# leonavery/KSFD

Hardware: AMD Instinct MI355X
Metric: grid-point-updates/sec (implicit step) (higher is better)
Workload: dtype f64

## Files before the change

### ksfd_amd/csrc/handle.hip.h

```cpp
#pragma once
enum { KC_RHS = 0, KC_JVP, KC_MULTIDOT, KC_GSUPDATE, KC_LINCOMB, KC_BASISAXPY, KC_FINISH, KC_REDUCE,
       KC_GFIELD, KC_VELOCITY, KC_MISC, KC_HALO, KC_MG, KC_SPECTRAL };
static const char *kc_names[KSFD_NKCLASS] = { "rhs", "jvp", "multidot", "gs_update", "lincomb", "basis_axpy",
                                              "rosw_finish", "reduce", "gfield", "velocity", "misc", "halo", "mg", "spectral" };
extern "C" const char *ksfd_kernel_class_name(int32_t c) { return (c >= 0 && c < KSFD_NKCLASS) ? kc_names[c] : "?"; }

static thread_local std::string g_create_error;

struct EvPair { hipEvent_t a, b; int cls; };

struct MGLevel {
    KGeom G;
    KPhys P;
    KVec kv;
    int64_t vlen = 0;
    int nblk = 1;
    double *coef = nullptr;
    float *dinv = nullptr;
    double *x = nullptr, *b = nullptr, *r = nullptr, *d = nullptr, *Ad = nullptr, *dG = nullptr;
    float *x32 = nullptr, *b32 = nullptr, *r32 = nullptr, *d32 = nullptr;
    float *coef32 = nullptr;
    bool f32 = false;
    double *pv = nullptr;
    double pv_norm = 0.0;
    double lam_max = 2.3;
    double ratio = 60.0;
};

struct SpecState {
    bool ok = false, means_valid = false, tile_major = false;
    int cols_split = 0;
    KFFTPlan px, py, pz;
    int dim = 2, lg_cz = 0, pb = 1, nent = 0, lg_rb3 = 0;
    size_t lds_y3 = 0, lds_z3 = 0;
    int *posz = nullptr, *kzofpos = nullptr;
    float *lz = nullptr;
    int rb = 0, npair = 0, nyp = 0;
    int nch = 1;
    size_t lds_rows = 0, lds_cols = 0;
    kcf *W = nullptr, *W2 = nullptr, *twx = nullptr, *twy = nullptr, *twz = nullptr;
    int *posy = nullptr, *kyofpos = nullptr;
    int2 *ytab = nullptr;
    int lgw = -1;
    int4 *pairtab = nullptr;
    int nxl = 0, nblk_cols = 0, lg_pl = 0;
    std::vector<A2APiece> a2a_fwd_s, a2a_fwd_r, a2a_bwd_s, a2a_bwd_r;
    float *lx = nullptr, *ly = nullptr;
    double a_rr = 0.0, a_rU[KSFD_MAXL] = { 0 };
    long long bad_until = 0;
    bool user_off = false;
    int backoff = 8;
    double rho_step = 0.0, rho_prev = 0.0;
};

struct LUState {
    int64_t n = 0, nnz = 0;
    double *A = nullptr;
    int *piv = nullptr, *perm = nullptr, *info = nullptr;
    long long *col = nullptr;
    double *val = nullptr;
    double *y = nullptr, *z = nullptr;
    std::vector<int> piv_h, perm_h;
    bool valid = false;
    double shift = 0.0;
};

struct ksfd_handle {
    ksfd_config cfg;
    int32_t lig_group[KSFD_MAXL];
    double lig_w[KSFD_MAXL], lig_s[KSFD_MAXL], lig_gamma[KSFD_MAXL], lig_D[KSFD_MAXL];
    double grp_alpha[KSFD_MAXL], grp_beta[KSFD_MAXL];
    KGeom G;
    KPhys P;
    KPhys Pst[4];
    bool Pst_valid[4] = { false, false, false, false };
    KVec kv;
    int rank = 0, size = 1, device = 0;
    bool ring = false;
    int64_t slow0 = 0;
    hipStream_t st = nullptr;
    hipStream_t st_comm = nullptr;
    hipEvent_t ev_ready = nullptr, ev_halo = nullptr;
    bool overlap = true;
    Transport *tr = nullptr;
    std::string err;

    int64_t vlen = 0;
    double *u = nullptr, *usave = nullptr, *Z = nullptr, *bvec = nullptr, *Y = nullptr, *V = nullptr;
    double *t1 = nullptr, *t2 = nullptr, *t3 = nullptr, *errv = nullptr;
    double *ckpt = nullptr;
    double *bstore = nullptr;
    bool spec_guess = true;
    int guess_max = getenv("KSFD_GUESS_MAX") ? std::max(1, std::min(atoi(getenv("KSFD_GUESS_MAX")), 3)) : 2;
    bool spec_predict = true;
    long long n_predicted = 0;
    long long n_residual = 0;
    long long n_host_sync = 0;
    struct SolverMemo { double lamJ; int lam_age, lam_period; double mg_shift_floor; int sf_dir, sf_hold; bool sf_tried_down; double sf_prev_its, sf_prev_floor;
                        long long nsteps, spec_bad_until; int spec_backoff; double spec_rho_step, spec_rho_prev; };
    SpecState spec;
    long long nsteps = 0;
    double spec_from = 0.1;
    SolverMemo ckpt_memo;
    bool ckpt_valid = false;
    double *Gb = nullptr, *dGb = nullptr;
    double *coef = nullptr;
    bool use_frozen = true;
    bool coef_fresh = false;
    double *flat = nullptr;
    double *src[4][KSFD_MAXL + 1];
    double *part = nullptr;
    double *dres = nullptr;
    double *hres = nullptr;
    double *hres_dev = nullptr;
    unsigned long long *pub_flag = nullptr, *pub_flag_dev = nullptr, pub_seq = 0;
    unsigned int *pub_count = nullptr;
    bool zero_copy = true;
    int restart_alloc = 0;
    bool restart_grow = true;
    int nblk_vec = 0;
    bool have_err = false;

    int use_fused = 1;
    int yseg = 48;
    int yseg_jvp = 16;
    int zseg = 32;

    bool profiling = false;
    int prof_only = -1;
    std::vector<EvPair> pending;
    std::vector<hipEvent_t> pool;
    ksfd_profile prof;
    double bytes_acc = 0.0;

    double *gm_dev = nullptr;
    double *gm_host = nullptr;
    std::vector<hipEvent_t> gm_ev;
    int async_mode = 0;

    double *Zb = nullptr;
    double *pvec = nullptr;
    double lamJ = -1.0;
    int lam_age = 0, lam_period = 1;
    int poly_deg = 0;
    double poly_alpha[8];
    double poly_shift = -1.0;
    int poly_max_deg = 6;
    double mg_threshold = 75.0;
    double poly_target = 0.02;
    float *coef32 = nullptr;
    bool rhs_carry = true;
    bool fuse_stage = true;
    bool j3l_attr_set = false, j3l_usable = false;
    bool rhs3d_strip = true;
    bool poly_fp32 = true;

    hipStream_t st_io = nullptr;
    double *snap_dev[2] = { nullptr, nullptr }, *snap_host[2] = { nullptr, nullptr };
    hipEvent_t snap_ready[2] = { nullptr, nullptr }, snap_done[2] = { nullptr, nullptr };
    bool snap_busy[2] = { false, false };
    int snap_next = 0;

    struct RecSpace { bool valid = false; int vb = 0, zb = 0, k = 0, pc = 0; std::vector<double> H; };
    RecSpace rec[4];
    int rec_vtop = 0, rec_ztop = 0;
    int rec_mode = 1;
    int rec_keep = 3;
    bool rhs_dots = true;
    bool rec_mg = false;

    int dr_keep = 0;
    bool dr_carry = false;
    double *dr_P = nullptr, *dr_Phost = nullptr;
    struct DrKept { bool valid = false; int kk = 0, pc = -1; double shift = 0.0, shift_pc = 0.0; std::vector<double> H; };
    DrKept dr;
    ksfd_deflation_stats dr_stats = {};

    LUState lu;

    std::vector<MGLevel> mg;
    double mg_shift_floor = 0.0;
    int sf_dir = 0, sf_hold = 0;
    bool sf_tried_down = false, sf_auto = true;
    double sf_prev_its = 0.0, sf_prev_floor = 0.0;
    bool mg_fp32 = true;
    bool mg_use32 = false;
    bool mg_graph_f32 = false;
    bool mg_warm_power = true;
    bool mg_fuse = true;
    bool mg_ok = false;
    double mg_shift = -1.0;
    bool mg_coef_valid = false;
    hipGraphExec_t mg_graph = nullptr;
    double mg_graph_shift = -1.0, mg_graph_bytes = 0.0;
    const void *mg_graph_x = nullptr;
    bool capturing = false, mg_use_graph = true;
    int mg_nu = 2, mg_ncoarse = 400, mg_power_its = 8;
    double mg_ratio = 6.0, mg_coarse_tol = 0.3;

    double At[4][4], Ginv[4][4], bt[4], b2t[4], asum[4];
};

#define GAMMA_RA 4.3586652150845900e-01

static int fail(ksfd_handle *h, int code, const char *fmt, ...)
{
    char buf[512];
    va_list ap;
    va_start(ap, fmt);
    vsnprintf(buf, sizeof buf, fmt, ap);
    va_end(ap);
    if (h) h->err = buf; else g_create_error = buf;
    return code;
}
#define HIPCHK(h, call)                                                                                   \
    do {                                                                                                  \
        hipError_t e_ = (call);                                                                           \
        if (e_ != hipSuccess) return fail(h, KSFD_EHIP, "%s failed: %s (%s:%d)", #call, hipGetErrorString(e_), __FILE__, __LINE__); \
    } while (0)

static hipEvent_t ev_get(ksfd_handle *h)
{
    if (!h->pool.empty()) { hipEvent_t e = h->pool.back(); h->pool.pop_back(); return e; }
    hipEvent_t e;
    hipEventCreate(&e);
    return e;
}
struct Scope {
    ksfd_handle *h; EvPair p; bool on;
    Scope(ksfd_handle *h_, int cls, double bytes, double alg = -1.0) : h(h_), on(h_->profiling && !h_->capturing && (h_->prof_only < 0 || h_->prof_only == cls))
    {
        h->bytes_acc += bytes;
        h->prof.bytes[cls] += bytes;
        h->prof.alg_bytes[cls] += alg < 0.0 ? bytes : alg;
        h->prof.launches[cls] += 1;
        if (on) { p.a = ev_get(h); p.b = ev_get(h); p.cls = cls; hipEventRecord(p.a, h->st); }
    }
    ~Scope() { if (on) { hipEventRecord(p.b, h->st); h->pending.push_back(p); } }
};
static void prof_resolve(ksfd_handle *h)
{
    if (h->pending.empty()) return;
    hipStreamSynchronize(h->st);
    for (auto &p : h->pending) {
        float ms = 0.f;
        if (hipEventElapsedTime(&ms, p.a, p.b) == hipSuccess) h->prof.ms[p.cls] += ms;
        h->pool.push_back(p.a);
        h->pool.push_back(p.b);
    }
    h->pending.clear();
}

static inline dim3 vgrid(const ksfd_handle *h) { return dim3(h->nblk_vec, h->G.F); }
static inline double vbytes(const ksfd_handle *h, double nvec) { return nvec * 8.0 * (double)h->G.F * (double)h->G.nloc; }

static void build_tableau(ksfd_handle *h)
{
    static const double A[4][4] = { { 0, 0, 0, 0 }, { 8.7173304301691801e-01, 0, 0, 0 },
                                    { 8.4457060015369423e-01, -1.1299064236484185e-01, 0, 0 }, { 0, 0, 1., 0 } };
    static const double Gm[4][4] = { { GAMMA_RA, 0, 0, 0 }, { -8.7173304301691801e-01, GAMMA_RA, 0, 0 },
                                     { -9.0338057013044082e-01, 5.4180672388095326e-02, GAMMA_RA, 0 },
                                     { 2.4212380706095346e-01, -1.2232505839045147e+00, 5.4526025533510214e-01, GAMMA_RA } };
    static const double b[4] = { 2.4212380706095346e-01, -1.2232505839045147e+00, 1.5452602553351020e+00, GAMMA_RA };
    static const double b2[4] = { 3.7810903145819369e-01, -9.6042292212423178e-02, 0.5, 2.1793326075422950e-01 };
    memset(h->Ginv, 0, sizeof h->Ginv);
    for (int col = 0; col < 4; col++)
        for (int i = col; i < 4; i++) {
            double s = (i == col) ? 1.0 : 0.0;
            for (int k = col; k < i; k++) s -= Gm[i][k] * h->Ginv[k][col];
            h->Ginv[i][col] = s / Gm[i][i];
        }
    for (int i = 0; i < 4; i++) {
        h->asum[i] = 0.0;
        for (int j = 0; j < 4; j++) {
            double s = 0.0;
            for (int k = 0; k < 4; k++) s += A[i][k] * h->Ginv[k][j];
            h->At[i][j] = s;
            h->asum[i] += A[i][j];
        }
    }
    for (int j = 0; j < 4; j++) {
        double s = 0.0, s2 = 0.0;
        for (int k = 0; k < 4; k++) { s += b[k] * h->Ginv[k][j]; s2 += b2[k] * h->Ginv[k][j]; }
        h->bt[j] = s;
        h->b2t[j] = s2;
    }
}

static int fill_phys(ksfd_handle *h, const ksfd_config *c, KPhys *dst = nullptr)
{
    if (c->nlig < 1 || c->nlig > KSFD_MAXL || c->ngroups < 1 || c->ngroups > KSFD_MAXL)
        return fail(h, KSFD_EINVAL, "nlig=%d ngroups=%d outside 1..%d", c->nlig, c->ngroups, KSFD_MAXL);
    KPhys &P = dst ? *dst : h->P;
    memset(&P, 0, sizeof P);
    P.nlig = c->nlig; P.ngroups = c->ngroups; P.cap_kind = c->cap_kind;
    for (int a = 0; a < 3; a++) {
        double sp = c->L[a] / (double)c->n[a];
        P.inv_h[a] = 1.0 / sp;
        P.inv_h2[a] = 1.0 / (sp * sp);
    }
    P.s2 = c->s2; P.rhomax = c->rhomax; P.inv_cushion = 1.0 / c->cushion; P.ms = c->maxscale * c->s2;
    P.rhomin = c->rhomin; P.Umin = c->Umin; P.inv_rhomax = 1.0 / c->rhomax;
    for (int l = 0; l < c->nlig; l++) {
        if (c->lig_group[l] < 0 || c->lig_group[l] >= c->ngroups) return fail(h, KSFD_EINVAL, "lig_group[%d] out of range", l);
        P.lig_group[l] = h->lig_group[l] = c->lig_group[l];
        P.lig_w[l] = h->lig_w[l] = c->lig_w[l];
        P.lig_s[l] = h->lig_s[l] = c->lig_s[l];
        P.lig_gamma[l] = h->lig_gamma[l] = c->lig_gamma[l];
        P.lig_D[l] = h->lig_D[l] = c->lig_D[l];
    }
    for (int l = c->nlig; l < KSFD_MAXL; l++) P.lig_group[l] = -1;
    for (int q = 0; q < c->ngroups; q++) {
        P.grp_alpha[q] = h->grp_alpha[q] = c->grp_alpha[q];
        P.grp_beta[q] = h->grp_beta[q] = c->grp_beta[q];
    }
    return KSFD_OK;
}

static int alloc_d(ksfd_handle *h, double **p, int64_t n)
{
    if (hipMalloc((void **)p, sizeof(double) * (size_t)n) != hipSuccess) return fail(h, KSFD_ENOMEM, "hipMalloc of %lld doubles failed", (long long)n);
    return KSFD_OK;
}

static bool fused_ok(const ksfd_handle *h)
{
    return h->use_fused && h->G.dim == 2 && (h->G.nx % 2 == 0) && h->G.nx >= 4 && h->G.sloc >= 4 && h->P.nlig <= 4;
}
static bool strip3d_ok(const ksfd_handle *h)
{
    return h->use_fused && h->G.dim == 3 && (h->G.nx % 2 == 0) && h->G.nx >= 4 && h->P.nlig <= 4;
}
```

### ksfd_amd/csrc/krylov.hip.h

```cpp
#pragma once
static int est_lambda_max(ksfd_handle *h, double shift, int nits)
{
    int rc;
    if (!h->pvec) {
        if (alloc_d(h, &h->pvec, h->vlen)) return KSFD_ENOMEM;
        const int nb = blocks_for(h->vlen);
        hipLaunchKernelGGL(k_hash_fill, dim3(nb), dim3(KSFD_BLOCK), 0, h->st, (long long)h->vlen, h->pvec);
        if ((rc = op_multidot(h, h->pvec, h->pvec, 0))) return rc;
        const double n0 = sqrt(h->hres[0]);
        const double *xs[1] = { h->pvec }; double a[1] = { 1.0 / n0 };
        if ((rc = op_lincomb(h, 1, xs, a, h->pvec))) return rc;
    }
    double lamA = 0.0;
    for (int it = 0; it < nits; it++) {
        if ((rc = op_jvp_frozen_halo(h, h->pvec, 1, shift, h->t3))) return rc;
        if ((rc = op_multidot(h, h->t3, h->t3, 0))) return rc;
        lamA = sqrt(h->hres[0]);
        if (!(lamA > 0.0) || lamA != lamA) return fail(h, KSFD_ENAN, "power iteration on the Jacobian broke down");
        const double *xs[1] = { h->t3 }; double a[1] = { 1.0 / lamA };
        if ((rc = op_lincomb(h, 1, xs, a, h->pvec))) return rc;
    }
    const double est = lamA - shift;
    h->lamJ = est > 0.0 ? est : 0.0;
    return KSFD_OK;
}

static void poly_setup(ksfd_handle *h, double shift)
{
    const double a = 0.97, b = 1.0 + 1.15 * h->lamJ / shift;
    h->poly_shift = shift;
    h->poly_deg = 0;
    const double kappa = b / a;
    if (kappa < 1.3) return;
    const double rc_ = (sqrt(kappa) - 1.0) / (sqrt(kappa) + 1.0);
    int d = (int)ceil(log(h->poly_target) / log(rc_)) - 1;
    d = std::min(std::max(d, 1), std::max(h->poly_max_deg, 1));
    const int n = d + 1;
    double m0 = (b + a) / (b - a), m1 = -2.0 / (b - a);
    double Tp[10] = { 1.0 }, Tc[10] = { m0, m1 }, Tn[10];
    int degc = 1;
    for (int k = 1; k < n; k++) {
        for (int i = 0; i < 10; i++) Tn[i] = 0.0;
        for (int i = 0; i <= degc; i++) { Tn[i] += 2.0 * m0 * Tc[i]; Tn[i + 1] += 2.0 * m1 * Tc[i]; }
        for (int i = 0; i <= degc - 1; i++) Tn[i] -= Tp[i];
        for (int i = 0; i < 10; i++) { Tp[i] = Tc[i]; Tc[i] = Tn[i]; }
        degc++;
    }
    const double t0 = Tc[0];
    for (int i = 0; i <= d; i++) h->poly_alpha[i] = -(Tc[i + 1] / t0) / shift;
    h->poly_deg = d;
}

static int poly_apply(ksfd_handle *h, double shift, double *v, double *z)
{
    int rc;
    const int d = h->poly_deg;
    const double *al = h->poly_alpha;
    if (h->poly_fp32 && h->coef32 && fused_ok(h)) {
        const float *C = h->coef32;
        float *tf[2] = { reinterpret_cast<float *>(h->t1), reinterpret_cast<float *>(h->t2) };
        const double *nod = nullptr;
        if (d == 1) return jvp2d_halo_t<float, double, double, double>(h, C, v, 4, shift, z, nod, al[0], al[1] / shift);
        if ((rc = jvp2d_halo_t<float, double, double, float>(h, C, v, 4, shift, tf[0], nod, al[d - 1], al[d] / shift))) return rc;
        int cur32 = 0;
        for (int i = d - 2; i >= 1; i--) {
            if ((rc = jvp2d_halo_t<float, float, double, float>(h, C, tf[cur32], 3, shift, tf[cur32 ^ 1], (const double *)v, al[i], 1.0 / shift))) return rc;
            cur32 ^= 1;
        }
        return jvp2d_halo_t<float, float, double, double>(h, C, tf[cur32], 3, shift, z, (const double *)v, al[0], 1.0 / shift);
    }
    double *tmp[2] = { h->t1, h->t2 };
    double *cur = (d == 1) ? z : tmp[0];
    if ((rc = op_jvp_frozen_halo(h, v, 4, shift, cur, nullptr, al[d - 1], al[d] / shift))) return rc;
    int flip = 1;
    for (int i = d - 2; i >= 0; i--) {
        double *nxt = (i == 0) ? z : tmp[flip];
        if ((rc = op_jvp_frozen_halo(h, cur, 3, shift, nxt, v, al[i], 1.0 / shift))) return rc;
        cur = nxt;
        flip ^= 1;
    }
    return KSFD_OK;
}

struct LinStats { int its; double rel; };

static void rec_reset(ksfd_handle *h)
{
    for (auto &r : h->rec) r.valid = false;
    h->rec_vtop = h->rec_ztop = 0;
}

static void hess_lsq(const double *H, int k, const double *g, double *y, double *Hy)
{
    const int ld = k + 1;
    std::vector<double> R((size_t)ld * k), q((size_t)k + 1);
    for (int i = 0; i < ld * k; i++) R[i] = H[i];
    for (int i = 0; i <= k; i++) q[i] = g[i];
    for (int j = 0; j < k; j++) {
        const double a = R[j * ld + j], b = R[j * ld + j + 1], den = hypot(a, b);
        const double c = den > 0.0 ? a / den : 1.0, sn = den > 0.0 ? b / den : 0.0;
        for (int l = j; l < k; l++) {
            const double t = c * R[l * ld + j] + sn * R[l * ld + j + 1];
            R[l * ld + j + 1] = -sn * R[l * ld + j] + c * R[l * ld + j + 1];
            R[l * ld + j] = t;
        }
        const double t = c * q[j] + sn * q[j + 1];
        q[j + 1] = -sn * q[j] + c * q[j + 1];
        q[j] = t;
    }
    for (int i = k - 1; i >= 0; i--) {
        double t = q[i];
        for (int l = i + 1; l < k; l++) t -= R[l * ld + i] * y[l];
        y[i] = R[i * ld + i] != 0.0 ? t / R[i * ld + i] : 0.0;
    }
    for (int i = 0; i <= k; i++) {
        double t = 0.0;
        for (int l = 0; l < k; l++) t += H[l * ld + i] * y[l];
        Hy[i] = t;
    }
}

static int gmres(ksfd_handle *h, const double *ustate, double shift, const double *b, double *x,
                 const ksfd_step_opts *o, LinStats *ls, int pcmode, int stage = -1, double tol_abs = -1.0)
{
    const bool use_pc = pcmode == 1;
    h->dr.valid = false;
    const double shift_pc = std::max(shift, h->mg_shift_floor);
    const bool use_poly = pcmode == 2 || pcmode == 3;
    auto apply_A = [&](const double *vin, double *wout) -> int {
        return h->use_frozen ? op_jvp_frozen(h, vin, 1, shift, wout) : op_jvp(h, ustate, vin, 1, shift, wout);
    };
    const int m_opt = std::min(o->ksp_restart > 0 ? o->ksp_restart : 30, h->restart_alloc);
    const int maxit = o->ksp_max_it > 0 ? o->ksp_max_it : 2000;
    const int64_t vs = h->vlen;
    const bool rec_full = use_pc && h->rec_mg && stage >= 0 && stage < 4 && h->use_frozen && h->rec_mode > 0;
    bool rec_on = stage >= 0 && stage < 4 && h->rec_mode > 0 && h->use_frozen && (!use_pc || rec_full);
    if (!rec_on || stage == 0 || h->restart_alloc - h->rec_vtop < (rec_full ? 16 : 6)) { if (stage != 0) rec_on = false; rec_reset(h); }
    const int vb = rec_on ? h->rec_vtop : 0, zb = rec_on ? h->rec_ztop : 0;
    const int m = h->restart_alloc - vb;
    int m_cur = (rec_full && rec_on) ? m : std::min(m_opt, m);
    double *V = h->V + (int64_t)vb * vs;
    double *Zq = use_poly ? h->Zb + (int64_t)zb * vs : nullptr;
    int rc;
    std::vector<double> H((size_t)(m + 1) * m, 0.0), Hraw((size_t)(m + 1) * m, 0.0), cs(m), sn(m), g(m + 1), y(m), hcol(m + 2), d(m + 2), Gm((size_t)(m + 1) * (m + 1), 0.0);
    static const int sel[4][3] = { { -1, -1, -1 }, { 0, -1, -1 }, { 0, -1, -1 }, { 0, 2, -1 } };
    int first_space = -1;
    std::vector<double> g_first((size_t)h->restart_alloc + 3, 0.0);
    if (rec_on && stage > 0)
        for (int q = 0; q < stage && first_space < 0; q++) {
            bool use = h->rec_mode == 2 || rec_full;
            for (int e = 0; e < 3; e++) use = use || sel[stage][e] == q;
            if (use && h->rec[q].valid && h->rec[q].pc == pcmode) first_space = q;
        }
    if (first_space >= 0) {
        const ksfd_handle::RecSpace &S = h->rec[first_space];
        if ((rc = op_multidot(h, b, h->V + (int64_t)S.vb * vs, S.k + 1))) return rc;
        for (int i = 0; i <= S.k + 1; i++) g_first[i] = h->hres[i];
    } else if ((rc = op_multidot(h, b, V, 0))) return rc;
    const double bn = sqrt(first_space >= 0 ? g_first[h->rec[first_space].k + 1] : h->hres[0]);
    ls->its = 0; ls->rel = 0.0;
    if (!(bn > 0.0)) {
        if (bn != bn) return fail(h, KSFD_ENAN, "GMRES: right-hand side is not finite");
        HIPCHK(h, hipMemsetAsync(x, 0, sizeof(double) * (size_t)vs, h->st));
        return KSFD_OK;
    }
    const double tol = tol_abs > 0.0 ? tol_abs : std::max(o->ksp_rtol * bn, o->ksp_atol);
    double beta = bn, rn = bn;
    int total = 0;
    bool first = true;
    bool x_set = false;
    bool restarted = false;
    const double *rsrc = b;
    const bool defer_x0 = rec_on && !use_pc;
    std::vector<double> xcoef((size_t)std::max(h->restart_alloc + 2, KSFD_MAXDOT), 0.0);
    bool x0_pending = false;
    double *const Xbase = use_poly ? h->Zb : h->V;
    const int xslot0 = use_poly ? zb : vb;
    bool pc_x0_pending = false;
    double *const rbuf = (x == h->t3) ? V : h->t3;
    if (rec_on && stage > 0) {
        int last_space = -1;
        for (int q = 0; q < stage; q++) {
            bool use = h->rec_mode == 2 || rec_full;
            for (int e = 0; e < 3; e++) use = use || sel[stage][e] == q;
            if (use && h->rec[q].valid && h->rec[q].pc == pcmode) last_space = q;
        }
        bool have_norm = false;
        for (int q = 0; q < stage; q++) {
            bool use = h->rec_mode == 2 || rec_full;
            for (int e = 0; e < 3; e++) use = use || sel[stage][e] == q;
            const ksfd_handle::RecSpace &S = h->rec[q];
            if (!use || !S.valid || S.pc != pcmode) continue;
            const double *Vs = h->V + (int64_t)S.vb * vs;
            const double *Zs = use_poly ? h->Zb + (int64_t)S.zb * vs : Vs;
            std::vector<double> gq_((size_t)S.k + 2), yq_((size_t)S.k + 1), Hy_((size_t)S.k + 2), neg_((size_t)S.k + 2);
            double *gq = gq_.data(), *yq = yq_.data(), *Hy = Hy_.data(), *neg = neg_.data();
            if (q == first_space && rsrc == b) {
                for (int i = 0; i <= S.k; i++) gq[i] = g_first[i];
            } else {
                if ((rc = op_multidot(h, rsrc, Vs, S.k + 1))) return rc;
                for (int i = 0; i <= S.k; i++) gq[i] = h->hres[i];
            }
            hess_lsq(S.H.data(), S.k, gq, yq, Hy);
            if (use_pc) {
                if ((rc = op_basis_axpy(h, h->t2, Vs, S.k, yq, pc_x0_pending ? 1.0 : 0.0))) return rc;
                pc_x0_pending = true;
            } else if (defer_x0) {
                for (int i = 0; i < S.k; i++) xcoef[(use_poly ? S.zb : S.vb) + i] += yq[i];
                x0_pending = true;
            } else {
// ... 355 lines not shown
```

### ksfd_amd/csrc/ksfd_hip.hip

```cpp
#include <hip/hip_runtime.h>
#include <dlfcn.h>
#include <math.h>
#include <stdarg.h>
#include <stdio.h>
#include <stdlib.h>
#include <string.h>
#include <string>
#include <vector>

#include "../../include/ksfd_hip.h"
#include "stencil.hip.h"
#include "mg.hip.h"
#include "spectral.hip.h"
#include "lu.hip.h"
#include "transport.h"


#include "handle.hip.h"
#include "ops.hip.h"
#include "spectral_host.hip.h"
#include "mg_host.hip.h"
#include "krylov.hip.h"
#include "krylov_dr.hip.h"
#include "lu_host.hip.h"
// ... 40 lines not shown
{
    if (!cfg || !out) return fail(nullptr, KSFD_EINVAL, "null argument");
    *out = nullptr;
    if (cfg->dim < 1 || cfg->dim > 3) return fail(nullptr, KSFD_EINVAL, "dim must be 1, 2 or 3");
    for (int a = 0; a < cfg->dim; a++)
        if (cfg->n[a] < 5) return fail(nullptr, KSFD_EINVAL, "n[%d]=%lld < 5: the width-2 periodic star needs >= 5 points", a, (long long)cfg->n[a]);
    ksfd_handle *h = new ksfd_handle();
    memset(h->src, 0, sizeof h->src);
    memset(&h->prof, 0, sizeof h->prof);
    h->cfg = *cfg;
    h->cfg.lig_group = nullptr; h->cfg.lig_w = h->cfg.lig_s = h->cfg.lig_gamma = h->cfg.lig_D = nullptr;
    h->cfg.grp_alpha = h->cfg.grp_beta = nullptr;
    int rc = fill_phys(h, cfg);
    if (rc) { g_create_error = h->err; delete h; return rc; }
    h->rank = dist ? dist->rank : 0;
    h->size = dist ? dist->size : 1;
    h->device = dist ? dist->device : 0;
    if (h->size < 1 || h->rank < 0 || h->rank >= h->size) { delete h; return fail(nullptr, KSFD_EINVAL, "bad rank/size"); }
    h->ring = h->size > 1 || (dist && dist->transport != 0);
    int ndev = 0;
    if (hipGetDeviceCount(&ndev) != hipSuccess || ndev < 1) { delete h; return fail(nullptr, KSFD_EHIP, "no HIP device available (libksfd_hip has no CPU path)"); }
    if (h->device < 0 || h->device >= ndev) { delete h; return fail(nullptr, KSFD_EINVAL, "device %d of %d", h->device, ndev); }
#define CFAIL(code, ...) do { int rc_ = fail(nullptr, code, __VA_ARGS__); ksfd_destroy(h); return rc_; } while (0)
    if (hipSetDevice(h->device) != hipSuccess) CFAIL(KSFD_EHIP, "hipSetDevice(%d) failed", h->device);
    if (hipStreamCreateWithFlags(&h->st, hipStreamNonBlocking) != hipSuccess) CFAIL(KSFD_EHIP, "hipStreamCreate failed");
    if (h->ring && (hipStreamCreateWithFlags(&h->st_comm, hipStreamNonBlocking) != hipSuccess ||
                        hipEventCreateWithFlags(&h->ev_ready, hipEventDisableTiming) != hipSuccess ||
                        hipEventCreateWithFlags(&h->ev_halo, hipEventDisableTiming) != hipSuccess)) CFAIL(KSFD_EHIP, "comm stream/event creation failed");

    KGeom &G = h->G;
    G.dim = cfg->dim; G.F = cfg->nlig + 1;
    const int slow = cfg->dim - 1;
    int64_t nglob = cfg->n[slow];
    if (h->size > 1 && (nglob % h->size != 0 || nglob / h->size < 4))
        CFAIL(KSFD_EINVAL, "slab axis extent %lld must be divisible by %d ranks with >= 4 units each", (long long)nglob, h->size);
    int64_t sloc = nglob / h->size;
    h->slow0 = sloc * h->rank;
    G.ng = h->ring ? 2 : 0;
    G.wrap_slow = !h->ring;
    G.nx = cfg->n[0]; G.ny = cfg->dim >= 2 ? cfg->n[1] : 1; G.nz = cfg->dim >= 3 ? cfg->n[2] : 1;
    if (slow == 0) G.nx = sloc; else if (slow == 1) G.ny = sloc; else G.nz = sloc;
    G.inner = slow == 0 ? 1 : (slow == 1 ? G.nx : G.nx * G.ny);
    G.sloc = sloc;
    G.plane = (sloc + 2 * G.ng) * G.inner;
    G.nloc = sloc * G.inner;
    h->kv.plane = G.plane; h->kv.off = (long long)G.ng * G.inner; h->kv.nloc = G.nloc; h->kv.nf = G.F;
    h->vlen = (int64_t)G.F * G.plane;
    h->nblk_vec = (int)std::min<long long>((G.nloc + KSFD_BLOCK - 1) / KSFD_BLOCK, 2048);
    build_tableau(h);

    h->restart_alloc = 30;
    int fit_local = 30;
    {
        size_t mfree = 0, mtotal = 0;
        if (hipMemGetInfo(&mfree, &mtotal) == hipSuccess && mfree > 0) {
            const double vecbytes = 8.0 * (double)h->vlen;
            const double room = 0.92 * (double)mfree / vecbytes - 30.0;
            const int fit_room = (int)floor(std::min((room - 1.0) / 2.0, 1.0e6));
            const int fit_40 = (int)floor(std::min(0.4 * (double)mfree / vecbytes / 2.0, 1.0e6));
            static const int cap = getenv("KSFD_RESTART_MAX") ? std::max(8, std::min(atoi(getenv("KSFD_RESTART_MAX")), 120)) : 120;
            fit_local = std::max(std::min(std::min(cap, fit_room), fit_40), std::min(30, fit_room));
        }
    }
    if (alloc_d(h, &h->dres, 128)) CFAIL(KSFD_ENOMEM, "%s", h->err.c_str());
    if (h->ring) {
        std::string terr;
        h->tr = make_transport(dist, G.F, G.inner, terr);
        if (!h->tr) CFAIL(KSFD_ECOMM, "transport %d: %s", dist->transport, terr.c_str());
        double v = -(double)fit_local;
        if (hipMemcpyAsync(h->dres, &v, sizeof v, hipMemcpyHostToDevice, h->st) != hipSuccess || h->tr->allreduce(h->dres, 1, 1, h->st))
            CFAIL(KSFD_ECOMM, "agreeing on the restart length failed: %s", h->tr->error().c_str());
        if (h->tr->result_on_host()) v = h->tr->host_result()[0];
        else if (hipMemcpyAsync(&v, h->dres, sizeof v, hipMemcpyDeviceToHost, h->st) != hipSuccess || hipStreamSynchronize(h->st) != hipSuccess)
            CFAIL(KSFD_EHIP, "reading the agreed restart length failed");
        fit_local = (int)(-v + 0.5);
    }
    if (fit_local != 30) {
        if (fit_local < 8) CFAIL(KSFD_ENOMEM, "grid too large for this device: a vector is %.2f GB, the solver needs ~47 of them (restart length that fits: %d)", 8.0 * (double)h->vlen / 1e9, fit_local);
        h->restart_alloc = fit_local;
    }
    double **vecs[] = { &h->u, &h->usave, &h->Z, &h->bvec, &h->t1, &h->t2, &h->t3, &h->errv };
    for (double **v : vecs) {
        if (alloc_d(h, v, h->vlen)) CFAIL(KSFD_ENOMEM, "%s", h->err.c_str());
        hipMemsetAsync(*v, 0, sizeof(double) * (size_t)h->vlen, h->st);
    }
    if (alloc_d(h, &h->Y, 4 * h->vlen) || alloc_d(h, &h->V, (int64_t)(h->restart_alloc + 1) * h->vlen) ||
        alloc_d(h, &h->Gb, G.plane) || alloc_d(h, &h->dGb, G.plane) || alloc_d(h, &h->coef, (int64_t)(3 + cfg->nlig) * G.plane) ||
        alloc_d(h, &h->flat, (int64_t)std::max(G.F, 3) * G.nloc) ||
        alloc_d(h, &h->part, (int64_t)(2 * KSFD_MAXDOT + 4) * 4096))
        CFAIL(KSFD_ENOMEM, "%s", h->err.c_str());
    if (hipMalloc((void **)&h->Zb, sizeof(double) * (size_t)h->restart_alloc * (size_t)h->vlen) != hipSuccess) { h->Zb = nullptr; hipGetLastError(); }
    hipMemsetAsync(h->Y, 0, sizeof(double) * (size_t)(4 * h->vlen), h->st);
    hipMemsetAsync(h->V, 0, sizeof(double) * (size_t)((h->restart_alloc + 1) * h->vlen), h->st);
    if (hipHostMalloc((void **)&h->hres, sizeof(double) * 128 + 64, hipHostMallocMapped | hipHostMallocCoherent) != hipSuccess) CFAIL(KSFD_ENOMEM, "hipHostMalloc failed");
    h->pub_flag = reinterpret_cast<unsigned long long *>(h->hres + 128);
    *h->pub_flag = 0;
    if (hipHostGetDevicePointer((void **)&h->hres_dev, h->hres, 0) != hipSuccess || hipMalloc((void **)&h->pub_count, sizeof(unsigned int)) != hipSuccess ||
        hipMemset(h->pub_count, 0, sizeof(unsigned int)) != hipSuccess) { h->zero_copy = false; h->hres_dev = nullptr; }
    else h->pub_flag_dev = reinterpret_cast<unsigned long long *>(h->hres_dev + 128);
    {
        const int m = h->restart_alloc;
        const size_t ndev = (size_t)(m + 1) * (m + 1) + (size_t)(m + 1) * m + 2 * m + (m + 1) + KSFD_MAXDOT + 1 + 2 * (m + 1);
        const size_t nhost = 2 * (m + 1) + (size_t)(m + 1) * m + (m + 1);
        if (alloc_d(h, &h->gm_dev, (int64_t)ndev)) CFAIL(KSFD_ENOMEM, "%s", h->err.c_str());
        if (hipHostMalloc((void **)&h->gm_host, sizeof(double) * nhost, hipHostMallocDefault) != hipSuccess) CFAIL(KSFD_ENOMEM, "hipHostMalloc failed");
        h->gm_ev.resize(m + 1);
        for (auto &e : h->gm_ev) if (hipEventCreateWithFlags(&e, hipEventDisableTiming) != hipSuccess) CFAIL(KSFD_EHIP, "hipEventCreate failed");
    }

    spec_build(h);
    if (mg_build(h)) { mg_free(h); h->mg_ok = false; }
    if ((h->spec.ok || h->mg_ok) && alloc_d(h, &h->bstore, 3 * h->vlen)) { h->bstore = nullptr; h->spec_guess = false; h->err.clear(); }
    if (h->ring) {
        double flags[3] = { h->spec.ok ? 1.0 : 0.0, h->mg_ok ? 1.0 : 0.0, (h->spec_guess && h->bstore) ? 1.0 : 0.0 };
        for (double &f : flags) f = -f;
        if (hipMemcpyAsync(h->dres, flags, sizeof flags, hipMemcpyHostToDevice, h->st) != hipSuccess || h->tr->allreduce(h->dres, 3, 1, h->st))
            CFAIL(KSFD_ECOMM, "agreeing on the available solvers failed: %s", h->tr->error().c_str());
        if (h->tr->result_on_host()) memcpy(flags, h->tr->host_result(), sizeof flags);
        else if (hipMemcpyAsync(flags, h->dres, sizeof flags, hipMemcpyDeviceToHost, h->st) != hipSuccess || hipStreamSynchronize(h->st) != hipSuccess)
            CFAIL(KSFD_EHIP, "reading the agreed solver flags failed");
        if (flags[0] > -0.5 && h->spec.ok) spec_free(h);
        if (flags[1] > -0.5 && h->mg_ok) { mg_free(h); h->mg_ok = false; }
        if (flags[2] > -0.5) h->spec_guess = false;
    }
    if (hipStreamSynchronize(h->st) != hipSuccess) CFAIL(KSFD_EHIP, "stream sync failed in create");
#undef CFAIL
    *out = h;
    return KSFD_OK;
}

extern "C" int ksfd_rccl_unique_id(void *out128)
{
    if (!out128) return KSFD_EINVAL;
    std::string err;
    RcclApi api;
    if (!api.load(err)) return fail(nullptr, KSFD_ECOMM, "%s", err.c_str());
    auto getid = (decltype(&ncclGetUniqueId))dlsym(api.lib, "ncclGetUniqueId");
    if (!getid) return fail(nullptr, KSFD_ECOMM, "librccl lacks ncclGetUniqueId");
    ncclUniqueId id;
    ncclResult_t r = getid(&id);
    if (r != ncclSuccess) return fail(nullptr, KSFD_ECOMM, "ncclGetUniqueId: %s", api.GetErrorString(r));
    memcpy(out128, &id, sizeof id);
    return KSFD_OK;
}

extern "C" int ksfd_update_params(ksfd_handle *h, const ksfd_config *cfg)
{
    if (!h || !cfg) return KSFD_EINVAL;
    if (cfg->dim != h->cfg.dim || cfg->nlig != h->cfg.nlig) return fail(h, KSFD_EINVAL, "update_params cannot change dim/nlig");
    for (int a = 0; a < 3; a++) if (cfg->n[a] != h->cfg.n[a]) return fail(h, KSFD_EINVAL, "update_params cannot change the grid");
    h->cfg = *cfg;
    h->cfg.lig_group = nullptr; h->cfg.lig_w = h->cfg.lig_s = h->cfg.lig_gamma = h->cfg.lig_D = nullptr;
    h->cfg.grp_alpha = h->cfg.grp_beta = nullptr;
    h->coef_fresh = false;
    return fill_phys(h, cfg);
}

extern "C" int ksfd_set_stage_params(ksfd_handle *h, int32_t stage, const ksfd_config *cfg)
{
    if (!h || stage < -1 || stage > 3) return KSFD_EINVAL;
    if (!cfg) {
        for (int s = 0; s < 4; s++) if (stage == -1 || s == stage) h->Pst_valid[s] = false;
        return KSFD_OK;
    }
    if (cfg->dim != h->cfg.dim || cfg->nlig != h->cfg.nlig) return fail(h, KSFD_EINVAL, "set_stage_params cannot change dim/nlig");
    for (int a = 0; a < 3; a++) if (cfg->n[a] != h->cfg.n[a] || cfg->L[a] != h->cfg.L[a]) return fail(h, KSFD_EINVAL, "set_stage_params cannot change the grid");
    for (int s = 0; s < 4; s++) {
        if (stage != -1 && s != stage) continue;
        int rc = fill_phys(h, cfg, &h->Pst[s]);
        if (rc) return rc;
        h->Pst_valid[s] = true;
    }
    return KSFD_OK;
}

extern "C" int ksfd_local_range(const ksfd_handle *h, int64_t *b, int64_t *e)
{
    if (!h) return KSFD_EINVAL;
    if (b) *b = h->slow0;
    if (e) *e = h->slow0 + h->G.sloc;
    return KSFD_OK;
}
extern "C" int64_t ksfd_local_size(const ksfd_handle *h) { return h ? (int64_t)h->G.F * h->G.nloc : 0; }
extern "C" double *ksfd_device_state(ksfd_handle *h) { return h ? h->u : nullptr; }
extern "C" int64_t ksfd_device_plane_stride(const ksfd_handle *h) { return h ? h->G.plane : 0; }
extern "C" int64_t ksfd_device_interior_offset(const ksfd_handle *h) { return h ? (int64_t)h->G.ng * h->G.inner : 0; }

extern "C" int ksfd_set_state(ksfd_handle *h, const double *u, int32_t layout)
{
    if (!h || !u) return KSFD_EINVAL;
    hipSetDevice(h->device);
    int rc = upload(h, u, layout, h->u);
    h->coef_fresh = false;
    if (rc) return rc;
    HIPCHK(h, hipStreamSynchronize(h->st));
    return KSFD_OK;
}
extern "C" int ksfd_snapshot_begin(ksfd_handle *h, int32_t layout, int32_t *slot)
{
    if (!h || !slot) return KSFD_EINVAL;
    if (layout < 0 || layout > 2) return fail(h, KSFD_EINVAL, "bad layout %d", layout);
    hipSetDevice(h->device);
    const KGeom &G = h->G;
    const size_t bytes = sizeof(double) * (size_t)G.F * G.nloc;
    if (!h->st_io) {
        if (hipStreamCreateWithFlags(&h->st_io, hipStreamNonBlocking) != hipSuccess) return fail(h, KSFD_EHIP, "hipStreamCreate (io) failed");
        for (int q = 0; q < 2; q++) {
            if (hipMalloc((void **)&h->snap_dev[q], bytes) != hipSuccess || hipHostMalloc((void **)&h->snap_host[q], bytes, hipHostMallocDefault) != hipSuccess)
                return fail(h, KSFD_ENOMEM, "snapshot staging buffers (%zu bytes each) could not be allocated", bytes);
            if (hipEventCreateWithFlags(&h->snap_ready[q], hipEventDisableTiming) != hipSuccess ||
                hipEventCreateWithFlags(&h->snap_done[q], hipEventDisableTiming) != hipSuccess) return fail(h, KSFD_EHIP, "hipEventCreate failed");
        }
    }
    const int q = h->snap_next;
    h->snap_next ^= 1;
    if (h->snap_busy[q]) HIPCHK(h, hipEventSynchronize(h->snap_done[q]));
    {
        Scope sc(h, KC_MISC, vbytes(h, 2));
        hipLaunchKernelGGL(k_to_host_layout, vgrid(h), dim3(KSFD_BLOCK), 0, h->st, G, layout, (const double *)h->u, G.plane,
                           (long long)G.ng * G.inner, h->snap_dev[q]);
    }
    HIPCHK(h, hipGetLastError());
    HIPCHK(h, hipEventRecord(h->snap_ready[q], h->st));
    HIPCHK(h, hipStreamWaitEvent(h->st_io, h->snap_ready[q], 0));
    HIPCHK(h, hipMemcpyAsync(h->snap_host[q], h->snap_dev[q], bytes, hipMemcpyDeviceToHost, h->st_io));
    HIPCHK(h, hipEventRecord(h->snap_done[q], h->st_io));
    h->snap_busy[q] = true;
    *slot = q;
    return KSFD_OK;
}

extern "C" int ksfd_snapshot_wait(ksfd_handle *h, int32_t slot, const double **host)
{
    if (!h || !host || slot < 0 || slot > 1) return KSFD_EINVAL;
    if (!h->snap_busy[slot]) return fail(h, KSFD_EINVAL, "snapshot slot %d holds nothing", slot);
    hipSetDevice(h->device);
    HIPCHK(h, hipEventSynchronize(h->snap_done[slot]));
    *host = h->snap_host[slot];
    return KSFD_OK;
}

extern "C" int ksfd_checkpoint(ksfd_handle *h, int32_t op)
{
    if (!h || op < 0 || op > 1) return KSFD_EINVAL;
    hipSetDevice(h->device);
    h->dr.valid = false;
    if (op == 0) {
        if (!h->ckpt && alloc_d(h, &h->ckpt, h->vlen)) return KSFD_ENOMEM;
        HIPCHK(h, hipMemcpyAsync(h->ckpt, h->u, sizeof(double) * (size_t)h->vlen, hipMemcpyDeviceToDevice, h->st));
        h->ckpt_memo = { h->lamJ, h->lam_age, h->lam_period, h->mg_shift_floor, h->sf_dir, h->sf_hold, h->sf_tried_down, h->sf_prev_its, h->sf_prev_floor,
                         h->nsteps, h->spec.bad_until, h->spec.backoff, h->spec.rho_step, h->spec.rho_prev };
        for (MGLevel &L : h->mg) L.pv_norm = 0.0;
        h->ckpt_valid = true;
        return KSFD_OK;
    }
    if (!h->ckpt_valid) return fail(h, KSFD_EINVAL, "no checkpoint has been saved");
    HIPCHK(h, hipMemcpyAsync(h->u, h->ckpt, sizeof(double) * (size_t)h->vlen, hipMemcpyDeviceToDevice, h->st));
    h->coef_fresh = false;
    const ksfd_handle::SolverMemo &m = h->ckpt_memo;
    h->lamJ = m.lamJ; h->lam_age = m.lam_age; h->lam_period = m.lam_period; h->mg_shift_floor = m.mg_shift_floor;
    h->sf_dir = m.sf_dir; h->sf_hold = m.sf_hold; h->sf_tried_down = m.sf_tried_down; h->sf_prev_its = m.sf_prev_its; h->sf_prev_floor = m.sf_prev_floor;
    h->nsteps = m.nsteps; h->spec.bad_until = m.spec_bad_until; h->spec.backoff = m.spec_backoff; h->spec.means_valid = false;
    h->spec.rho_step = m.spec_rho_step; h->spec.rho_prev = m.spec_rho_prev;
    h->mg_coef_valid = false; h->mg_shift = -1.0; h->poly_shift = -1.0; h->have_err = false;
    for (MGLevel &L : h->mg) L.pv_norm = 0.0;
    rec_reset(h);
    return KSFD_OK;
}

extern "C" int ksfd_set_state_random(ksfd_handle *h, const int64_t *nc, const double *z, double rho0)
{
    if (!h || !nc || !z) return KSFD_EINVAL;
    hipSetDevice(h->device);
    int64_t n = 1;
    for (int a = 0; a < 3; a++) {
        if (a < h->G.dim ? nc[a] < 1 : nc[a] != 1) return fail(h, KSFD_EINVAL, "coarse grid must be >= 1 per used axis and 1 elsewhere");
        n *= nc[a];
    }
    double *dz = nullptr;
    h->coef_fresh = false;
    if (hipMalloc((void **)&dz, sizeof(double) * (size_t)n) != hipSuccess) return fail(h, KSFD_ENOMEM, "hipMalloc of the coarse samples failed");
    hipError_t e = hipMemcpyAsync(dz, z, sizeof(double) * (size_t)n, hipMemcpyHostToDevice, h->st);
    const KGeom &G = h->G;
    int nb = (int)std::min<long long>((G.nloc + KSFD_BLOCK - 1) / KSFD_BLOCK, 65535);
    if (e == hipSuccess) {
        Scope sc(h, KC_MISC, vbytes(h, 1));
        NL_DISPATCH(h->P.nlig, hipLaunchKernelGGL((k_random_start<NL>), dim3(nb), dim3(KSFD_BLOCK), 0, h->st, G, h->P, (long long)h->cfg.n[G.dim - 1],
                                                  (long long)h->slow0, (long long)nc[0], (long long)nc[1], (long long)nc[2], (const double *)dz, rho0, h->u));
        e = hipGetLastError();
    }
    if (e == hipSuccess) e = hipStreamSynchronize(h->st);
    hipFree(dz);
    if (e != hipSuccess) return fail(h, KSFD_EHIP, "random start: %s", hipGetErrorString(e));
    return KSFD_OK;
}
extern "C" int ksfd_get_state(ksfd_handle *h, double *u, int32_t layout)
{
    if (!h || !u) return KSFD_EINVAL;
    hipSetDevice(h->device);
    return download(h, h->u, layout, u);
}

extern "C" int ksfd_set_source(ksfd_handle *h, int32_t stage, int32_t field, const double *srch, int32_t layout)
{
    if (!h || field < 0 || field >= h->G.F || stage < -1 || stage > 3) return h ? fail(h, KSFD_EINVAL, "bad stage/field") : KSFD_EINVAL;
    if (layout != KSFD_LAYOUT_SOA) return fail(h, KSFD_EINVAL, "sources are single dense planes: pass layout SOA");
    hipSetDevice(h->device);
    for (int s = 0; s < 4; s++) {
        if (stage != -1 && s != stage) continue;
        if (!srch) {
            if (h->src[s][field]) { HIPCHK(h, hipStreamSynchronize(h->st)); hipFree(h->src[s][field]); h->src[s][field] = nullptr; }
            continue;
        }
        if (!h->src[s][field] && alloc_d(h, &h->src[s][field], h->G.nloc)) return KSFD_ENOMEM;
        HIPCHK(h, hipMemcpyAsync(h->src[s][field], srch, sizeof(double) * (size_t)h->G.nloc, hipMemcpyHostToDevice, h->st));
    }
    HIPCHK(h, hipStreamSynchronize(h->st));
    return KSFD_OK;
}

extern "C" int ksfd_rhs(ksfd_handle *h, double t, const double *uh, double *outh, int32_t layout)
{
    (void)t;
    if (!h || !outh) return KSFD_EINVAL;
    hipSetDevice(h->device);
    int rc;
    double *uin = h->u;
    if (uh) { if ((rc = upload(h, uh, layout, h->t1))) return rc; uin = h->t1; }
    if ((rc = halo(h, uin))) return rc;
    if ((rc = op_rhs(h, uin, 0, h->t3))) return rc;
    return download(h, h->t3, layout, outh);
}

extern "C" int ksfd_jvp(ksfd_handle *h, const double *uh, const double *vh, double *outh, int32_t layout)
{
    if (!h || !vh || !outh) return KSFD_EINVAL;
    hipSetDevice(h->device);
    int rc;
    double *uin = h->u;
    if (uh) { if ((rc = upload(h, uh, layout, h->t1))) return rc; uin = h->t1; }
    if ((rc = upload(h, vh, layout, h->t2))) return rc;
    if ((rc = halo(h, uin)) || (rc = halo(h, h->t2))) return rc;
    if (!uh && h->use_frozen) {
        if ((rc = ensure_coef(h, true))) return rc;
        if ((rc = op_jvp_frozen(h, h->t2, 0, 0.0, h->t3))) return rc;
    } else if ((rc = op_jvp(h, uin, h->t2, 0, 0.0, h->t3))) return rc;
    return download(h, h->t3, layout, outh);
}

static int velocity_common(ksfd_handle *h, const double *uin, double *vel_dev, double vmax[3])
{
    const KGeom &G = h->G;
    int rc;
    const double *Gplane = h->Gb;
    if (uin == h->u && h->use_frozen) {
        if ((rc = ensure_coef(h))) return rc;
        Gplane = h->coef + G.plane;
    } else {
        if ((rc = halo(h, (double *)uin))) return rc;
        Scope sc(h, KC_GFIELD, 8.0 * (G.F + 1) * (double)G.plane);
        NL_DISPATCH(h->P.nlig, hipLaunchKernelGGL((k_gfield<NL, false>), dim3(plane_blocks(G)), dim3(KSFD_BLOCK), 0, h->st, G, h->P, uin, (const double *)nullptr, h->Gb, (double *)nullptr));
    }
    int nb = (int)std::min<long long>((G.nloc + KSFD_BLOCK - 1) / KSFD_BLOCK, 1024);
    if (vmax && !vel_dev && G.dim == 2 && (G.nx % 2 == 0) && G.nx >= 4) {
        const int bx = (int)((G.nx / 2 + KSFD_BLOCK - 1) / KSFD_BLOCK), by = (int)std::min<long long>(G.sloc, std::max(1, 2048 / bx));
        nb = bx * by;
        Scope sc(h, KC_VELOCITY, 8.0 * (double)G.nloc);
        hipLaunchKernelGGL(k_velmax2d, dim3(bx, by), dim3(KSFD_BLOCK), 0, h->st, G, h->P, Gplane, h->part);
    } else if (vmax && !vel_dev && G.dim == 3 && (G.nx % 2 == 0) && G.nx >= 4 && G.ny >= 4 && G.nx * G.ny < (1LL << 30)) {
        const int bx = (int)((G.nx / 2 * G.ny + KSFD_BLOCK - 1) / KSFD_BLOCK);
        int zseg = (int)G.sloc;
        while (zseg >= 32 && (long long)bx * ((G.sloc + zseg - 1) / zseg) < 8192) zseg = (zseg + 1) / 2;
        const int by = (int)((G.sloc + zseg - 1) / zseg);
        nb = bx * by;
        if (3LL * nb > part_capacity()) return fail(h, KSFD_EINVAL, "velocity_max: grid too large for the partial-result buffer");
        Scope sc(h, KC_VELOCITY, 8.0 * (double)G.nloc);
        hipLaunchKernelGGL(k_velmax3d, dim3(bx, by), dim3(KSFD_BLOCK), 0, h->st, G, h->P, zseg, Gplane, h->part);
    } else {
        Scope sc(h, KC_VELOCITY, 8.0 * (double)G.nloc * (1 + (vel_dev ? G.dim : 0)));
        hipLaunchKernelGGL(k_velocity, dim3(nb), dim3(KSFD_BLOCK), 0, h->st, G, h->P, Gplane, vel_dev, vmax ? h->part : (double *)nullptr);
    }
    HIPCHK(h, hipGetLastError());
    if (vmax) {
        if ((rc = reduce_rows(h, 3, nb, 1))) return rc;
        for (int a = 0; a < 3; a++) vmax[a] = a < G.dim ? h->hres[a] : 0.0;
    }
    return KSFD_OK;
}

extern "C" int ksfd_velocity(ksfd_handle *h, const double *uh, double *velh, int32_t layout)
{
    if (!h || !velh) return KSFD_EINVAL;
    if (layout != KSFD_LAYOUT_SOA) return fail(h, KSFD_EINVAL, "velocity output is dim dense SoA planes: pass layout SOA for it");
    hipSetDevice(h->device);
    int rc;
    double *uin = h->u;
    if (uh) { if ((rc = upload(h, uh, layout, h->t1))) return rc; uin = h->t1; }
    if ((rc = velocity_common(h, uin, h->flat, nullptr))) return rc;
    HIPCHK(h, hipMemcpyAsync(velh, h->flat, sizeof(double) * (size_t)h->G.dim * h->G.nloc, hipMemcpyDeviceToHost, h->st));
    HIPCHK(h, hipStreamSynchronize(h->st));
    return KSFD_OK;
}

extern "C" int ksfd_velocity_max(ksfd_handle *h, double vmax[3])
{
    if (!h || !vmax) return KSFD_EINVAL;
    hipSetDevice(h->device);
    return velocity_common(h, h->u, nullptr, vmax);
}

extern "C" int ksfd_groom(ksfd_handle *h)
{
    if (!h) return KSFD_EINVAL;
    hipSetDevice(h->device);
    Scope sc(h, KC_MISC, vbytes(h, 2));
    hipLaunchKernelGGL(k_groom, vgrid(h), dim3(KSFD_BLOCK), 0, h->st, h->kv, h->u, h->P.rhomin, h->P.Umin);
    HIPCHK(h, hipGetLastError());
    return KSFD_OK;
}

extern "C" int ksfd_count_worms(ksfd_handle *h, double *total)
{
    if (!h || !total) return KSFD_EINVAL;
    hipSetDevice(h->device);
    {
        Scope sc(h, KC_MISC, 8.0 * (double)h->G.nloc);
        hipLaunchKernelGGL(k_sum_rho, dim3(h->nblk_vec), dim3(KSFD_BLOCK), 0, h->st, h->kv, h->u, h->part);
    }
    HIPCHK(h, hipGetLastError());
    int rc = reduce_rows(h, 1, h->nblk_vec, 0);
    if (rc) return rc;
    *total = h->hres[0];
    return KSFD_OK;
}

extern "C" int ksfd_scale_rho(ksfd_handle *h, double factor)
{
    if (!h) return KSFD_EINVAL;
    hipSetDevice(h->device);
    h->coef_fresh = false;
    Scope sc(h, KC_MISC, 16.0 * (double)h->G.nloc);
    hipLaunchKernelGGL(k_mul_rho, dim3(h->nblk_vec), dim3(KSFD_BLOCK), 0, h->st, h->kv, h->u, (const double *)nullptr, factor);
    HIPCHK(h, hipGetLastError());
    return KSFD_OK;
}

extern "C" int ksfd_mul_rho(ksfd_handle *h, const double *fh)
{
    if (!h || !fh) return KSFD_EINVAL;
    hipSetDevice(h->device);
    HIPCHK(h, hipMemcpyAsync(h->flat, fh, sizeof(double) * (size_t)h->G.nloc, hipMemcpyHostToDevice, h->st));
    h->coef_fresh = false;
    Scope sc(h, KC_MISC, 24.0 * (double)h->G.nloc);
    hipLaunchKernelGGL(k_mul_rho, dim3(h->nblk_vec), dim3(KSFD_BLOCK), 0, h->st, h->kv, h->u, (const double *)h->flat, 1.0);
    HIPCHK(h, hipGetLastError());
    HIPCHK(h, hipStreamSynchronize(h->st));
    return KSFD_OK;
}

extern "C" int ksfd_jacobian_nnz(ksfd_handle *h, int64_t *nrows, int64_t *nnz)
{
    if (!h) return KSFD_EINVAL;
    const int64_t npts = 4 * h->G.dim + 1;
    if (nrows) *nrows = (int64_t)h->G.F * h->G.nloc;
    if (nnz) *nnz = h->G.nloc * ((int64_t)h->G.F * npts + (int64_t)h->P.nlig * (npts + 1));
    return KSFD_OK;
}

extern "C" int ksfd_jacobian_csr(ksfd_handle *h, int64_t *rowptr, int64_t *col, double *val)
{
    if (!h || !rowptr || !col || !val) return KSFD_EINVAL;
    hipSetDevice(h->device);
    int64_t nrows, nnz;
    ksfd_jacobian_nnz(h, &nrows, &nnz);
    int rc;
    if ((rc = ensure_coef(h))) return rc;
    long long *dcol = nullptr;
    double *dval = nullptr;
    if (hipMalloc((void **)&dcol, sizeof(long long) * (size_t)nnz) != hipSuccess ||
        hipMalloc((void **)&dval, sizeof(double) * (size_t)nnz) != hipSuccess) {
        if (dcol) hipFree(dcol);
        return fail(h, KSFD_ENOMEM, "hipMalloc of the CSR staging buffers failed");
    }
    const KGeom &G = h->G;
    int nb = (int)std::min<long long>((G.nloc + KSFD_BLOCK - 1) / KSFD_BLOCK, 65535);
    {
        Scope sc(h, KC_MISC, 16.0 * (double)nnz + 8.0 * (3 + h->P.nlig) * (double)G.nloc);
        NL_DISPATCH(h->P.nlig, hipLaunchKernelGGL((k_jac_csr<NL>), dim3(nb), dim3(KSFD_BLOCK), 0, h->st, G, h->P, (const double *)h->coef,
                                                  (long long)h->cfg.n[G.dim - 1], (long long)h->slow0, dcol, dval));
    }
    hipError_t e = hipGetLastError();
    if (e == hipSuccess) e = hipMemcpyAsync(col, dcol, sizeof(long long) * (size_t)nnz, hipMemcpyDeviceToHost, h->st);
    if (e == hipSuccess) e = hipMemcpyAsync(val, dval, sizeof(double) * (size_t)nnz, hipMemcpyDeviceToHost, h->st);
    if (e == hipSuccess) e = hipStreamSynchronize(h->st);
    hipFree(dcol);
    hipFree(dval);
    if (e != hipSuccess) return fail(h, KSFD_EHIP, "jacobian export: %s", hipGetErrorString(e));
    const int64_t npts = 4 * G.dim + 1, F = G.F, per = F * npts + (F - 1) * (npts + 1);
    for (int64_t p = 0; p < G.nloc; p++) {
        rowptr[p * F] = p * per;
        for (int64_t l = 1; l < F; l++) rowptr[p * F + l] = p * per + F * npts + (l - 1) * (npts + 1);
    }
    rowptr[nrows] = nnz;
    return KSFD_OK;
}


extern "C" void ksfd_default_step_opts(ksfd_step_opts *o)
{
    memset(o, 0, sizeof *o);
    o->rtol = 1e-5; o->atol = 1e-5;
    o->adapt = 1; o->max_reject = 10;
    o->clip_lo = 0.1; o->clip_hi = 5.0;
    o->dt_min = 1e-20; o->dt_max = 1e4;
    o->safety = 0.9; o->reject_safety = 0.5;
    o->ksp_rtol = 1e-6; o->ksp_atol = 1e-50;
    o->ksp_restart = 30; o->ksp_max_it = 2000;
    o->pc_type = 2;
}

extern "C" int ksfd_step(ksfd_handle *h, double *t, double *hstep, const ksfd_step_opts *opts, ksfd_step_stats *stats)
{
    if (!h || !t || !hstep || !opts) return KSFD_EINVAL;
    hipSetDevice(h->device);
    const bool direct = opts->pc_type == 5;
    if (direct) {
        const int g = direct_guard(h);
        if (g) return g;
    }
    const bool dr_on = h->dr_keep > 0 && !direct;
    if (dr_on) {
        const int m_dr = std::min(opts->ksp_restart > 0 ? opts->ksp_restart : 30, h->restart_alloc);
        if (h->dr_keep > m_dr - 3) return fail(h, KSFD_EINVAL, "deflation: keep = %d needs a restart length of at least %d (ksp_restart %d, basis vectors allocated %d)", h->dr_keep, h->dr_keep + 3, (int)opts->ksp_restart, h->restart_alloc);
    }
    memset(&h->dr_stats, 0, sizeof h->dr_stats);
    if (getenv("KSFD_PC_SIGMA")) { h->mg_shift_floor = atof(getenv("KSFD_PC_SIGMA")); h->sf_auto = false; }
    ksfd_step_stats st;
    memset(&st, 0, sizeof st);
    const double bytes0 = h->bytes_acc;
    const int64_t rhs0 = h->prof.launches[KC_RHS], jvp0 = h->prof.launches[KC_JVP];
    int64_t launches0 = 0;
    for (int c = 0; c < KSFD_NKCLASS; c++) launches0 += h->prof.launches[c];
    const long long sync0 = h->n_host_sync, pred0 = h->n_predicted, resid0 = h->n_residual;
    int rc = KSFD_OK;
    const int64_t vs = h->vlen;
    double hh = *hstep;
    bool prev_accept = !(opts->reserved & 4);
    bool lam_done = false;
    int rejects = 0;
    const int max_rej = opts->max_reject < 0 ? 0x7fffffff : opts->max_reject;
    const bool single = (opts->reserved & 2) != 0;
    {
        Scope sc(h, KC_MISC, vbytes(h, 3));
        hipLaunchKernelGGL(k_groom, vgrid(h), dim3(KSFD_BLOCK), 0, h->st, h->kv, h->u, h->P.rhomin, h->P.Umin, h->usave);
        if (hipGetLastError() != hipSuccess) { rc = fail(h, KSFD_EHIP, "k_groom launch failed"); goto out; }
    }
    if ((rc = halo(h, h->u))) goto out;
    if (h->use_frozen && (rc = ensure_coef(h, true))) goto out;
    h->poly_shift = -1.0;
    h->nsteps++;
    if (h->spec.rho_step > 0.0) h->spec.rho_prev = h->spec.rho_step;
    h->spec.rho_step = 0.0;
    while (true) {
        const double shift = 1.0 / (GAMMA_RA * hh);
        h->dr.valid = false;
        double dmax = h->P.s2, lap = 0.0;
        for (int l = 0; l < h->P.nlig; l++) dmax = std::max(dmax, h->P.lig_D[l]);
        for (int a = 0; a < h->G.dim; a++) lap += (16.0 / 3.0) * h->P.inv_h2[a];
        const double stiff = dmax * lap / shift;
        const double mg_from = h->mg_threshold * ((double)h->G.F * (double)h->G.nloc < 8.0e6 ? 3.0 : 1.0);
        bool use_spec = !direct && h->spec.ok && h->use_frozen && (opts->pc_type == 4 || (opts->pc_type == 2 && stiff >= (fused_ok(h) ? h->spec_from : std::max(h->spec_from, 0.3)) && h->nsteps > h->spec.bad_until && !h->spec.user_off));
        if (use_spec) {
            if (!h->Zb && alloc_d(h, &h->Zb, (int64_t)h->restart_alloc * h->vlen)) { rc = KSFD_ENOMEM; goto out; }
            if (!h->spec.means_valid && (rc = spec_means(h))) goto out;
        }
        const bool use_pc = !direct && !use_spec && h->mg_ok && h->use_frozen && (opts->pc_type == 1 || (opts->pc_type == 2 && stiff > mg_from));
        bool use_poly = false;
        if (!use_spec && !use_pc && h->use_frozen && (opts->pc_type == 2 || opts->pc_type == 3) && stiff >= 0.3) {
            if (!h->Zb && alloc_d(h, &h->Zb, (int64_t)h->restart_alloc * h->vlen)) { rc = KSFD_ENOMEM; goto out; }
            if (!lam_done) {
                if (h->lamJ < 0.0 || ++h->lam_age >= h->lam_period) {
                    const double before = h->lamJ;
                    if ((rc = est_lambda_max(h, shift, before < 0.0 ? 8 : 2))) goto out;
                    const bool stable = before > 0.0 && fabs(h->lamJ - before) <= 0.02 * before;
                    h->lam_period = stable ? std::min(2 * h->lam_period, 8) : 1;
                    h->lam_age = 0;
                }
                lam_done = true;
            }
            if (h->poly_shift != shift) poly_setup(h, shift);
            use_poly = h->poly_deg >= 1 && h->poly_max_deg >= 1;
        }
        const bool small = (double)h->G.F * (double)h->G.nloc <= 6.0e6;
        const bool use_async = !dr_on && !direct && !use_spec && !use_pc && !use_poly && h->use_frozen && !(opts->reserved & 1) && stiff >= 1e-3 &&
                               (!h->ring || h->tr->device_allreduce()) &&
                               (h->async_mode == 1 || (h->async_mode == 2 && small));
        h->mg_use32 = opts->ksp_rtol >= 1e-7;
        const bool fuse_stage = (fused_ok(h) || (strip3d_ok(h) && h->rhs3d_strip)) && h->P.nlig <= 4 && h->fuse_stage;
        const int its_before = st.linear_its;
        bool spec_failed = false;
        const bool guess_on = (use_spec || use_pc) && fuse_stage && h->spec_guess && h->bstore;
        double gb[4][4];
        if (direct && !(rc = ensure_coef(h, true))) rc = direct_factor(h, shift);
        for (int i = 0; i < 4 && !rc; i++) {
            const double *zin = h->u;
            double bnorm2 = -1.0;
            bool rhs_dots_done = false;
            double rhs_dot[2] = { 0.0, 0.0 };
            double *bcur = (guess_on && i < 3) ? h->bstore + (int64_t)i * vs : h->bvec;
            if (fuse_stage) {
                KComb cmb = KComb{};
                for (int j = 0; j < i; j++) {
                    if (h->At[i][j] != 0.0) { cmb.yin[cmb.nin] = h->Y + (int64_t)j * vs; cmb.ain[cmb.nin++] = h->At[i][j]; }
                    if (h->Ginv[i][j] != 0.0) { cmb.yout[cmb.nout] = h->Y + (int64_t)j * vs; cmb.aout[cmb.nout++] = -h->Ginv[i][j] / hh; }
                }
                const int gdot_j0 = std::max(0, i - h->guess_max), gdot_n = (guess_on && i > 0 && h->rhs_dots) ? i - gdot_j0 : 0;
                const bool rhs_norm = use_spec && fused_ok(h) && (!(guess_on && i > 0) || (gdot_n > 0 && gdot_n <= 2 && strip_waves(h) * (1 + gdot_n) <= part_capacity()));
                rhs_dots_done = rhs_norm && gdot_n > 0;
                if ((rc = op_rhs(h, h->u, i, bcur, &cmb, rhs_norm, i > 0 ? h->Y + (int64_t)(i - 1) * vs : nullptr, rhs_dots_done ? gdot_n : 0,
                                 rhs_dots_done ? h->bstore + (int64_t)gdot_j0 * vs : nullptr))) break;
                if (rhs_norm) bnorm2 = h->hres[0];
                if (rhs_dots_done) for (int j = 0; j < gdot_n; j++) rhs_dot[j] = h->hres[1 + j];
            } else {
            if (i > 0) {
                const double *xs[5]; double a[5]; int nt = 0;
                xs[nt] = h->u; a[nt++] = 1.0;
                for (int j = 0; j < i; j++) if (h->At[i][j] != 0.0) { xs[nt] = h->Y + (int64_t)j * vs; a[nt++] = h->At[i][j]; }
                if (nt > 1) {
                    if ((rc = op_lincomb(h, nt, xs, a, h->Z))) break;
                    if ((rc = halo(h, h->Z))) break;
                    zin = h->Z;
                }
            }
            if ((rc = op_rhs(h, zin, i, h->bvec))) break;
            if (i > 0) {
                const double *xs[5]; double a[5]; int nt = 0;
                xs[nt] = h->bvec; a[nt++] = 1.0;
                for (int j = 0; j < i; j++) if (h->Ginv[i][j] != 0.0) { xs[nt] = h->Y + (int64_t)j * vs; a[nt++] = -h->Ginv[i][j] / hh; }
                if (nt > 1 && (rc = op_lincomb(h, nt, xs, a, h->bvec))) break;
            }
            }
            LinStats ls;
            SpecGuess sg;
            sg.n = 0;
            {
                if (guess_on) {
                    if (i == 0) {
                        if (bnorm2 < 0.0) { if ((rc = op_multidot(h, bcur, bcur, 0))) break; bnorm2 = h->hres[0]; }
                        gb[0][0] = bnorm2;
                    }
                    else {
                        const int j0 = std::max(0, i - h->guess_max), ng = i - j0;
                        if (rhs_dots_done) {
                            for (int j = 0; j < ng; j++) gb[i][j0 + j] = gb[j0 + j][i] = rhs_dot[j];
                            gb[i][i] = bnorm2;
                        } else {
                            if ((rc = op_multidot(h, bcur, h->bstore + (int64_t)j0 * vs, ng))) break;
                            for (int j = 0; j < ng; j++) gb[i][j0 + j] = gb[j0 + j][i] = h->hres[j];
                            gb[i][i] = bnorm2 = h->hres[ng];
                        }
                        double M[3][4];
                        for (int a = 0; a < ng; a++) { for (int c = 0; c < ng; c++) M[a][c] = gb[j0 + a][j0 + c]; M[a][ng] = gb[i][j0 + a]; M[a][a] *= 1.0 + 1e-13; }
                        bool okls = ng > 0;
                        for (int c = 0; c < ng && okls; c++) {
                            int pv = c;
                            for (int a = c + 1; a < ng; a++) if (fabs(M[a][c]) > fabs(M[pv][c])) pv = a;
                            if (!(fabs(M[pv][c]) > 0.0)) { okls = false; break; }
                            for (int q = 0; q <= ng; q++) std::swap(M[c][q], M[pv][q]);
                            for (int a = c + 1; a < ng; a++) { const double f = M[a][c] / M[c][c]; for (int q = c; q <= ng; q++) M[a][q] -= f * M[c][q]; }
                        }
                        double cf[3] = { 0, 0, 0 };
                        for (int a = ng - 1; a >= 0 && okls; a--) { double t = M[a][ng]; for (int q = a + 1; q < ng; q++) t -= M[a][q] * cf[q]; cf[a] = t / M[a][a]; }
                        double pred = gb[i][i];
                        for (int a = 0; a < ng; a++) { pred -= 2.0 * cf[a] * gb[i][j0 + a]; for (int c = 0; c < ng; c++) pred += cf[a] * cf[c] * gb[j0 + a][j0 + c]; }
                        if (okls && pred == pred && pred < 0.09 * gb[i][i]) {
                            for (int j = 0; j < ng; j++) if (cf[j] != 0.0) { sg.Y[sg.n] = h->Y + (int64_t)(j0 + j) * vs; sg.b[sg.n] = h->bstore + (int64_t)(j0 + j) * vs; sg.c[sg.n++] = cf[j]; }
                        }
                    }
                }
            }
            if (direct) {
                rc = direct_stage(h, shift, bcur, h->Y + (int64_t)i * vs, opts, &ls);
                st.pc_used |= 16;
            } else if (use_spec) {
                const bool skip = spec_failed && opts->pc_type == 2;
                if (!skip) {
                    rc = spec_solve(h, shift, bcur, h->Y + (int64_t)i * vs, opts, &ls, bnorm2, opts->pc_type == 2 ? (h->spec.backoff > 8 ? 8 : 40) : 0, sg.n ? &sg : nullptr);
                    st.pc_used |= 8;
                }
                if (skip || (rc == KSFD_ELINEAR && opts->pc_type == 2)) {
                    if (!skip) st.linear_its += ls.its;
                    spec_failed = true;
                    const bool mg_here = h->mg_ok && stiff > 0.3;
                    rc = gmres(h, h->u, shift, bcur, h->Y + (int64_t)i * vs, opts, &ls, mg_here ? 1 : 0);
                    st.pc_used |= mg_here ? 2 : 1;
                }
            } else if (use_pc && sg.n) {
                double *xi = h->Y + (int64_t)i * vs;
                const double *xs[3]; double a[3];
                for (int j = 0; j < sg.n; j++) { xs[j] = sg.Y[j]; a[j] = sg.c[j]; }
                if ((rc = op_lincomb(h, sg.n, xs, a, xi)) || (rc = halo(h, xi)) || (rc = op_jvp_frozen(h, xi, 2, shift, h->Z, bcur))) break;
                const double tol = std::max(opts->ksp_rtol * sqrt(bnorm2), opts->ksp_atol);
                rc = dr_on ? gmres_dr(h, h->u, shift, h->Z, h->t3, opts, &ls, 1, i, tol)
                           : gmres(h, h->u, shift, h->Z, h->t3, opts, &ls, 1, i, tol);
                if (!rc) { const double *x2[2] = { xi, h->t3 }; double a2[2] = { 1.0, 1.0 }; rc = op_lincomb(h, 2, x2, a2, xi); }
                st.pc_used |= 2;
            } else {
            rc = use_async ? gmres_async(h, shift, bcur, h->Y + (int64_t)i * vs, opts, &ls)
                 : dr_on ? gmres_dr(h, h->u, shift, bcur, h->Y + (int64_t)i * vs, opts, &ls, use_pc ? 1 : (use_poly ? 2 : 0), i)
                           : gmres(h, h->u, shift, bcur, h->Y + (int64_t)i * vs, opts, &ls, use_pc ? 1 : (use_poly ? 2 : 0), i);
            st.pc_used |= use_pc ? 2 : (use_poly ? 4 : 1);
            }
            st.linear_its += ls.its;
            st.ksp_resid = ls.rel;
            {
                static const bool stage_trace = getenv("KSFD_STAGE_TRACE") != nullptr;
                if (stage_trace) fprintf(stderr, "[stage %d] its %d rel %.2e guess %d\n", i, ls.its, ls.rel, sg.n);
            }
            if (rc == KSFD_ELINEAR && !direct && !use_pc && h->mg_ok && h->use_frozen && opts->pc_type) {
                rc = gmres(h, h->u, shift, bcur, h->Y + (int64_t)i * vs, opts, &ls, 1);
                st.pc_used |= 2;
                st.linear_its += ls.its;
                st.ksp_resid = ls.rel;
            }
        }
        if (use_spec && opts->pc_type == 2) {
            if (spec_failed || st.linear_its - its_before > 48) {
                h->spec.bad_until = h->nsteps + h->spec.backoff;
                h->spec.backoff = std::min(2 * h->spec.backoff, 512);
            } else h->spec.backoff = 8;
        }
        if (!rc && use_pc && h->sf_auto) {
            const double its = (double)(st.linear_its - its_before);
            if (h->sf_dir == 0) {
                if (h->sf_hold > 0) h->sf_hold--;
                else if (its > 64.0) {
                    h->sf_prev_its = its; h->sf_prev_floor = h->mg_shift_floor;
                    h->mg_shift_floor = 2.0 * std::max(h->mg_shift_floor, shift);
                    h->sf_dir = 1; h->sf_tried_down = false;
                }
            } else if (its < 0.95 * h->sf_prev_its) {
                h->sf_prev_its = its; h->sf_prev_floor = h->mg_shift_floor;
                h->mg_shift_floor = h->sf_dir > 0 ? 2.0 * h->mg_shift_floor : 0.5 * h->mg_shift_floor;
                if (h->mg_shift_floor <= shift) { h->sf_dir = 0; h->sf_hold = 25; }
            } else {
                h->mg_shift_floor = h->sf_prev_floor;
                if (h->sf_dir > 0 && !h->sf_tried_down && 0.5 * h->sf_prev_floor > shift) {
                    h->sf_dir = -1; h->sf_tried_down = true;
                    h->mg_shift_floor = 0.5 * h->sf_prev_floor;
                } else { h->sf_dir = 0; h->sf_hold = 25; }
            }
        }
        if (rc == KSFD_ELINEAR && opts->adapt && !single && rejects < max_rej && hh * 0.25 >= opts->dt_min) {
            rejects++;
            st.rejections = rejects;
            prev_accept = false;
            if ((rc = op_copy(h, h->u, h->usave))) goto out;
            hh *= 0.25;
            *hstep = hh;
            if ((rc = halo(h, h->u))) goto out;
            continue;
        }
        if (rc) { op_copy(h, h->u, h->usave); hipStreamSynchronize(h->st); goto out; }
        {
            Scope sc(h, KC_FINISH, vbytes(h, 7));
            hipLaunchKernelGGL(k_rosw_finish, dim3(h->nblk_vec), dim3(KSFD_BLOCK), 0, h->st, h->kv, h->u, h->Y, vs,
                               h->bt[0], h->bt[1], h->bt[2], h->bt[3], h->b2t[0] - h->bt[0], h->b2t[1] - h->bt[1],
                               h->b2t[2] - h->bt[2], h->b2t[3] - h->bt[3], opts->atol, opts->rtol, h->errv, h->part);
        }
        h->have_err = true;
        h->coef_fresh = false;
        if ((rc = reduce_rows(h, 1, h->nblk_vec, 0))) goto out;
        {
            double ntot = (double)h->G.F * (double)h->cfg.n[0] * (double)h->cfg.n[1] * (double)h->cfg.n[2];
            st.wrms = sqrt(h->hres[0] / ntot);
        }
        if (!(st.wrms == st.wrms) || isinf(st.wrms)) {
            op_copy(h, h->u, h->usave); hipStreamSynchronize(h->st);
            h->coef_fresh = h->use_frozen;
            rc = fail(h, KSFD_ENAN, "non-finite error norm at t=%g h=%g", *t, hh);
            goto out;
        }
        bool accept = true;
        double hnext = hh;
        if (opts->adapt) {
            double safety = opts->safety;
            if (st.wrms > 1.0) {
                if (!prev_accept) safety *= opts->reject_safety;
                accept = hh < (1.0 + 1.4901161193847656e-08) * opts->dt_min;
            }
            double hfac = st.wrms > 0.0 ? safety * pow(st.wrms, -1.0 / 3.0) : INFINITY;
            hfac = std::min(std::max(hfac, opts->clip_lo), opts->clip_hi);
            hnext = std::min(std::max(hh * hfac, opts->dt_min), opts->dt_max);
        }
        prev_accept = accept;
        if (accept) {
            st.accepted = 1; st.h_used = hh;
            *t += hh;
            *hstep = hnext;
            break;
        }
        rejects++;
        st.rejections = rejects;
        if ((rc = op_copy(h, h->u, h->usave))) goto out;
        h->coef_fresh = h->use_frozen;
        hh = hnext;
        *hstep = hnext;
        if (single) break;
        if (rejects > max_rej) { rc = fail(h, KSFD_EREJECT, "step rejected %d times at t=%g", rejects, *t); break; }
        if ((rc = halo(h, h->u))) goto out;
    }
out:
    prof_resolve(h);
    st.bytes = h->bytes_acc - bytes0;
    st.rhs_evals = (int32_t)(h->prof.launches[KC_RHS] - rhs0);
    st.jvp_evals = (int32_t)(h->prof.launches[KC_JVP] - jvp0);
    {
        int64_t l1 = 0;
        for (int c = 0; c < KSFD_NKCLASS; c++) l1 += h->prof.launches[c];
        st.launches = (int32_t)(l1 - launches0);
    }
    st.host_syncs = (int32_t)(h->n_host_sync - sync0);
    st.predicted_final = (int32_t)(h->n_predicted - pred0);
    st.residual_evals = (int32_t)(h->n_residual - resid0);
    if (stats) *stats = st;
    return rc;
}

extern "C" int ksfd_get_last_error_vector(ksfd_handle *h, double *eh, int32_t layout)
{
    if (!h || !eh) return KSFD_EINVAL;
    if (!h->have_err) return fail(h, KSFD_EINVAL, "no step has been attempted yet");
    hipSetDevice(h->device);
    return download(h, h->errv, layout, eh);
}

extern "C" int ksfd_set_profiling(ksfd_handle *h, int32_t on)
{
    if (!h) return KSFD_EINVAL;
    prof_resolve(h);
    if (on < 0 || on >= 2 + KSFD_NKCLASS) return KSFD_EINVAL;
    h->profiling = on != 0;
    h->prof_only = on >= 2 ? on - 2 : -1;
    return KSFD_OK;
}
extern "C" int ksfd_get_profile(ksfd_handle *h, ksfd_profile *p, int32_t reset)
{
    if (!h || !p) return KSFD_EINVAL;
    prof_resolve(h);
    *p = h->prof;
    if (reset) memset(&h->prof, 0, sizeof h->prof);
    return KSFD_OK;
}
extern "C" int ksfd_set_mg_params(ksfd_handle *h, int32_t nu, int32_t ncoarse_max, int32_t power_its, double ratio, double coarse_tol)
{
    if (!h) return KSFD_EINVAL;
    if (nu > 0) h->mg_nu = nu;
    if (ncoarse_max > 0) h->mg_ncoarse = ncoarse_max;
    if (power_its > 0) h->mg_power_its = power_its;
    if (ratio > 1.0) h->mg_ratio = ratio;
    if (coarse_tol > 0.0) h->mg_coarse_tol = coarse_tol;
    h->mg_use_graph = power_its != -7 && !h->ring;
    h->mg_shift = -1.0;
    return KSFD_OK;
}
extern "C" int ksfd_set_poly_params(ksfd_handle *h, int32_t max_degree, double target, double mg_threshold)
{
    if (!h || max_degree < 0 || max_degree > 7) return KSFD_EINVAL;
    if (mg_threshold > 0.0) h->mg_threshold = mg_threshold;
    h->poly_max_deg = max_degree;
    if (target > 0.0 && target < 1.0) h->poly_target = target;
    h->poly_shift = -1.0;
    return KSFD_OK;
}
extern "C" int ksfd_spectral_apply(ksfd_handle *h, double shift, const double *vh, double *outh, int32_t layout)
{
    if (!h || !vh || !outh || !(shift > 0.0)) return KSFD_EINVAL;
    hipSetDevice(h->device);
    if (!h->spec.ok) return fail(h, KSFD_EINVAL, "spectral preconditioner not available for this handle (needs power-of-two extents of 32 ... 16384 points; 1, 2, 4 or 8 slab ranks with an all-to-all transport)");
    int rc;
    if ((rc = upload(h, vh, layout, h->t2))) return rc;
    if ((rc = ensure_coef(h))) return rc;
    if ((rc = spec_means(h)) || (rc = spec_apply(h, shift, h->t2, h->t3))) return rc;
    return download(h, h->t3, layout, outh);
}
extern "C" int ksfd_direct_apply(ksfd_handle *h, double shift, const double *vh, double *outh, int32_t layout)
{
    if (!h || !vh || !outh) return KSFD_EINVAL;
    if (!isfinite(shift)) return fail(h, KSFD_EINVAL, "direct_apply: non-finite shift");
    if (layout < 0 || layout > 2) return fail(h, KSFD_EINVAL, "bad layout %d", layout);
    hipSetDevice(h->device);
    int rc;
    if ((rc = direct_guard(h))) return rc;
    if ((rc = ensure_coef(h)) || (rc = direct_factor(h, shift))) return rc;
    if ((rc = upload(h, vh, layout, h->t2)) || (rc = direct_solve(h, h->t2, h->t3))) return rc;
    return download(h, h->t3, layout, outh);
}
extern "C" int ksfd_set_deflation(ksfd_handle *h, int32_t keep, int32_t carry_stages)
{
    if (!h) return KSFD_EINVAL;
    if (keep < 0 || keep > 16) return fail(h, KSFD_EINVAL, "deflation: keep = %d outside 0 (off) .. 16", (int)keep);
    h->dr_keep = keep;
    h->dr_carry = carry_stages != 0;
    h->dr.valid = false;
    return KSFD_OK;
}
extern "C" int ksfd_get_deflation_stats(ksfd_handle *h, ksfd_deflation_stats *s)
{
    if (!h || !s) return KSFD_EINVAL;
    *s = h->dr_stats;
    return KSFD_OK;
}
extern "C" int32_t ksfd_basis_capacity(const ksfd_handle *h) { return h ? h->restart_alloc + 1 : 0; }
extern "C" int ksfd_basis_rotate(ksfd_handle *h, int32_t nin, int32_t nout, const double *P, const double *vin, double *vout, int32_t layout)
{
    if (!h || !P || !vin || !vout) return KSFD_EINVAL;
    if (layout < 0 || layout > 2) return fail(h, KSFD_EINVAL, "bad layout %d", layout);
    if (nin < 1 || nout < 1 || nout > nin || nout > KSFD_ROT_MAXOUT || nin > KSFD_ROT_MAXIN || nin > h->restart_alloc + 1)
        return fail(h, KSFD_EINVAL, "basis_rotate: %d -> %d vectors outside 1 <= nout <= %d, nout <= nin <= min(%d, %d)", (int)nin, (int)nout, KSFD_ROT_MAXOUT, KSFD_ROT_MAXIN, h->restart_alloc + 1);
    hipSetDevice(h->device);
    h->dr.valid = false;
    rec_reset(h);
    int rc;
    const int64_t nl = (int64_t)h->G.F * h->G.nloc;
    for (int i = 0; i < nin; i++) {
        if ((rc = upload(h, vin + (int64_t)i * nl, layout, h->V + (int64_t)i * h->vlen))) return rc;
        HIPCHK(h, hipStreamSynchronize(h->st));
    }
    std::vector<double> Pp((size_t)nin * KSFD_ROT_MAXOUT, 0.0);
    for (int i = 0; i < nin; i++) for (int j = 0; j < nout; j++) Pp[(size_t)i * KSFD_ROT_MAXOUT + j] = P[(size_t)i * nout + j];
    if ((rc = op_basis_rotate(h, h->V, nin, nout, Pp.data(), KSFD_ROT_MAXOUT))) return rc;
    for (int i = 0; i < nin; i++)
        if ((rc = download(h, h->V + (int64_t)i * h->vlen, layout, vout + (int64_t)i * nl))) return rc;
    return KSFD_OK;
}
extern "C" int ksfd_set_spectral_params(ksfd_handle *h, double from_stiffness, int32_t enable)
{
    if (!h) return KSFD_EINVAL;
    if (from_stiffness > 0.0) h->spec_from = from_stiffness;
    if (enable == 0) h->spec.user_off = true;
    else if (enable > 0) { h->spec.user_off = false; h->spec.bad_until = 0; h->spec.backoff = 8; }
    return KSFD_OK;
}
extern "C" int ksfd_synchronize(ksfd_handle *h)
{
    if (!h) return KSFD_EINVAL;
    hipSetDevice(h->device);
    HIPCHK(h, hipStreamSynchronize(h->st));
    return KSFD_OK;
}
extern "C" int ksfd_set_tuning(ksfd_handle *h, int32_t use_fused, int32_t yseg, int32_t yseg_jvp)
{
    if (!h) return KSFD_EINVAL;
    if (use_fused >= 0) {
        h->use_fused = use_fused & 1; h->use_frozen = !(use_fused & 2); h->overlap = !(use_fused & 4);
        h->async_mode = (use_fused & 8) ? 1 : 0;
        h->rec_mode = (use_fused & 16) ? 0 : ((use_fused & 32) ? 2 : 1);
        if ((use_fused >> 6) & 7) h->rec_keep = std::min((use_fused >> 6) & 7, 4);
        h->poly_fp32 = !(use_fused & 512);
        h->fuse_stage = !(use_fused & 1024);
        h->zero_copy = !(use_fused & 2048) && h->hres_dev;
        h->rhs3d_strip = !(use_fused & 8192);
        h->spec_guess = !(use_fused & 16384);
        h->rhs_carry = !(use_fused & 32768);
        h->spec_predict = !(use_fused & 65536);
        h->restart_grow = !(use_fused & 131072);
        h->mg_warm_power = !(use_fused & 262144);
        h->mg_fp32 = !(use_fused & 524288);
        h->rec_mg = (use_fused & 1048576) != 0;
        h->rhs_dots = !(use_fused & 2097152);
        if (h->mg_fuse != !(use_fused & 4096)) { h->mg_fuse = !(use_fused & 4096); h->mg_shift = -1.0; if (h->mg_graph) { hipGraphExecDestroy(h->mg_graph); h->mg_graph = nullptr; } }
    }
    if (yseg > 0) h->yseg = yseg;
    if (yseg_jvp > 0) h->yseg_jvp = yseg_jvp;
    return KSFD_OK;
}

extern "C" int ksfd_bench_kernel(ksfd_handle *h, int32_t cls, int32_t reps, double *avg_ms, double *bytes_per_launch)
{
    if (!h || reps < 1 || !avg_ms) return KSFD_EINVAL;
    hipSetDevice(h->device);
    hipEvent_t a, b;
    HIPCHK(h, hipEventCreate(&a));
    HIPCHK(h, hipEventCreate(&b));
    const bool was = h->profiling;
    h->profiling = false;
    int rc = KSFD_OK;
    double by = 0.0;
    auto one = [&]() -> int {
        const double b0 = h->bytes_acc;
        int r = KSFD_OK;
        double coef[KSFD_MAXDOT] = { 0 };
        switch (cls) {
        case KC_RHS: r = op_rhs(h, h->u, -1, h->t3); break;
        case KC_JVP: r = h->use_frozen ? op_jvp_frozen(h, h->Y, 1, 1.0, h->t3) : op_jvp(h, h->u, h->Y, 1, 1.0, h->t3); break;
        case KC_MULTIDOT: {
            Scope sc(h, KC_MULTIDOT, vbytes(h, 9));
            VW_DISPATCH(h, hipLaunchKernelGGL((k_multidot<8, VW>), dim3(vec2(h) ? (h->nblk_vec + 1) / 2 : h->nblk_vec), dim3(KSFD_BLOCK), 0, h->st, h->kv, (const double *)h->t3, (const double *)h->V, h->vlen, 8, h->part));
        } break;
        case KC_GSUPDATE: r = op_gs_update(h, h->t3, h->V, 8, coef, 1.0); break;
        case KC_SPECTRAL: r = spec_apply(h, 10.0, h->Y, h->t3); break;
        case KC_LINCOMB: { const double *xs[3] = { h->u, h->Y, h->Y + h->vlen }; double aa[3] = { 1.0, 0.5, 0.25 }; r = op_lincomb(h, 3, xs, aa, h->t3); } break;
        case KSFD_BENCH_ROTATE: {
            std::vector<double> Pb((size_t)31 * KSFD_ROT_MAXOUT, 0.0);
            for (int j = 0; j < 11; j++) Pb[(size_t)j * KSFD_ROT_MAXOUT + j] = 1.0;
            r = op_basis_rotate(h, h->V, 31, 11, Pb.data(), KSFD_ROT_MAXOUT);
        } break;
        case KSFD_BENCH_ROTATE_COMPOSED: {
            for (int i = 0; i < 31; i++) coef[i] = 1.0 / 31.0;
            for (int j = 0; j < 11 && !r; j++) r = op_basis_axpy(h, h->Zb + (int64_t)j * h->vlen, h->V, 31, coef, 0.0);
        } break;
        default: r = fail(h, KSFD_EINVAL, "bench_kernel: class %d not benchable", cls);
        }
        by = h->bytes_acc - b0;
        return r;
    };
    if ((cls == KSFD_BENCH_ROTATE || cls == KSFD_BENCH_ROTATE_COMPOSED) && (h->restart_alloc < 30 || !h->Zb)) { rc = fail(h, KSFD_EINVAL, "bench_kernel: the rotation benchmark needs 31 basis vectors and the flexible basis"); goto done; }
    if (cls == KSFD_BENCH_ROTATE || cls == KSFD_BENCH_ROTATE_COMPOSED) { h->dr.valid = false; rec_reset(h); }
    if ((rc = halo(h, h->u))) goto done;
    if (h->use_frozen && (cls == KC_JVP || cls == KC_SPECTRAL) && (rc = ensure_coef(h, true))) goto done;
    if (cls == KC_SPECTRAL && (rc = spec_means(h))) goto done;
    for (int i = 0; i < 3 && !rc; i++) rc = one();
    if (rc) goto done;
    hipEventRecord(a, h->st);
    for (int i = 0; i < reps && !rc; i++) rc = one();
    hipEventRecord(b, h->st);
    if (hipEventSynchronize(b) != hipSuccess) rc = fail(h, KSFD_EHIP, "event sync failed");
    if (!rc) {
        float ms = 0.f;
        hipEventElapsedTime(&ms, a, b);
        *avg_ms = ms / reps;
        if (bytes_per_launch) *bytes_per_launch = by;
    }
done:
    h->profiling = was;
    hipEventDestroy(a);
    hipEventDestroy(b);
    return rc;
}
```

### ksfd_amd/csrc/mg_host.hip.h

```cpp
#pragma once
static void mg_free(ksfd_handle *h)
{
    if (h->mg_graph) { hipGraphExecDestroy(h->mg_graph); h->mg_graph = nullptr; }
    for (size_t l = 0; l < h->mg.size(); l++) {
        MGLevel &L = h->mg[l];
        if (L.dinv) hipFree(L.dinv);
        double *bufs[] = { l ? L.coef : nullptr, l ? L.x : nullptr, l ? L.b : nullptr, L.r, L.d, L.Ad, L.dG, L.pv };
        for (double *b : bufs) if (b) hipFree(b);
        float *fb[] = { L.x32, L.b32, L.r32, L.d32, L.coef32 };
        for (float *b : fb) if (b) hipFree(b);
    }
    h->mg.clear();
    h->mg_ok = false;
}

static int mg_build(ksfd_handle *h)
{
    const int dim = h->G.dim;
    int nl = h->P.nlig, F = h->G.F;
    long long nx = h->G.nx, ny = dim == 3 ? h->G.ny : 1, rows = h->G.sloc;
    KPhys P = h->P;
    for (int l = 0;; l++) {
        MGLevel L;
        L.G = h->G; L.G.nx = nx;
// ... 281 lines not shown
static int mg_vcycle(ksfd_handle *h, size_t l, double shift, const double *b, double *x);

static int mg_coarse_correction(ksfd_handle *h, size_t l, double shift, double *x)
{
    int rc;
    MGLevel &L = h->mg[l], &Lc = h->mg[l + 1];
    if ((rc = mg_halo(h, L, L.r, L.G.F))) return rc;
    {
        Scope sc(h, KC_MG, 8.0 * L.G.F * (L.G.nloc + Lc.G.nloc));
        mg_launch_restrict(h, L, Lc, L.G.F, L.r, Lc.b);
    }
    if ((rc = mg_vcycle(h, l + 1, shift, Lc.b, Lc.x))) return rc;
    if ((rc = mg_halo(h, Lc, Lc.x, L.G.F))) return rc;
    {
        Scope sc(h, KC_MG, 8.0 * L.G.F * (2 * L.G.nloc + Lc.G.nloc));
        mg_launch_prolong(h, L, Lc, L.G.F, Lc.x, x);
    }
    HIPCHK(h, hipGetLastError());
    return KSFD_OK;
}

template <typename Body>
static int mg_coarse_graph(ksfd_handle *h, double shift, const void *xkey, bool f32, Body body)
{
    int rc;
    if (!h->mg_graph || h->mg_graph_shift != shift || h->mg_graph_x != xkey || h->mg_graph_f32 != f32) {
        if (h->mg_graph) { hipGraphExecDestroy(h->mg_graph); h->mg_graph = nullptr; }
        hipGraph_t g = nullptr;
        const double b0 = h->bytes_acc;
        HIPCHK(h, hipStreamBeginCapture(h->st, hipStreamCaptureModeThreadLocal));
        h->capturing = true;
        rc = body();
        h->capturing = false;
        hipError_t e = hipStreamEndCapture(h->st, &g);
        if (rc) { if (g) hipGraphDestroy(g); return rc; }
        if (e != hipSuccess || !g) return fail(h, KSFD_EHIP, "hipStreamEndCapture: %s", hipGetErrorString(e));
        e = hipGraphInstantiate(&h->mg_graph, g, nullptr, nullptr, 0);
        hipGraphDestroy(g);
        if (e != hipSuccess) { h->mg_graph = nullptr; return fail(h, KSFD_EHIP, "hipGraphInstantiate: %s", hipGetErrorString(e)); }
        h->mg_graph_bytes = h->bytes_acc - b0;
        h->bytes_acc = b0;
        h->mg_graph_shift = shift;
        h->mg_graph_x = xkey;
        h->mg_graph_f32 = f32;
    }
    Scope sc(h, KC_MG, h->mg_graph_bytes);
    HIPCHK(h, hipGraphLaunch(h->mg_graph, h->st));
    return KSFD_OK;
}

static int mg_vcycle(ksfd_handle *h, size_t l, double shift, const double *b, double *x)
{
    int rc;
    MGLevel &L = h->mg[l];
    if (l + 1 == h->mg.size()) {
        int sweeps = (int)ceil(0.5 * sqrt(L.ratio) * log(2.0 / h->mg_coarse_tol));
        sweeps = std::min(std::max(sweeps, 4), h->mg_ncoarse);
        return mg_smooth(h, L, shift, b, x, sweeps, true, L.ratio);
    }
    if ((rc = mg_smooth(h, L, shift, b, x, h->mg_nu, true, h->mg_ratio))) return rc;
    if ((rc = mg_op(h, L, x, 2, shift, L.r, b))) return rc;
    if (l == 0 && h->mg_use_graph && !h->capturing) {
        if ((rc = mg_coarse_graph(h, shift, x, false, [&]() { return mg_coarse_correction(h, 0, shift, x); }))) return rc;
    } else if ((rc = mg_coarse_correction(h, l, shift, x))) return rc;
    return mg_smooth(h, L, shift, b, x, h->mg_nu, false, h->mg_ratio);
}

static int mg_op32(ksfd_handle *h, MGLevel &L, const float *v, int mode, double shift, float *out, const float *yadd, const KSmoothT<float> *sm)
{
    const KGeom &G = L.G;
    if (h->ring) { int rch = mg_halo32(h, L, const_cast<float *>(v), G.F); if (rch) return rch; }
    const int cls = (&L == &h->mg[0]) ? KC_JVP : KC_MG;
    const float *c32 = (&L == &h->mg[0]) ? (h->poly_fp32 ? h->coef32 : nullptr) : L.coef32;
    const double by = ((c32 ? 4.0 : 8.0) * (3 + h->P.nlig) + 4.0 * G.F + (mode == 2 ? 8.0 * G.F : 12.0 * G.F + 4.0 * G.F * G.F + ((sm && sm->x64) ? 4.0 * G.F : 0.0))) * (double)G.nloc;
    const KStrips K = strips_for(G, h->yseg_jvp, 4096);
    const KSmoothT<float> S = sm ? *sm : KSmoothT<float>{};
    Scope sc(h, cls, by);
    if (sm && c32) {
        NL_DISPATCH(h->P.nlig, if constexpr (NL <= 4) hipLaunchKernelGGL((k_jvp2d_frozen<NL, float, float, float, float, 1, true, float>), dim3(K.nblocks), dim3(KSFD_BLOCK), 0, h->st, G, L.P, K, c32, v, mode, shift, out, yadd, 0.0, 0.0, S));
    } else if (sm) {
        NL_DISPATCH(h->P.nlig, if constexpr (NL <= 4) hipLaunchKernelGGL((k_jvp2d_frozen<NL, double, float, float, float, 1, true, float>), dim3(K.nblocks), dim3(KSFD_BLOCK), 0, h->st, G, L.P, K, (const double *)L.coef, v, mode, shift, out, yadd, 0.0, 0.0, S));
    } else if (c32) {
        NL_DISPATCH(h->P.nlig, if constexpr (NL <= 4) hipLaunchKernelGGL((k_jvp2d_frozen<NL, float, float, float, float>), dim3(K.nblocks), dim3(KSFD_BLOCK), 0, h->st, G, L.P, K, c32, v, mode, shift, out, yadd));
    } else {
        NL_DISPATCH(h->P.nlig, if constexpr (NL <= 4) hipLaunchKernelGGL((k_jvp2d_frozen<NL, double, float, float, float>), dim3(K.nblocks), dim3(KSFD_BLOCK), 0, h->st, G, L.P, K, (const double *)L.coef, v, mode, shift, out, yadd));
    }
    HIPCHK(h, hipGetLastError());
    return KSFD_OK;
}

static int mg_vcycle32(ksfd_handle *h, size_t l, double shift, const double *b64, double *x64);

static int mg_coarse_correction32(ksfd_handle *h, size_t l, double shift)
{
    int rc;
    MGLevel &L = h->mg[l], &Lc = h->mg[l + 1];
    const int F = L.G.F;
    const int nbr = point_blocks(Lc.G);
    const int nbp = point_blocks(L.G);
    if ((rc = mg_halo32(h, L, L.r32, F))) return rc;
    {
        Scope sc(h, KC_MG, F * (4.0 * L.G.nloc + (Lc.f32 ? 4.0 : 8.0) * Lc.G.nloc));
        if (Lc.f32) hipLaunchKernelGGL((k_restrict2d<float, float>), dim3(nbr), dim3(KSFD_BLOCK), 0, h->st, F, L.G.nx, L.G.sloc, L.G.wrap_slow, (const float *)L.r32, L.G.plane, L.kv.off, Lc.b32, Lc.G.plane, Lc.kv.off);
        else hipLaunchKernelGGL((k_restrict2d<float, double>), dim3(nbr), dim3(KSFD_BLOCK), 0, h->st, F, L.G.nx, L.G.sloc, L.G.wrap_slow, (const float *)L.r32, L.G.plane, L.kv.off, Lc.b, Lc.G.plane, Lc.kv.off);
    }
    if (Lc.f32) rc = mg_vcycle32(h, l + 1, shift, nullptr, nullptr);
    else rc = mg_vcycle(h, l + 1, shift, Lc.b, Lc.x);
    if (rc) return rc;
    if ((rc = Lc.f32 ? mg_halo32(h, Lc, Lc.x32, F) : mg_halo(h, Lc, Lc.x, F))) return rc;
    {
        Scope sc(h, KC_MG, F * (8.0 * L.G.nloc + (Lc.f32 ? 4.0 : 8.0) * Lc.G.nloc));
        if (Lc.f32) hipLaunchKernelGGL((k_prolong_add2d<float, float>), dim3(nbp), dim3(KSFD_BLOCK), 0, h->st, F, L.G.nx, L.G.sloc, L.G.wrap_slow, (const float *)Lc.x32, Lc.G.plane, Lc.kv.off, L.x32, L.G.plane, L.kv.off);
        else hipLaunchKernelGGL((k_prolong_add2d<double, float>), dim3(nbp), dim3(KSFD_BLOCK), 0, h->st, F, L.G.nx, L.G.sloc, L.G.wrap_slow, (const double *)Lc.x, Lc.G.plane, Lc.kv.off, L.x32, L.G.plane, L.kv.off);
    }
    HIPCHK(h, hipGetLastError());
    return KSFD_OK;
}

static int mg_vcycle32(ksfd_handle *h, size_t l, double shift, const double *b64, double *x64)
{
    int rc;
    MGLevel &L = h->mg[l];
    const int F = L.G.F;
    const int nb = point_blocks(L.G);
    const double lmax = L.lam_max, lmin = lmax / h->mg_ratio;
    const double theta = 0.5 * (lmax + lmin), delta = 0.5 * (lmax - lmin), sig1 = theta / delta;
    const double rho0 = 1.0 / sig1, rhon = 1.0 / (2.0 * sig1 - rho0);
    const long long off = L.kv.off;
    KSmoothT<float> S = KSmoothT<float>{};
    S.dinv = L.dinv; S.x = L.x32; S.c1 = rhon * rho0; S.c2 = 2.0 * rhon / delta;
    {
        Scope sc(h, KC_MG, ((b64 ? 8.0 + 4.0 : 4.0) * F + 4.0 * F + 4.0 * F * F) * (double)L.G.nloc);
        if (b64) {
            NL_DISPATCH(h->P.nlig, hipLaunchKernelGGL((k_dinv_apply<NL, double, float>), dim3(nb), dim3(KSFD_BLOCK), 0, h->st, L.G.nloc, L.G.plane, (const float *)(L.dinv + off), b64 + off, 1.0 / theta, L.d32 + off, (float *)nullptr, L.b32 + off));
        } else {
            NL_DISPATCH(h->P.nlig, hipLaunchKernelGGL((k_dinv_apply<NL, float, float>), dim3(nb), dim3(KSFD_BLOCK), 0, h->st, L.G.nloc, L.G.plane, (const float *)(L.dinv + off), (const float *)(L.b32 + off), 1.0 / theta, L.d32 + off));
        }
    }
    S.rr = L.b32; S.x_has_d = 1;
    if ((rc = mg_op32(h, L, L.d32, 6, shift, nullptr, nullptr, &S))) return rc;
    if ((rc = mg_op32(h, L, L.x32, 2, shift, L.r32, L.b32, nullptr))) return rc;
    if (l == 0 && h->mg_use_graph && !h->capturing) {
        if ((rc = mg_coarse_graph(h, shift, L.x32, true, [&]() { return mg_coarse_correction32(h, 0, shift); }))) return rc;
    } else if ((rc = mg_coarse_correction32(h, l, shift))) return rc;
    S.out2 = L.d32; S.scale = 1.0 / theta;
    if ((rc = mg_op32(h, L, L.x32, 5, shift, L.r32, L.b32, &S))) return rc;
    S.rr = L.r32; S.x_has_d = 0; S.x64 = x64;
    return mg_op32(h, L, L.d32, 6, shift, nullptr, nullptr, &S);
}

static int mg_precond(ksfd_handle *h, double shift, const double *in, double *out)
{
    int rc;
    if (!h->mg_coef_valid && (rc = mg_restrict_coefs(h))) return rc;
    if (h->mg_shift != shift && (rc = mg_setup_shift(h, shift))) return rc;
    if (h->mg_use32 && h->mg_fp32 && h->mg[0].f32 && h->mg_nu == 2 && mg_can_fuse(h, h->mg[0])) return mg_vcycle32(h, 0, shift, in, out);
    return mg_vcycle(h, 0, shift, in, out);
}
```

### ksfd_amd/csrc/ops.hip.h

```cpp
#pragma once
static int halo(ksfd_handle *h, double *vec)
{
    if (!h->ring) return KSFD_OK;
    Scope sc(h, KC_HALO, 4.0 * 2.0 * 8.0 * h->G.F * (double)h->G.inner * 2.0);
    int rc = h->tr->exchange(vec, h->G.F, h->G.plane, h->G.inner, h->G.sloc, h->G.ng, h->st);
    if (rc) return fail(h, KSFD_ECOMM, "halo exchange failed: %s", h->tr->error().c_str());
    return KSFD_OK;
}

static int spin_for(ksfd_handle *h, unsigned long long seq)
{
    for (unsigned long long spins = 1;; spins++) {
        if (__atomic_load_n(h->pub_flag, __ATOMIC_ACQUIRE) == seq) return KSFD_OK;
        if ((spins & 0xffff) == 0) {
            hipError_t e = hipStreamQuery(h->st);
            if (e == hipSuccess) {
                if (__atomic_load_n(h->pub_flag, __ATOMIC_ACQUIRE) == seq) return KSFD_OK;
                return fail(h, KSFD_EHIP, "reduction finished without publishing its result");
            }
            if (e != hipErrorNotReady) return fail(h, KSFD_EHIP, "stream error while waiting for a reduction: %s", hipGetErrorString(e));
        }
    }
}

// ... 95 lines not shown
{
    static const int env = getenv("KSFD_J3L") ? atoi(getenv("KSFD_J3L")) : 1;
    if (!env || !strip3d_ok(h) || h->P.nlig > 2 || h->G.ny % KSFD_J3L_ROWS) return false;
    if (!h->j3l_attr_set) {
        hipError_t e = hipSuccess;
        if (h->P.nlig == 1) {
            e = hipFuncSetAttribute((const void *)k_jvp3d_lds<1, double>, hipFuncAttributeMaxDynamicSharedMemorySize, (int)ksfd_j3l_lds_bytes<1>());
            if (e == hipSuccess) e = hipFuncSetAttribute((const void *)k_jvp3d_lds<1, float>, hipFuncAttributeMaxDynamicSharedMemorySize, (int)ksfd_j3l_lds_bytes<1>());
        } else {
            e = hipFuncSetAttribute((const void *)k_jvp3d_lds<2, double>, hipFuncAttributeMaxDynamicSharedMemorySize, (int)ksfd_j3l_lds_bytes<2>());
            if (e == hipSuccess) e = hipFuncSetAttribute((const void *)k_jvp3d_lds<2, float>, hipFuncAttributeMaxDynamicSharedMemorySize, (int)ksfd_j3l_lds_bytes<2>());
        }
        h->j3l_attr_set = true;
        h->j3l_usable = e == hipSuccess;
        if (e != hipSuccess) hipGetLastError();
    }
    return h->j3l_usable;
}
static K3D make_k3d_lds(const ksfd_handle *h) { return k3d_for(h->G, KSFD_J3L_ROWS, 0, h->zseg, 1024); }

static inline long long part_capacity() { return (long long)(2 * KSFD_MAXDOT + 4) * 4096; }
static long long strip_waves(const ksfd_handle *h, bool jvp = false) { const KStrips K = make_strips(h, jvp); return (long long)K.nstrips * K.nseg; }
static long long k3d_waves(ksfd_handle *h) { const K3D K = j3l_ok(h) ? make_k3d_lds(h) : make_k3d(h); return (long long)K.nblocks * K.rows; }

template <typename TO>
static void j3l_launch(ksfd_handle *h, const K3D &K, const double *v, int mode, double shift, TO *out, const double *yadd, double alpha, double beta, double *normpart)
{
    const KGeom &G = h->G;
    if (h->P.nlig == 1) hipLaunchKernelGGL((k_jvp3d_lds<1, TO>), dim3(K.nblocks), dim3(KSFD_J3L_ROWS * KSFD_WAVE), ksfd_j3l_lds_bytes<1>(), h->st, G, h->P, K, (const double *)h->coef, v, mode, shift, out, yadd, alpha, beta, normpart);
    else hipLaunchKernelGGL((k_jvp3d_lds<2, TO>), dim3(K.nblocks), dim3(KSFD_J3L_ROWS * KSFD_WAVE), ksfd_j3l_lds_bytes<2>(), h->st, G, h->P, K, (const double *)h->coef, v, mode, shift, out, yadd, alpha, beta, normpart);
}

static KSrc src_of(const ksfd_handle *h, int stage)
{
    KSrc s;
    for (int c = 0; c <= KSFD_MAXL; c++) s.p[c] = (stage >= 0 && c < h->G.F) ? h->src[stage][c] : nullptr;
    return s;
}

static void dg_pass(ksfd_handle *h, const KGeom &G, const double *coef, const double *v, double *dG, int cls = KC_GFIELD)
{
    auto launch = [&] { NL_DISPATCH(h->P.nlig, hipLaunchKernelGGL((k_dg_frozen<NL>), dim3(plane_blocks(G)), dim3(KSFD_BLOCK), 0, h->st, G, coef, v, dG)); };
    if (cls < 0) return launch();
    Scope sc(h, cls, 8.0 * (2 + h->P.nlig + G.F) * (double)G.plane);
    launch();
}

struct JvpBytes { double impl, alg; };
template <typename TC = double, typename TV = double, typename TY = double, typename TO = double>
static JvpBytes jvp_bytes(const KGeom &G, int mode, double ncoef, double extra = 0.0)
{
    const double y = (mode == 2 || mode == 3) ? G.F : 0;
    return { ncoef * sizeof(TC) + G.F * (double)(sizeof(TV) + sizeof(TO)) + y * (double)sizeof(TY) + extra, 8.0 * (3.0 * G.F + y) };
}

template <typename Exchange, typename Launch>
static int with_halo_overlap(ksfd_handle *h, const KStrips &K, double *normpart, Exchange exchange, Launch launch)
{
    int rc;
    const bool ovl = h->overlap && K.nseg >= 3;
    if (ovl) {
        HIPCHK(h, hipEventRecord(h->ev_ready, h->st));
        if ((rc = launch(strips_sub(K, 1, 1, K.nseg - 2), (double)(K.nseg - 2) / K.nseg, normpart))) return rc;
        HIPCHK(h, hipStreamWaitEvent(h->st_comm, h->ev_ready, 0));
    }
    if (exchange(ovl ? h->st_comm : h->st)) return fail(h, KSFD_ECOMM, "halo exchange failed: %s", h->tr->error().c_str());
    if (!ovl) return launch(K, 1.0, normpart);
    HIPCHK(h, hipEventRecord(h->ev_halo, h->st_comm));
    HIPCHK(h, hipStreamWaitEvent(h->st, h->ev_halo, 0));
    return launch(strips_sub(K, 0, K.nseg - 1, 2), 2.0 / K.nseg, normpart ? normpart + (long long)K.nstrips * (K.nseg - 2) : nullptr);
}

static int op_rhs(ksfd_handle *h, const double *u, int stage, double *out, const KComb *cmb = nullptr, bool want_norm = false, double *halo_vec = nullptr,
                  int ndots = 0, const double *dotv = nullptr)
{
    const KGeom &G = h->G;
    KSrc S = src_of(h, stage);
    const KPhys &PP = (stage >= 0 && stage < 4 && h->Pst_valid[stage]) ? h->Pst[stage] : h->P;
    if (!h->ring) halo_vec = nullptr;
    if (fused_ok(h)) {
        KStrips K = make_strips(h);
        KComb C = cmb ? *cmb : KComb{};
        const long long nwaves = strip_waves(h);
        const bool fused_norm = want_norm && nwaves * (1 + ndots) <= part_capacity();
        KDots D = KDots{};
        if (fused_norm && ndots > 0) { D.n = std::min(ndots, 2); D.stride = nwaves; for (int q = 0; q < D.n; q++) D.v[q] = dotv + (int64_t)q * h->vlen; }
        bool carry = h->rhs_carry && C.nout > 0 && C.nout == C.nin;
        for (int j = 0; j < C.nout && carry; j++) carry = C.yin[j] == C.yout[j];
        auto launch = [&](const KStrips &Kx, double frac, double *np) -> int {
            Scope sc(h, KC_RHS, vbytes(h, 2 + C.nin + (carry ? 0 : C.nout) + D.n) * frac, vbytes(h, 2 + C.nin + C.nout + D.n) * frac);
            if (carry) { NL_DISPATCH(h->P.nlig, if constexpr (NL <= 4) hipLaunchKernelGGL((k_rhs2d_fused<NL, true>), dim3(Kx.nblocks), dim3(KSFD_BLOCK), 0, h->st, G, PP, Kx, u, S, out, C, np, D)); }
            else { NL_DISPATCH(h->P.nlig, if constexpr (NL <= 4) hipLaunchKernelGGL((k_rhs2d_fused<NL>), dim3(Kx.nblocks), dim3(KSFD_BLOCK), 0, h->st, G, PP, Kx, u, S, out, C, np, D)); }
            return KSFD_OK;
        };
        double *np = fused_norm ? h->part : (double *)nullptr;
        int rc = !halo_vec ? launch(K, 1.0, np) : with_halo_overlap(h, K, np, [&](hipStream_t st) {
            Scope sc(h, KC_HALO, 4.0 * 2.0 * 8.0 * G.F * (double)G.inner * 2.0);
            return h->tr->exchange(halo_vec, G.F, G.plane, G.inner, G.sloc, G.ng, st);
        }, launch);
        if (rc) return rc;
        HIPCHK(h, hipGetLastError());
        if (fused_norm) return reduce_rows(h, 1 + D.n, (int)nwaves, 0);
        if (want_norm) return fail(h, KSFD_EINVAL, "op_rhs: fused norm needs the strip kernels");
        return KSFD_OK;
    }
    if (halo_vec) { int rc = halo(h, halo_vec); if (rc) return rc; }
    if (strip3d_ok(h) && h->rhs3d_strip) {
        if (want_norm) return fail(h, KSFD_EINVAL, "op_rhs: fused norm is a 2-D feature");
        KComb C = cmb ? *cmb : KComb{};
        const double *uin = u;
        const double *Gplane = h->Gb;
        const bool reuse_G = C.nin == 0 && u == h->u && h->coef_fresh && h->use_frozen && h->coef && &PP == &h->P;
        if (reuse_G) Gplane = h->coef + G.plane;
        else {
            Scope sc(h, KC_GFIELD, 8.0 * ((1 + C.nin) * G.F + (C.nin ? G.F : 0) + 1) * (double)G.plane, C.nin ? vbytes(h, 2 + C.nin) : 0.0);
            NL_DISPATCH(h->P.nlig, if constexpr (NL <= 4) hipLaunchKernelGGL((k_gfield_comb<NL>), dim3(plane_blocks(G)), dim3(KSFD_BLOCK), 0, h->st, G, PP, u, C, C.nin ? h->Z : (double *)nullptr, h->Gb));
        }
        if (C.nin) uin = h->Z;
        K3D K = make_k3d(h);
        Scope sc(h, KC_RHS, 8.0 * (2.0 * G.F + 1 + C.nout * G.F) * (double)G.nloc, vbytes(h, 2 + C.nout));
        if (K.rows == 8) hipLaunchKernelGGL((k_rhs3d_strip<1, 8>), dim3(K.nblocks), dim3(8 * KSFD_WAVE), 0, h->st, G, PP, K, uin, Gplane, S, out, C);
        else NL_DISPATCH(h->P.nlig, if constexpr (NL <= 4) hipLaunchKernelGGL((k_rhs3d_strip<NL>), dim3(K.nblocks), dim3(KSFD_BLOCK), 0, h->st, G, PP, K, uin, Gplane, S, out, C));
    } else {
        {
            Scope sc(h, KC_GFIELD, 8.0 * (G.F + 1) * (double)G.plane);
            NL_DISPATCH(h->P.nlig, hipLaunchKernelGGL((k_gfield<NL, false>), dim3(plane_blocks(G)), dim3(KSFD_BLOCK), 0, h->st, G, PP, u, (const double *)nullptr, h->Gb, (double *)nullptr));
        }
        Scope sc(h, KC_RHS, vbytes(h, 2) + 8.0 * (double)G.nloc, vbytes(h, 2));
        NL_DISPATCH(h->P.nlig, hipLaunchKernelGGL((k_rhs_generic<NL>), dim3(point_blocks(G)), dim3(KSFD_BLOCK), 0, h->st, G, PP, u, h->Gb, S, out));
    }
    HIPCHK(h, hipGetLastError());
    return KSFD_OK;
}

static int op_jvp(ksfd_handle *h, const double *u, const double *v, int mode, double shift, double *out)
{
    const KGeom &G = h->G;
    if (fused_ok(h)) {
        KStrips K = make_strips(h, true);
        Scope sc(h, KC_JVP, vbytes(h, 3));
        NL_DISPATCH(h->P.nlig, if constexpr (NL <= 4) hipLaunchKernelGGL((k_jvp2d_fused<NL>), dim3(K.nblocks), dim3(KSFD_BLOCK), 0, h->st, G, h->P, K, u, v, mode, shift, out));
    } else {
        {
            Scope sc(h, KC_GFIELD, 8.0 * (2 * G.F + 2) * (double)G.plane);
            NL_DISPATCH(h->P.nlig, hipLaunchKernelGGL((k_gfield<NL, true>), dim3(plane_blocks(G)), dim3(KSFD_BLOCK), 0, h->st, G, h->P, u, v, h->Gb, h->dGb));
        }
        Scope sc(h, KC_JVP, vbytes(h, 3) + 16.0 * (double)G.nloc, vbytes(h, 3));
        NL_DISPATCH(h->P.nlig, hipLaunchKernelGGL((k_jvp_generic<NL>), dim3(point_blocks(G)), dim3(KSFD_BLOCK), 0, h->st, G, h->P, u, v, h->Gb, h->dGb, mode, shift, out));
    }
    HIPCHK(h, hipGetLastError());
    return KSFD_OK;
}

static int op_jcoef(ksfd_handle *h, const double *u, bool want_means = false)
{
    const KGeom &G = h->G;
    const int nbp = plane_blocks(G);
    if (!h->coef32 && h->poly_fp32 && fused_ok(h) && h->P.nlig <= 4 && G.plane % 2 == 0 && G.inner % 2 == 0 &&
        hipMalloc((void **)&h->coef32, sizeof(float) * (size_t)(3 + h->P.nlig) * G.plane) != hipSuccess) { h->coef32 = nullptr; h->poly_fp32 = false; }
    float *c32 = h->poly_fp32 ? h->coef32 : nullptr;
    want_means = want_means && (long long)(1 + h->P.nlig) * nbp <= part_capacity();
    {
    Scope sc(h, KC_GFIELD, (8.0 * (G.F + 3 + h->P.nlig) + (c32 ? 4.0 * (3 + h->P.nlig) : 0.0)) * (double)G.plane);
    NL_DISPATCH(h->P.nlig, hipLaunchKernelGGL((k_jcoef<NL>), dim3(nbp), dim3(KSFD_BLOCK), 0, h->st, G, h->P, u, h->coef, c32, want_means ? h->part : (double *)nullptr));
    }
    HIPCHK(h, hipGetLastError());
    if (want_means) {
        int rc = reduce_rows(h, 1 + h->P.nlig, nbp, 0);
        if (rc) return rc;
        const double ntot = (double)h->cfg.n[0] * (double)h->cfg.n[1] * (double)h->cfg.n[2];
        h->spec.a_rr = h->hres[0] / ntot;
        for (int l = 0; l < h->P.nlig; l++) h->spec.a_rU[l] = h->hres[1 + l] / ntot;
    }
    return KSFD_OK;
}

static int ensure_coef(ksfd_handle *h, bool ghosts_done = false)
{
    if (h->coef_fresh) return KSFD_OK;
    int rc;
    if (!ghosts_done && (rc = halo(h, h->u))) return rc;
    if ((rc = op_jcoef(h, h->u, h->spec.ok))) return rc;
    h->coef_fresh = true;
    h->mg_coef_valid = false; h->mg_shift = -1.0;
    h->spec.means_valid = h->spec.ok && (long long)(1 + h->P.nlig) * plane_blocks(h->G) <= part_capacity();
    return KSFD_OK;
}

static int op_jvp_frozen(ksfd_handle *h, const double *v, int mode, double shift, double *out,
                         const double *yadd = nullptr, double alpha = 0.0, double beta = 0.0, bool want_norm = false)
{
    const KGeom &G = h->G;
    const JvpBytes B = jvp_bytes(G, mode, 3 + h->P.nlig), Bdg = jvp_bytes(G, mode, 3);
    if (fused_ok(h)) {
        KStrips K = make_strips(h, true);
        const long long nwaves = strip_waves(h, true);
        if (want_norm && nwaves > part_capacity()) return fail(h, KSFD_EINVAL, "op_jvp_frozen: too many waves for the fused norm");
        {
            Scope sc(h, KC_JVP, B.impl * (double)G.nloc, B.alg * (double)G.nloc);
            NL_DISPATCH(h->P.nlig, if constexpr (NL <= 4) hipLaunchKernelGGL((k_jvp2d_frozen<NL>), dim3(K.nblocks), dim3(KSFD_BLOCK), 0, h->st, G, h->P, K, (const double *)h->coef, v, mode, shift, out, yadd, alpha, beta, KSmooth{}, want_norm ? h->part : (double *)nullptr));
        }
        HIPCHK(h, hipGetLastError());
        return want_norm ? reduce_rows(h, 1, (int)nwaves, 0) : KSFD_OK;
    } else if (!want_norm && j3l_ok(h)) {
        K3D K = make_k3d_lds(h);
        Scope sc(h, KC_JVP, B.impl * (double)G.nloc, B.alg * (double)G.nloc);
        j3l_launch<double>(h, K, v, mode, shift, out, yadd, alpha, beta, nullptr);
    } else if (h->use_fused && G.dim == 3 && (G.nx % 2 == 0) && G.nx >= 4 && h->P.nlig <= 4) {
        dg_pass(h, G, h->coef, v, h->dGb);
        K3D K = make_k3d(h);
        Scope sc(h, KC_JVP, Bdg.impl * (double)G.nloc, Bdg.alg * (double)G.nloc);
        if (K.rows == 8) hipLaunchKernelGGL((k_jvp3d_frozen<1, double, 8>), dim3(K.nblocks), dim3(8 * KSFD_WAVE), 0, h->st, G, h->P, K, (const double *)h->coef, v, (const double *)h->dGb, mode, shift, out, yadd, alpha, beta);
        else NL_DISPATCH(h->P.nlig, if constexpr (NL <= 4) hipLaunchKernelGGL((k_jvp3d_frozen<NL>), dim3(K.nblocks), dim3(KSFD_BLOCK), 0, h->st, G, h->P, K, (const double *)h->coef, v, (const double *)h->dGb, mode, shift, out, yadd, alpha, beta));
    } else {
        dg_pass(h, G, h->coef, v, h->dGb);
        Scope sc(h, KC_JVP, Bdg.impl * (double)G.nloc, Bdg.alg * (double)G.nloc);
        NL_DISPATCH(h->P.nlig, hipLaunchKernelGGL((k_jvp_generic<NL>), dim3(point_blocks(G)), dim3(KSFD_BLOCK), 0, h->st, G, h->P, (const double *)h->coef, v, (const double *)(h->coef + G.plane), (const double *)h->dGb, mode, shift, out, yadd, alpha, beta));
    }
    HIPCHK(h, hipGetLastError());
    return KSFD_OK;
}

template <typename TC, typename TV, typename TY, typename TO>
static int jvp2d_launch_t(ksfd_handle *h, const KStrips &K, double frac, const TC *C, const TV *v, int mode, double shift,
                          TO *out, const TY *yadd, double alpha, double beta, double *normpart = nullptr)
{
    const KGeom &G = h->G;
    const JvpBytes B = jvp_bytes<TC, TV, TY, TO>(G, mode, 3 + h->P.nlig);
    Scope sc(h, KC_JVP, B.impl * (double)G.nloc * frac, B.alg * (double)G.nloc * frac);
    NL_DISPATCH(h->P.nlig, if constexpr (NL <= 4) hipLaunchKernelGGL((k_jvp2d_frozen<NL, TC, TV, TY, TO>), dim3(K.nblocks), dim3(KSFD_BLOCK), 0, h->st,
                                                                     G, h->P, K, C, (const TV *)v, mode, shift, out, yadd, alpha, beta, KSmooth{}, normpart));
    HIPCHK(h, hipGetLastError());
    return KSFD_OK;
}

template <typename TC, typename TV, typename TY, typename TO>
static int jvp2d_halo_t(ksfd_handle *h, const TC *C, TV *v, int mode, double shift, TO *out, const TY *yadd, double alpha, double beta, double *normpart = nullptr)
{
    const KGeom &G = h->G;
    auto launch = [&](const KStrips &Kx, double frac, double *np) { return jvp2d_launch_t(h, Kx, frac, C, v, mode, shift, out, yadd, alpha, beta, np); };
    if (!h->ring) return launch(make_strips(h, true), 1.0, normpart);
    const long long scale = sizeof(double) / sizeof(TV);
    return with_halo_overlap(h, make_strips(h, true), normpart, [&](hipStream_t st) {
        Scope sc(h, KC_HALO, 4.0 * 2.0 * sizeof(TV) * G.F * (double)G.inner * 2.0);
        return h->tr->exchange(reinterpret_cast<double *>(v), G.F, G.plane / scale, G.inner / scale, G.sloc, G.ng, st);
    }, launch);
}

static int op_jvp_frozen_halo(ksfd_handle *h, double *v, int mode, double shift, double *out,
                              const double *yadd = nullptr, double alpha = 0.0, double beta = 0.0)
{
    if (!h->ring) return op_jvp_frozen(h, v, mode, shift, out, yadd, alpha, beta);
    if (!h->overlap || !fused_ok(h) || make_strips(h, true).nseg < 3 || h->P.nlig > 4) {
        const int rc = halo(h, v);
        return rc ? rc : op_jvp_frozen(h, v, mode, shift, out, yadd, alpha, beta);
    }
    return jvp2d_halo_t<double, double, double, double>(h, (const double *)h->coef, v, mode, shift, out, yadd, alpha, beta);
}

static int op_residual32(ksfd_handle *h, const double *x, double shift, const double *b, float *r32)
{
    const KGeom &G = h->G;
    const long long nwaves = G.dim == 3 ? k3d_waves(h) : strip_waves(h, true);
    if (G.dim == 3) {
        const bool j3l = j3l_ok(h);
        if (!j3l) dg_pass(h, G, h->coef, x, h->dGb);
        if (nwaves > part_capacity()) return fail(h, KSFD_EINVAL, "op_residual32: too many waves for the fused norm");
        const JvpBytes B = j3l ? jvp_bytes<double, double, double, float>(G, 2, 3 + h->P.nlig, 8.0 * G.F) : jvp_bytes<double, double, double, float>(G, 2, 3);
        const K3D K = j3l ? make_k3d_lds(h) : make_k3d(h);
        {
            Scope sc(h, KC_JVP, B.impl * (double)G.nloc, B.alg * (double)G.nloc);
            if (j3l) j3l_launch<float>(h, K, x, 2, shift, r32, b, 0.0, 0.0, h->part);
            else if (K.rows == 8) hipLaunchKernelGGL((k_jvp3d_frozen<1, float, 8>), dim3(K.nblocks), dim3(8 * KSFD_WAVE), 0, h->st, G, h->P, K, (const double *)h->coef, x, (const double *)h->dGb, 2, shift, r32, b, 0.0, 0.0, h->part);
            else NL_DISPATCH(h->P.nlig, if constexpr (NL <= 4) hipLaunchKernelGGL((k_jvp3d_frozen<NL, float>), dim3(K.nblocks), dim3(KSFD_BLOCK), 0, h->st, G, h->P, K, (const double *)h->coef, x, (const double *)h->dGb, 2, shift, r32, b, 0.0, 0.0, h->part));
        }
        HIPCHK(h, hipGetLastError());
        return reduce_rows(h, 1, (int)nwaves, 0);
    }
    if (nwaves > part_capacity()) return fail(h, KSFD_EINVAL, "op_residual32: too many waves for the fused norm");
    int rc = jvp2d_halo_t<double, double, double, float>(h, (const double *)h->coef, const_cast<double *>(x), 2, shift, r32, b, 0.0, 0.0, h->part);
    if (rc) return rc;
    return reduce_rows(h, 1, (int)nwaves, 0);
}

static inline bool vec2(const ksfd_handle *h) { return (h->G.nloc % 2 == 0) && (h->kv.off % 2 == 0) && (h->G.plane % 2 == 0); }
static inline dim3 vgridw(const ksfd_handle *h, int vw) { return dim3((h->nblk_vec + vw - 1) / vw, h->G.F); }
#define VW_DISPATCH(h, CALL) do { if (vec2(h)) { constexpr int VW = 2; CALL; } else { constexpr int VW = 1; CALL; } } while (0)
#define KB_DISPATCH(k, CALL)                                                                       \
    do {                                                                                           \
        if ((k) <= 4) { constexpr int KB = 4; CALL; }                                              \
        else if ((k) <= 8) { constexpr int KB = 8; CALL; }                                         \
        else if ((k) <= 16) { constexpr int KB = 16; CALL; }                                       \
        else { constexpr int KB = 32; CALL; }                                                      \
    } while (0)
#define NT_DISPATCH(nt, CALL)                                                                      \
    switch (nt) {                                                                                  \
    case 1: { constexpr int NT = 1; CALL; } break;                                                 \
    case 2: { constexpr int NT = 2; CALL; } break;                                                 \
    case 3: { constexpr int NT = 3; CALL; } break;                                                 \
    case 4: { constexpr int NT = 4; CALL; } break;                                                 \
    case 5: { constexpr int NT = 5; CALL; } break;                                                 \
    default: { constexpr int NT = 6; CALL; } break;                                                \
    }

static int op_lincomb(ksfd_handle *h, int nt, const double *const *x, const double *a, double *out, bool want_norm = false)
{
    double *part = want_norm ? h->part : nullptr;
    KLin L;
    for (int t = 0; t < 6; t++) { L.x[t] = t < nt ? x[t] : nullptr; L.a[t] = t < nt ? a[t] : 0.0; }
    Scope sc(h, KC_LINCOMB, vbytes(h, nt + 1));
    NT_DISPATCH(nt, VW_DISPATCH(h, hipLaunchKernelGGL((k_lincomb<NT, VW>), vgridw(h, VW), dim3(KSFD_BLOCK), 0, h->st, h->kv, L, out, part)));
    HIPCHK(h, hipGetLastError());
    if (want_norm) { const dim3 gr = vgridw(h, vec2(h) ? 2 : 1); return reduce_rows(h, 1, (int)(gr.x * gr.y), 0); }
    return KSFD_OK;
}

static int op_multidot(ksfd_handle *h, const double *w, const double *V, int k)
{
    if (k > 32) {
        std::vector<double> acc((size_t)k + 1);
        for (int c0 = 0; c0 < k; c0 += 32) {
            const int kc = std::min(32, k - c0);
            int rc = op_multidot(h, w, V + (int64_t)c0 * h->vlen, kc);
            if (rc) return rc;
            for (int i = 0; i < kc; i++) acc[c0 + i] = h->hres[i];
            acc[k] = h->hres[kc];
        }
        if (k + 1 > 128) return fail(h, KSFD_EINVAL, "op_multidot: %d vectors exceed the result buffer", k);
        for (int i = 0; i <= k; i++) h->hres[i] = acc[i];
        return KSFD_OK;
    }
    const int nb = vec2(h) ? (h->nblk_vec + 1) / 2 : h->nblk_vec;
    {
        Scope sc(h, KC_MULTIDOT, vbytes(h, k + 1));
        KB_DISPATCH(k, VW_DISPATCH(h, hipLaunchKernelGGL((k_multidot<KB, VW>), dim3(nb), dim3(KSFD_BLOCK), 0, h->st, h->kv, w, V, h->vlen, k, h->part)));
    }
    HIPCHK(h, hipGetLastError());
    return reduce_rows(h, k + 1, nb, 0);
// ... 107 lines not shown
```

### ksfd_amd/csrc/pointwise.hip.h

```cpp
#pragma once
#include <hip/hip_runtime.h>
#include "params.h"

#define KSFD_WAVE 64
#define KSFD_BLOCK 256
#define KSFD_MAXDOT 34

__device__ __forceinline__ double ksfd_clamp(double x, double lo) { return !(x >= lo) ? lo : x; }

__device__ __forceinline__ double ksfd_rcp(double x)
{
    double r = __builtin_amdgcn_rcp(x);
    r = fma(fma(-x, r, 1.0), r, r);
    r = fma(fma(-x, r, 1.0), r, r);
    return r;
}
__device__ __forceinline__ double ksfd_div(double a, double x)
{
    const double r = ksfd_rcp(x);
    const double q = a * r;
    return fma(fma(-x, q, a), r, q);
}
__device__ __forceinline__ double ksfd_log(double x)
{
// ... 94 lines not shown
__device__ __forceinline__ void kset(double2 &v, int e, double x) { if (e) v.y = x; else v.x = x; }
template <int VW> __device__ __forceinline__ typename KPack<VW>::T kload(const double *p)
{
    return *reinterpret_cast<const typename KPack<VW>::T *>(p);
}
template <int VW> __device__ __forceinline__ void kstore(double *p, const typename KPack<VW>::T &v)
{
    *reinterpret_cast<typename KPack<VW>::T *>(p) = v;
}

__device__ __forceinline__ void ksfd_block_sum_to(double v, double *dst)
{
    __shared__ double red_[KSFD_BLOCK / KSFD_WAVE];
    v = ksfd_wave_sum(v);
    if ((threadIdx.x & (KSFD_WAVE - 1)) == 0) red_[threadIdx.x / KSFD_WAVE] = v;
    __syncthreads();
    if (threadIdx.x == 0) {
        double t = 0.0;
        for (int q = 0; q < KSFD_BLOCK / KSFD_WAVE; q++) t += red_[q];
        *dst = t;
    }
}

struct KLin {
    const double *x[6];
    double a[6];
};
template <int NT, int VW>
__global__ void __launch_bounds__(KSFD_BLOCK) k_lincomb(KVec g, KLin L, double *out, double *part = nullptr)
{
    const long long base = (long long)blockIdx.y * g.plane + g.off;
    const long long stride = (long long)gridDim.x * blockDim.x * VW;
    double nrm = 0.0;
    for (long long p = ((long long)blockIdx.x * blockDim.x + threadIdx.x) * VW; p < g.nloc; p += stride) {
        typename KPack<VW>::T s, xv;
#pragma unroll
        for (int e = 0; e < VW; e++) kset(s, e, 0.0);
#pragma unroll
        for (int t = 0; t < NT; t++) {
            xv = kload<VW>(L.x[t] + base + p);
#pragma unroll
            for (int e = 0; e < VW; e++) kset(s, e, kget(s, e) + L.a[t] * kget(xv, e));
        }
        kstore<VW>(out + base + p, s);
#pragma unroll
        for (int e = 0; e < VW; e++) nrm += kget(s, e) * kget(s, e);
    }
    if (part) ksfd_block_sum_to(nrm, part + (long long)blockIdx.y * gridDim.x + blockIdx.x);
}

template <int KMAX, int VW>
__global__ void __launch_bounds__(KSFD_BLOCK) k_multidot(KVec g, const double *__restrict__ w,
                                                         const double *__restrict__ V, long long vstride,
                                                         int k, double *__restrict__ part)
{
    __shared__ double red[KSFD_BLOCK / KSFD_WAVE][KMAX + 1];
    double acc[KMAX + 1];
#pragma unroll
    for (int i = 0; i <= KMAX; i++) acc[i] = 0.0;
    const long long stride = (long long)gridDim.x * blockDim.x * VW;
    for (int c = 0; c < g.nf; c++) {
        const long long base = (long long)c * g.plane + g.off;
        for (long long p = ((long long)blockIdx.x * blockDim.x + threadIdx.x) * VW; p < g.nloc; p += stride) {
            const typename KPack<VW>::T wv = kload<VW>(w + base + p);
#pragma unroll
            for (int i = 0; i < KMAX; i++)
                if (i < k) {
                    const typename KPack<VW>::T vv = kload<VW>(V + (long long)i * vstride + base + p);
#pragma unroll
                    for (int e = 0; e < VW; e++) acc[i] += kget(wv, e) * kget(vv, e);
                }
#pragma unroll
            for (int e = 0; e < VW; e++) acc[KMAX] += kget(wv, e) * kget(wv, e);
        }
    }
    const int lane = threadIdx.x & (KSFD_WAVE - 1), wv_ = threadIdx.x / KSFD_WAVE;
#pragma unroll
    for (int i = 0; i <= KMAX; i++) {
        if (i < k || i == KMAX) {
            double s = ksfd_wave_sum(acc[i]);
            if (lane == 0) red[wv_][i] = s;
        }
    }
    __syncthreads();
    if (threadIdx.x <= KMAX) {
        int i = threadIdx.x;
        if (i < k || i == KMAX) {
            double s = 0.0;
            for (int q = 0; q < KSFD_BLOCK / KSFD_WAVE; q++) s += red[q][i];
            int row = (i == KMAX) ? k : i;
            part[(long long)row * gridDim.x + blockIdx.x] = s;
        }
    }
}

template <int KMAX, int VW>
__global__ void __launch_bounds__(KSFD_BLOCK) k_multidot_gram(KVec g, const double *__restrict__ w,
                                                              const double *__restrict__ V, long long vstride,
                                                              int k, double *__restrict__ part)
{
    __shared__ double red[KSFD_BLOCK / KSFD_WAVE][2 * KMAX + 1];
    double acc[2 * KMAX + 1];
#pragma unroll
    for (int i = 0; i <= 2 * KMAX; i++) acc[i] = 0.0;
    const long long stride = (long long)gridDim.x * blockDim.x * VW;
    for (int c = 0; c < g.nf; c++) {
        const long long base = (long long)c * g.plane + g.off;
        for (long long p = ((long long)blockIdx.x * blockDim.x + threadIdx.x) * VW; p < g.nloc; p += stride) {
            const typename KPack<VW>::T wv = kload<VW>(w + base + p);
            const typename KPack<VW>::T lv = kload<VW>(V + (long long)(k - 1) * vstride + base + p);
#pragma unroll
            for (int i = 0; i < KMAX; i++)
                if (i < k) {
                    const typename KPack<VW>::T vv = (i == k - 1) ? lv : kload<VW>(V + (long long)i * vstride + base + p);
#pragma unroll
                    for (int e = 0; e < VW; e++) {
                        acc[i] += kget(wv, e) * kget(vv, e);
                        acc[KMAX + i] += kget(lv, e) * kget(vv, e);
                    }
                }
#pragma unroll
            for (int e = 0; e < VW; e++) acc[2 * KMAX] += kget(wv, e) * kget(wv, e);
        }
    }
    const int lane = threadIdx.x & (KSFD_WAVE - 1), wv_ = threadIdx.x / KSFD_WAVE;
#pragma unroll
    for (int i = 0; i <= 2 * KMAX; i++) {
        const bool live = (i < k) || (i >= KMAX && i < KMAX + k) || (i == 2 * KMAX);
        if (live) {
            double s = ksfd_wave_sum(acc[i]);
            if (lane == 0) red[wv_][i] = s;
        }
    }
    __syncthreads();
    if (threadIdx.x <= 2 * KMAX) {
        const int i = threadIdx.x;
        const bool live = (i < k) || (i >= KMAX && i < KMAX + k) || (i == 2 * KMAX);
        if (live) {
            double s = 0.0;
            for (int q = 0; q < KSFD_BLOCK / KSFD_WAVE; q++) s += red[q][i];
            const int row = (i == 2 * KMAX) ? 2 * k : (i >= KMAX ? k + (i - KMAX) : i);
            part[(long long)row * gridDim.x + blockIdx.x] = s;
        }
    }
}

__global__ void __launch_bounds__(KSFD_BLOCK) k_reduce_rows(const double *__restrict__ part, int nblk, int op,
                                                            double *__restrict__ out, double *pub = nullptr,
                                                            unsigned int *count = nullptr, unsigned long long *flag = nullptr,
                                                            unsigned long long seq = 0)
{
    __shared__ double red[KSFD_BLOCK / KSFD_WAVE];
    const double *row = part + (long long)blockIdx.x * nblk;
    double s = op ? -1.0e300 : 0.0;
    for (int b0 = threadIdx.x; b0 < nblk; b0 += 8 * blockDim.x) {
        double t[8];
#pragma unroll
        for (int q = 0; q < 8; q++) { const int b = b0 + q * blockDim.x; t[q] = b < nblk ? row[b] : (op ? -1.0e300 : 0.0); }
#pragma unroll
        for (int q = 0; q < 8; q++) s = op ? fmax(s, t[q]) : s + t[q];
    }
    s = op ? ksfd_wave_max(s) : ksfd_wave_sum(s);
    if ((threadIdx.x & (KSFD_WAVE - 1)) == 0) red[threadIdx.x / KSFD_WAVE] = s;
    __syncthreads();
    if (threadIdx.x == 0) {
        double t = red[0];
        for (int q = 1; q < KSFD_BLOCK / KSFD_WAVE; q++) t = op ? fmax(t, red[q]) : t + red[q];
        out[blockIdx.x] = t;
        if (pub) {
            __hip_atomic_store(pub + blockIdx.x, t, __ATOMIC_RELAXED, __HIP_MEMORY_SCOPE_SYSTEM);
            __threadfence_system();
            if (atomicAdd(count, 1u) == gridDim.x - 1) {
                *count = 0;
                __threadfence_system();
                __hip_atomic_store(flag, seq, __ATOMIC_RELEASE, __HIP_MEMORY_SCOPE_SYSTEM);
            }
        }
    }
}

__global__ void k_publish(const double *__restrict__ res, int n, double *pub, unsigned long long *flag, unsigned long long seq)
{
    if (threadIdx.x < n) __hip_atomic_store(pub + threadIdx.x, res[threadIdx.x], __ATOMIC_RELAXED, __HIP_MEMORY_SCOPE_SYSTEM);
    __threadfence_system();
    __syncthreads();
    if (threadIdx.x == 0) __hip_atomic_store(flag, seq, __ATOMIC_RELEASE, __HIP_MEMORY_SCOPE_SYSTEM);
}

struct KCoef {
    double h[KSFD_MAXDOT];
};
template <int KMAX, int VW>
__global__ void __launch_bounds__(KSFD_BLOCK) k_gs_update(KVec g, double *__restrict__ w,
                                                          const double *__restrict__ V, long long vstride, int k,
                                                          KCoef C, double scale)
{
    const long long base = (long long)blockIdx.y * g.plane + g.off;
    const long long stride = (long long)gridDim.x * blockDim.x * VW;
    for (long long p = ((long long)blockIdx.x * blockDim.x + threadIdx.x) * VW; p < g.nloc; p += stride) {
        typename KPack<VW>::T s = kload<VW>(w + base + p);
#pragma unroll
        for (int i = 0; i < KMAX; i++)
            if (i < k) {
                const typename KPack<VW>::T vv = kload<VW>(V + (long long)i * vstride + base + p);
#pragma unroll
                for (int e = 0; e < VW; e++) kset(s, e, kget(s, e) - C.h[i] * kget(vv, e));
            }
#pragma unroll
        for (int e = 0; e < VW; e++) kset(s, e, kget(s, e) * scale);
        kstore<VW>(w + base + p, s);
    }
}

template <int KMAX, int VW>
__global__ void __launch_bounds__(KSFD_BLOCK) k_basis_axpy(KVec g, double *__restrict__ x,
                                                           const double *__restrict__ V, long long vstride, int k,
                                                           KCoef C, double beta, double *part = nullptr)
{
    const long long base = (long long)blockIdx.y * g.plane + g.off;
    const long long stride = (long long)gridDim.x * blockDim.x * VW;
    double nrm = 0.0;
    for (long long p = ((long long)blockIdx.x * blockDim.x + threadIdx.x) * VW; p < g.nloc; p += stride) {
        typename KPack<VW>::T s;
        if (beta == 0.0) {
#pragma unroll
            for (int e = 0; e < VW; e++) kset(s, e, 0.0);
        } else {
            s = kload<VW>(x + base + p);
#pragma unroll
            for (int e = 0; e < VW; e++) kset(s, e, beta * kget(s, e));
        }
#pragma unroll
        for (int i = 0; i < KMAX; i++)
            if (i < k && C.h[i] != 0.0) {
                const typename KPack<VW>::T vv = kload<VW>(V + (long long)i * vstride + base + p);
#pragma unroll
                for (int e = 0; e < VW; e++) kset(s, e, kget(s, e) + C.h[i] * kget(vv, e));
            }
        kstore<VW>(x + base + p, s);
#pragma unroll
        for (int e = 0; e < VW; e++) nrm += kget(s, e) * kget(s, e);
    }
    if (part) ksfd_block_sum_to(nrm, part + (long long)blockIdx.y * gridDim.x + blockIdx.x);
}

#define KSFD_ROT_MAXIN 121
#define KSFD_ROT_MAXOUT 18
template <int NOUT, int VW>
__global__ void __launch_bounds__(KSFD_BLOCK) k_basis_rotate(KVec g, double *V, long long vstride, int nin, int nout,
                                                             const double *__restrict__ P, int ldp)
{
    __shared__ double sP[KSFD_ROT_MAXIN * NOUT];
    for (int q = threadIdx.x; q < nin * NOUT; q += blockDim.x) {
        const int i = q / NOUT, j = q - i * NOUT;
        sP[q] = j < nout ? P[i * ldp + j] : 0.0;
    }
    __syncthreads();
    const long long base = (long long)blockIdx.y * g.plane + g.off;
    const long long stride = (long long)gridDim.x * blockDim.x * VW;
    for (long long p = ((long long)blockIdx.x * blockDim.x + threadIdx.x) * VW; p < g.nloc; p += stride) {
        double acc[NOUT][VW];
#pragma unroll
        for (int j = 0; j < NOUT; j++)
#pragma unroll
            for (int e = 0; e < VW; e++) acc[j][e] = 0.0;
        const double *src = V + base + p;
#pragma unroll 4
        for (int i = 0; i < nin; i++) {
            const typename KPack<VW>::T vv = kload<VW>(src + (long long)i * vstride);
            const double *row = sP + i * NOUT;
#pragma unroll
            for (int j = 0; j < NOUT; j++) {
                const double c = row[j];
#pragma unroll
                for (int e = 0; e < VW; e++) acc[j][e] = fma(c, kget(vv, e), acc[j][e]);
            }
        }
#pragma unroll
        for (int j = 0; j < NOUT; j++)
            if (j < nout) {
                typename KPack<VW>::T s;
#pragma unroll
                for (int e = 0; e < VW; e++) kset(s, e, acc[j][e]);
                kstore<VW>(V + (long long)j * vstride + base + p, s);
            }
    }
}

__global__ void __launch_bounds__(KSFD_BLOCK) k_rosw_finish(KVec g, double *__restrict__ u,
                                                            const double *__restrict__ Y, long long ystride,
                                                            double bt0, double bt1, double bt2, double bt3,
                                                            double e0, double e1, double e2, double e3,
                                                            double atol, double rtol, double *__restrict__ errout,
                                                            double *__restrict__ part)
{
    __shared__ double red[KSFD_BLOCK / KSFD_WAVE];
    double acc = 0.0;
    const long long stride = (long long)gridDim.x * blockDim.x;
    for (int c = 0; c < g.nf; c++) {
        const long long base = (long long)c * g.plane + g.off;
        for (long long p = (long long)blockIdx.x * blockDim.x + threadIdx.x; p < g.nloc; p += stride) {
            const double y0 = Y[base + p], y1 = Y[ystride + base + p], y2 = Y[2 * ystride + base + p],
                         y3 = Y[3 * ystride + base + p];
            const double un = u[base + p] + (bt0 * y0 + bt1 * y1 + bt2 * y2 + bt3 * y3);
            const double er = e0 * y0 + e1 * y1 + e2 * y2 + e3 * y3;
            const double tol = atol + rtol * fmax(fabs(un), fabs(un + er));
            const double q = er / tol;
            acc += q * q;
            u[base + p] = un;
            if (errout) errout[base + p] = er;
        }
    }
    acc = ksfd_wave_sum(acc);
    if ((threadIdx.x & (KSFD_WAVE - 1)) == 0) red[threadIdx.x / KSFD_WAVE] = acc;
    __syncthreads();
    if (threadIdx.x == 0) {
        double t = 0.0;
        for (int q = 0; q < KSFD_BLOCK / KSFD_WAVE; q++) t += red[q];
        part[blockIdx.x] = t;
    }
// ... 143 lines not shown
```

### ksfd_amd/csrc/stencil.hip.h

```cpp
#pragma once
#include <type_traits>
#include "pointwise.hip.h"

struct KSrc {
    const double *p[KSFD_MAXL + 1];
};

struct KComb {
    int nin, nout;
    const double *yin[3], *yout[3];
    double ain[3], aout[3];
};

struct KDots {
    int n;
    long long stride;
    const double *v[2];
};

template <typename TS = double>
struct KSmoothT {
    const float *dinv;
    const TS *rr;
    TS *x, *out2;
// ... 443 lines not shown
};
__device__ __forceinline__ KWaveJob ksfd_wave_job(const KGeom &G, const KStrips &S)
{
    KWaveJob J;
    const int lane = threadIdx.x & (KSFD_WAVE - 1);
    const long long wid = (long long)ksfd_xcd_remap(blockIdx.x, S.nblocks) * (KSFD_BLOCK / KSFD_WAVE) + (threadIdx.x >> 6);
    J.wid = wid;
    J.valid = wid < (long long)S.nstrips * S.nseg;
    const int strip = (int)(wid % S.nstrips);
    const long long seg = S.seg0 + (wid / S.nstrips) * S.seg_stride;
    const long long half = G.nx >> 1;
    const long long xs = 2 * ((long long)strip * half / S.nstrips);
    const long long xe = 2 * ((long long)(strip + 1) * half / S.nstrips);
    long long c = xs - 2 + 2 * lane;
    c %= G.nx;
    if (c < 0) c += G.nx;
    J.c0 = c;
    J.store = lane >= 1 && lane <= (int)((xe - xs) >> 1);
    J.r0 = seg * S.yseg;
    J.r1 = J.r0 + S.yseg < G.sloc ? J.r0 + S.yseg : G.sloc;
    J.up = (seg & 1) == 0;
    return J;
}

template <int NL, bool CARRY = false>
__global__ void __launch_bounds__(KSFD_BLOCK) k_rhs2d_fused(KGeom G, KPhys P, KStrips S, const double *__restrict__ u,
                                                            KSrc src, double *__restrict__ out, KComb cmb = KComb{},
                                                            double *__restrict__ normpart = nullptr, KDots dots = KDots{})
{
    const KWaveJob J = ksfd_wave_job(G, S);
    if (!J.valid) return;
    double nacc = 0.0, dacc[2] = { 0.0, 0.0 };
    double rw[5][2], gw[5][2], uw[NL][5][2];
    double nr[2], nu[NL][2];
    __shared__ double2 cring[CARRY ? KSFD_BLOCK / KSFD_WAVE : 1][CARRY ? 4 : 1][CARRY ? NL + 1 : 1][CARRY ? KSFD_WAVE : 1];
    const int cw = CARRY ? (threadIdx.x >> 6) : 0, cl = CARRY ? (threadIdx.x & (KSFD_WAVE - 1)) : 0;
    int nload = 0;

    auto load_row = [&](long long r) {
        const long long o = ksfd_rowoff(G, r) + J.c0;
        double2 t = ksfd_ld2(u + o);
        nr[0] = t.x; nr[1] = t.y;
#pragma unroll
        for (int l = 0; l < NL; l++) {
            double2 q = ksfd_ld2(u + (long long)(l + 1) * G.plane + o);
            nu[l][0] = q.x; nu[l][1] = q.y;
        }
        double2 co[NL + 1];
#pragma unroll
        for (int c = 0; c <= NL; c++) co[c] = make_double2(0.0, 0.0);
        for (int j = 0; j < cmb.nin; j++) {
            const double a = cmb.ain[j], ao = CARRY ? cmb.aout[j] : 0.0;
            double2 y = ksfd_ld2(cmb.yin[j] + o);
            nr[0] += a * y.x; nr[1] += a * y.y;
            if (CARRY) { co[0].x += ao * y.x; co[0].y += ao * y.y; }
#pragma unroll
            for (int l = 0; l < NL; l++) {
                double2 q = ksfd_ld2(cmb.yin[j] + (long long)(l + 1) * G.plane + o);
                nu[l][0] += a * q.x; nu[l][1] += a * q.y;
                if (CARRY) { co[l + 1].x += ao * q.x; co[l + 1].y += ao * q.y; }
            }
        }
        if (CARRY) {
#pragma unroll
            for (int c = 0; c <= NL; c++) cring[cw][nload & 3][c][cl] = co[c];
        }
        nload++;
    };
    auto push_row = [&]() {
#pragma unroll
        for (int s = 0; s < 4; s++) {
#pragma unroll
            for (int e = 0; e < 2; e++) {
                rw[s][e] = rw[s + 1][e];
                gw[s][e] = gw[s + 1][e];
#pragma unroll
                for (int l = 0; l < NL; l++) uw[l][s][e] = uw[l][s + 1][e];
            }
        }
#pragma unroll
        for (int e = 0; e < 2; e++) {
            double U[NL], GU[NL], gr;
            double rho = ksfd_clamp(nr[e], P.rhomin);
#pragma unroll
            for (int l = 0; l < NL; l++) { U[l] = ksfd_clamp(nu[l][e], P.Umin); uw[l][4][e] = U[l]; }
            ksfd_G<NL, false>(P, rho, U, gw[4][e], gr, GU);
            rw[4][e] = rho;
        }
    };

    for (int q = -2; q <= 1; q++) { load_row(J.row(J.r0 + q)); push_row(); }
    load_row(J.row(J.r0 + 2));
    for (long long r = J.r0; r < J.r1; r++) {
        push_row();
        if (r + 1 < J.r1) load_row(J.row(r + 3));
        const KX xr = ksfd_xnb(rw[2][0], rw[2][1]);
        const KX xg = ksfd_xnb(gw[2][0], gw[2][1]);
        double d1rx[2], d1gx[2], d2gx[2];
        ksfd_dx(rw[2][0], rw[2][1], xr, d1rx[0], d1rx[1]);
        ksfd_dx(gw[2][0], gw[2][1], xg, d1gx[0], d1gx[1]);
        ksfd_dxx(gw[2][0], gw[2][1], xg, d2gx[0], d2gx[1]);
        double res[NL + 1][2];
#pragma unroll
        for (int e = 0; e < 2; e++) {
            const double d1ry = KSFD_D1(rw[0][e], rw[1][e], rw[3][e], rw[4][e]) * P.inv_h[1];
            const double d1gy = KSFD_D1(gw[0][e], gw[1][e], gw[3][e], gw[4][e]) * P.inv_h[1];
            const double d2gy = KSFD_D2(gw[0][e], gw[1][e], gw[2][e], gw[3][e], gw[4][e]) * P.inv_h2[1];
            res[0][e] = (d1rx[e] * P.inv_h[0]) * (d1gx[e] * P.inv_h[0]) + d1ry * d1gy +
                        rw[2][e] * (d2gx[e] * P.inv_h2[0] + d2gy);
        }
#pragma unroll
        for (int l = 0; l < NL; l++) {
            const KX xu = ksfd_xnb(uw[l][2][0], uw[l][2][1]);
            double d2ux[2];
            ksfd_dxx(uw[l][2][0], uw[l][2][1], xu, d2ux[0], d2ux[1]);
#pragma unroll
            for (int e = 0; e < 2; e++) {
                const double d2uy = KSFD_D2(uw[l][0][e], uw[l][1][e], uw[l][2][e], uw[l][3][e], uw[l][4][e]) * P.inv_h2[1];
                res[l + 1][e] = -P.lig_gamma[l] * uw[l][2][e] + P.lig_s[l] * rw[2][e] +
                                P.lig_D[l] * (d2ux[e] * P.inv_h2[0] + d2uy);
            }
        }
        if (J.store) {
            const long long pi = J.row(r) * G.nx + J.c0;
            const long long o = (long long)G.ng * G.inner + pi;
#pragma unroll
            for (int c = 0; c <= NL; c++) {
                double a = res[c][0], b = res[c][1];
                if (src.p[c]) { double2 s = ksfd_ld2(src.p[c] + pi); a += s.x; b += s.y; }
                if (CARRY) { const double2 cc = cring[cw][(int)(r - J.r0 + 2) & 3][c][cl]; a += cc.x; b += cc.y; }
                else for (int j = 0; j < cmb.nout; j++) {
                    const double2 y = ksfd_ld2(cmb.yout[j] + (long long)c * G.plane + o);
                    a += cmb.aout[j] * y.x; b += cmb.aout[j] * y.y;
                }
                ksfd_st2(out + (long long)c * G.plane + o, a, b);
                nacc += a * a + b * b;
#pragma unroll
                for (int q = 0; q < 2; q++)
                    if (q < dots.n) { const double2 y = ksfd_ld2(dots.v[q] + (long long)c * G.plane + o); dacc[q] += a * y.x + b * y.y; }
            }
        }
    }
    if (normpart) {
        nacc = ksfd_wave_sum(nacc);
        if ((threadIdx.x & (KSFD_WAVE - 1)) == 0) normpart[J.wid] = nacc;
        for (int q = 0; q < dots.n; q++) {
            const double t = ksfd_wave_sum(dacc[q]);
            if ((threadIdx.x & (KSFD_WAVE - 1)) == 0) normpart[(long long)(1 + q) * dots.stride + J.wid] = t;
        }
    }
}

template <int NL>
__global__ void __launch_bounds__(KSFD_BLOCK) k_jvp2d_fused(KGeom G, KPhys P, KStrips S, const double *__restrict__ u,
                                                            const double *__restrict__ v, int mode, double shift,
                                                            double *__restrict__ out)
{
    const KWaveJob J = ksfd_wave_job(G, S);
    if (!J.valid) return;
    double rw[5][2], gw[5][2], vw[5][2], ew[5][2], zw[NL][5][2];
    double nr[2], nv[2], nu[NL][2], nz[NL][2];

    auto load_row = [&](long long r) {
        const long long o = ksfd_rowoff(G, r) + J.c0;
        double2 t = ksfd_ld2(u + o), w = ksfd_ld2(v + o);
        nr[0] = t.x; nr[1] = t.y; nv[0] = w.x; nv[1] = w.y;
#pragma unroll
        for (int l = 0; l < NL; l++) {
            double2 q = ksfd_ld2(u + (long long)(l + 1) * G.plane + o);
            double2 z = ksfd_ld2(v + (long long)(l + 1) * G.plane + o);
            nu[l][0] = q.x; nu[l][1] = q.y; nz[l][0] = z.x; nz[l][1] = z.y;
        }
    };
    auto push_row = [&]() {
#pragma unroll
        for (int s = 0; s < 4; s++) {
#pragma unroll
            for (int e = 0; e < 2; e++) {
                rw[s][e] = rw[s + 1][e]; gw[s][e] = gw[s + 1][e];
                vw[s][e] = vw[s + 1][e]; ew[s][e] = ew[s + 1][e];
#pragma unroll
                for (int l = 0; l < NL; l++) zw[l][s][e] = zw[l][s + 1][e];
            }
        }
#pragma unroll
        for (int e = 0; e < 2; e++) {
            double U[NL], GU[NL], gr;
            double rho = ksfd_clamp(nr[e], P.rhomin);
#pragma unroll
            for (int l = 0; l < NL; l++) U[l] = ksfd_clamp(nu[l][e], P.Umin);
            ksfd_G<NL, true>(P, rho, U, gw[4][e], gr, GU);
            double d = gr * nv[e];
#pragma unroll
            for (int l = 0; l < NL; l++) { d += GU[l] * nz[l][e]; zw[l][4][e] = nz[l][e]; }
            rw[4][e] = rho; vw[4][e] = nv[e]; ew[4][e] = d;
        }
    };

    for (int q = -2; q <= 1; q++) { load_row(J.row(J.r0 + q)); push_row(); }
    load_row(J.row(J.r0 + 2));
    for (long long r = J.r0; r < J.r1; r++) {
        push_row();
        if (r + 1 < J.r1) load_row(J.row(r + 3));
        const KX xr = ksfd_xnb(rw[2][0], rw[2][1]);
        const KX xg = ksfd_xnb(gw[2][0], gw[2][1]);
        const KX xv = ksfd_xnb(vw[2][0], vw[2][1]);
        const KX xe = ksfd_xnb(ew[2][0], ew[2][1]);
        double d1r[2], d1g[2], d1v[2], d1e[2], d2g[2], d2e[2];
        ksfd_dx(rw[2][0], rw[2][1], xr, d1r[0], d1r[1]);
        ksfd_dx(gw[2][0], gw[2][1], xg, d1g[0], d1g[1]);
        ksfd_dx(vw[2][0], vw[2][1], xv, d1v[0], d1v[1]);
        ksfd_dx(ew[2][0], ew[2][1], xe, d1e[0], d1e[1]);
        ksfd_dxx(gw[2][0], gw[2][1], xg, d2g[0], d2g[1]);
        ksfd_dxx(ew[2][0], ew[2][1], xe, d2e[0], d2e[1]);
        double res[NL + 1][2];
#pragma unroll
        for (int e = 0; e < 2; e++) {
            const double ih0 = P.inv_h[0], ih1 = P.inv_h[1];
            const double yr = KSFD_D1(rw[0][e], rw[1][e], rw[3][e], rw[4][e]) * ih1;
            const double yg = KSFD_D1(gw[0][e], gw[1][e], gw[3][e], gw[4][e]) * ih1;
            const double yv = KSFD_D1(vw[0][e], vw[1][e], vw[3][e], vw[4][e]) * ih1;
            const double ye = KSFD_D1(ew[0][e], ew[1][e], ew[3][e], ew[4][e]) * ih1;
            const double lapG = d2g[e] * P.inv_h2[0] + KSFD_D2(gw[0][e], gw[1][e], gw[2][e], gw[3][e], gw[4][e]) * P.inv_h2[1];
            const double lapE = d2e[e] * P.inv_h2[0] + KSFD_D2(ew[0][e], ew[1][e], ew[2][e], ew[3][e], ew[4][e]) * P.inv_h2[1];
            const double jr = (d1v[e] * ih0) * (d1g[e] * ih0) + (d1r[e] * ih0) * (d1e[e] * ih0) + yv * yg + yr * ye +
                              vw[2][e] * lapG + rw[2][e] * lapE;
            res[0][e] = mode ? shift * vw[2][e] - jr : jr;
        }
#pragma unroll
        for (int l = 0; l < NL; l++) {
            const KX xz = ksfd_xnb(zw[l][2][0], zw[l][2][1]);
            double d2z[2];
            ksfd_dxx(zw[l][2][0], zw[l][2][1], xz, d2z[0], d2z[1]);
#pragma unroll
            for (int e = 0; e < 2; e++) {
                const double lap = d2z[e] * P.inv_h2[0] +
                                   KSFD_D2(zw[l][0][e], zw[l][1][e], zw[l][2][e], zw[l][3][e], zw[l][4][e]) * P.inv_h2[1];
                const double ju = -P.lig_gamma[l] * zw[l][2][e] + P.lig_s[l] * vw[2][e] + P.lig_D[l] * lap;
                res[l + 1][e] = mode ? shift * zw[l][2][e] - ju : ju;
            }
        }
        if (J.store) {
            const long long o = (long long)G.ng * G.inner + J.row(r) * G.nx + J.c0;
#pragma unroll
            for (int c = 0; c <= NL; c++) ksfd_st2(out + (long long)c * G.plane + o, res[c][0], res[c][1]);
        }
    }
}

__global__ void __launch_bounds__(KSFD_BLOCK) k_velmax2d(KGeom G, KPhys P, const double *__restrict__ Gb, double *__restrict__ part)
{
    __shared__ double red[KSFD_BLOCK / KSFD_WAVE][2];
    double mx = 0.0, my = 0.0;
    const long long half = G.nx >> 1;
    const long long pc = (long long)blockIdx.x * blockDim.x + threadIdx.x;
    if (pc < half) {
        const long long x = 2 * pc;
        const long long xl = x >= 2 ? x - 2 : G.nx - 2, xr = x + 2 < G.nx ? x + 2 : 0;
        for (long long r = blockIdx.y; r < G.sloc; r += gridDim.y) {
            const double *row = Gb + ksfd_rowoff(G, r);
            const double2 c = ksfd_ld2(row + x), l = ksfd_ld2(row + xl), rr = ksfd_ld2(row + xr);
            const double2 m2 = ksfd_ld2(Gb + ksfd_rowoff(G, r - 2) + x), m1 = ksfd_ld2(Gb + ksfd_rowoff(G, r - 1) + x),
                          p1 = ksfd_ld2(Gb + ksfd_rowoff(G, r + 1) + x), p2 = ksfd_ld2(Gb + ksfd_rowoff(G, r + 2) + x);
            mx = fmax(mx, fmax(fabs(KSFD_D1(l.x, l.y, c.y, rr.x)), fabs(KSFD_D1(l.y, c.x, rr.x, rr.y))));
            my = fmax(my, fmax(fabs(KSFD_D1(m2.x, m1.x, p1.x, p2.x)), fabs(KSFD_D1(m2.y, m1.y, p1.y, p2.y))));
        }
    }
    mx = ksfd_wave_max(mx * P.inv_h[0]);
    my = ksfd_wave_max(my * P.inv_h[1]);
    if ((threadIdx.x & (KSFD_WAVE - 1)) == 0) { red[threadIdx.x / KSFD_WAVE][0] = mx; red[threadIdx.x / KSFD_WAVE][1] = my; }
    __syncthreads();
    if (threadIdx.x < 3) {
        double m = 0.0;
        if (threadIdx.x < 2) for (int q = 0; q < KSFD_BLOCK / KSFD_WAVE; q++) m = fmax(m, red[q][threadIdx.x]);
        const long long nb = (long long)gridDim.x * gridDim.y;
        part[(long long)threadIdx.x * nb + (long long)blockIdx.y * gridDim.x + blockIdx.x] = m;
    }
}

__global__ void __launch_bounds__(KSFD_BLOCK) k_velmax3d(KGeom G, KPhys P, int zseg, const double *__restrict__ Gb, double *__restrict__ part)
{
    __shared__ double red[KSFD_BLOCK / KSFD_WAVE][3];
    double mx = 0.0, my = 0.0, mz = 0.0;
    const int half = (int)(G.nx >> 1), ny = (int)G.ny, nx = (int)G.nx;
    const int t = blockIdx.x * blockDim.x + threadIdx.x;
    if (t < half * ny) {
        const int y = t / half, x = 2 * (t - y * half);
        const int xl = x >= 2 ? x - 2 : nx - 2, xr = x + 2 < nx ? x + 2 : 0;
        const int ym2 = y >= 2 ? y - 2 : y - 2 + ny, ym1 = y >= 1 ? y - 1 : ny - 1, yp1 = y + 1 < ny ? y + 1 : 0, yp2 = y + 2 < ny ? y + 2 : y + 2 - ny;
        auto zoff = [&](int k) -> long long {
            if (G.wrap_slow) { if (k < 0) k += (int)G.sloc; else if (k >= (int)G.sloc) k -= (int)G.sloc; return (long long)k * G.inner; }
            return (long long)(k + G.ng) * G.inner;
        };
        const int z0 = blockIdx.y * zseg, z1 = min(z0 + zseg, (int)G.sloc);
        const long long yo = (long long)y * nx + x;
        double2 m2 = ksfd_ld2(Gb + zoff(z0 - 2) + yo), m1 = ksfd_ld2(Gb + zoff(z0 - 1) + yo), c = ksfd_ld2(Gb + zoff(z0) + yo), p1 = ksfd_ld2(Gb + zoff(z0 + 1) + yo);
#pragma unroll 4
        for (int z = z0; z < z1; z++) {
            const double *pl = Gb + zoff(z);
            const double2 p2 = ksfd_ld2(Gb + zoff(z + 2) + yo);
            const double2 l = ksfd_ld2(pl + (long long)y * nx + xl), rr = ksfd_ld2(pl + (long long)y * nx + xr);
            const double2 a2 = ksfd_ld2(pl + (long long)ym2 * nx + x), a1 = ksfd_ld2(pl + (long long)ym1 * nx + x),
                          b1 = ksfd_ld2(pl + (long long)yp1 * nx + x), b2 = ksfd_ld2(pl + (long long)yp2 * nx + x);
            mx = fmax(mx, fmax(fabs(KSFD_D1(l.x, l.y, c.y, rr.x)), fabs(KSFD_D1(l.y, c.x, rr.x, rr.y))));
            my = fmax(my, fmax(fabs(KSFD_D1(a2.x, a1.x, b1.x, b2.x)), fabs(KSFD_D1(a2.y, a1.y, b1.y, b2.y))));
            mz = fmax(mz, fmax(fabs(KSFD_D1(m2.x, m1.x, p1.x, p2.x)), fabs(KSFD_D1(m2.y, m1.y, p1.y, p2.y))));
// ... 768 lines not shown
```

Measured before the change: 1.808 billion.

## Fuse step-head coefficient build, velocity max, means and first RHS into one kernel

Adds k_rhs2d_head, which at the start of a step computes the frozen Jacobian coefficients (fp64 and optional fp32), the stage-0 RHS with its norm, the spectral means and the per-axis velocity maxima in one sweep. The stage loop then reuses that stage-0 RHS instead of recomputing it. The fp32 coefficient copy is produced lazily through a separate conversion kernel only when polynomial or multigrid paths need it, and many state-change points invalidate the cached RHS. The aim is fewer passes over the state and fewer launches and host syncs per step, at the cost of extra validity-tracking state that must be invalidated correctly.

Measured after the change: 1.847 billion, median of 6. 1.02x the previous value.

```diff
diff --git a/ksfd_amd/csrc/handle.hip.h b/ksfd_amd/csrc/handle.hip.h
--- a/ksfd_amd/csrc/handle.hip.h
+++ b/ksfd_amd/csrc/handle.hip.h
@@ -107,6 +107,11 @@
     double *coef = nullptr;
     bool use_frozen = true;
     bool coef_fresh = false;
+    bool step_head = true;
+    bool b0_fresh = false;
+    double *b0_dst = nullptr, *b0_hint = nullptr;
+    double b0_norm2 = 0.0;
+    bool coef32_fresh = false, coef32_want = false;
     double *flat = nullptr;
     double *src[4][KSFD_MAXL + 1];
     double *part = nullptr;
@@ -323,6 +328,8 @@
     return KSFD_OK;
 }
 
+static inline void state_changed(ksfd_handle *h) { h->coef_fresh = false; h->b0_fresh = false; }
+
 static bool fused_ok(const ksfd_handle *h)
 {
     return h->use_fused && h->G.dim == 2 && (h->G.nx % 2 == 0) && h->G.nx >= 4 && h->G.sloc >= 4 && h->P.nlig <= 4;
diff --git a/ksfd_amd/csrc/krylov.hip.h b/ksfd_amd/csrc/krylov.hip.h
--- a/ksfd_amd/csrc/krylov.hip.h
+++ b/ksfd_amd/csrc/krylov.hip.h
@@ -56,6 +56,7 @@
     int rc;
     const int d = h->poly_deg;
     const double *al = h->poly_alpha;
+    if ((rc = ensure_coef32(h))) return rc;
     if (h->poly_fp32 && h->coef32 && fused_ok(h)) {
         const float *C = h->coef32;
         float *tf[2] = { reinterpret_cast<float *>(h->t1), reinterpret_cast<float *>(h->t2) };
diff --git a/ksfd_amd/csrc/ksfd_hip.hip b/ksfd_amd/csrc/ksfd_hip.hip
--- a/ksfd_amd/csrc/ksfd_hip.hip
+++ b/ksfd_amd/csrc/ksfd_hip.hip
@@ -216,13 +216,14 @@
     h->cfg = *cfg;
     h->cfg.lig_group = nullptr; h->cfg.lig_w = h->cfg.lig_s = h->cfg.lig_gamma = h->cfg.lig_D = nullptr;
     h->cfg.grp_alpha = h->cfg.grp_beta = nullptr;
-    h->coef_fresh = false;
+    state_changed(h);
     return fill_phys(h, cfg);
 }
 
 extern "C" int ksfd_set_stage_params(ksfd_handle *h, int32_t stage, const ksfd_config *cfg)
 {
     if (!h || stage < -1 || stage > 3) return KSFD_EINVAL;
+    h->b0_fresh = false;
     if (!cfg) {
         for (int s = 0; s < 4; s++) if (stage == -1 || s == stage) h->Pst_valid[s] = false;
         return KSFD_OK;
@@ -255,7 +256,7 @@
     if (!h || !u) return KSFD_EINVAL;
     hipSetDevice(h->device);
     int rc = upload(h, u, layout, h->u);
-    h->coef_fresh = false;
+    state_changed(h);
     if (rc) return rc;
     HIPCHK(h, hipStreamSynchronize(h->st));
     return KSFD_OK;
@@ -320,7 +321,7 @@
     }
     if (!h->ckpt_valid) return fail(h, KSFD_EINVAL, "no checkpoint has been saved");
     HIPCHK(h, hipMemcpyAsync(h->u, h->ckpt, sizeof(double) * (size_t)h->vlen, hipMemcpyDeviceToDevice, h->st));
-    h->coef_fresh = false;
+    state_changed(h);
     const ksfd_handle::SolverMemo &m = h->ckpt_memo;
     h->lamJ = m.lamJ; h->lam_age = m.lam_age; h->lam_period = m.lam_period; h->mg_shift_floor = m.mg_shift_floor;
     h->sf_dir = m.sf_dir; h->sf_hold = m.sf_hold; h->sf_tried_down = m.sf_tried_down; h->sf_prev_its = m.sf_prev_its; h->sf_prev_floor = m.sf_prev_floor;
@@ -342,7 +343,7 @@
         n *= nc[a];
     }
     double *dz = nullptr;
-    h->coef_fresh = false;
+    state_changed(h);
     if (hipMalloc((void **)&dz, sizeof(double) * (size_t)n) != hipSuccess) return fail(h, KSFD_ENOMEM, "hipMalloc of the coarse samples failed");
     hipError_t e = hipMemcpyAsync(dz, z, sizeof(double) * (size_t)n, hipMemcpyHostToDevice, h->st);
     const KGeom &G = h->G;
@@ -370,6 +371,7 @@
     if (!h || field < 0 || field >= h->G.F || stage < -1 || stage > 3) return h ? fail(h, KSFD_EINVAL, "bad stage/field") : KSFD_EINVAL;
     if (layout != KSFD_LAYOUT_SOA) return fail(h, KSFD_EINVAL, "sources are single dense planes: pass layout SOA");
     hipSetDevice(h->device);
+    h->b0_fresh = false;
     for (int s = 0; s < 4; s++) {
         if (stage != -1 && s != stage) continue;
         if (!srch) {
@@ -418,6 +420,7 @@
     int rc;
     const double *Gplane = h->Gb;
     if (uin == h->u && h->use_frozen) {
+        if (vmax && !vel_dev && !h->coef_fresh && step_head_ok(h)) return op_step_head(h, vmax);
         if ((rc = ensure_coef(h))) return rc;
         Gplane = h->coef + G.plane;
     } else {
@@ -502,7 +505,7 @@
 {
     if (!h) return KSFD_EINVAL;
     hipSetDevice(h->device);
-    h->coef_fresh = false;
+    state_changed(h);
     Scope sc(h, KC_MISC, 16.0 * (double)h->G.nloc);
     hipLaunchKernelGGL(k_mul_rho, dim3(h->nblk_vec), dim3(KSFD_BLOCK), 0, h->st, h->kv, h->u, (const double *)nullptr, factor);
     HIPCHK(h, hipGetLastError());
@@ -514,7 +517,7 @@
     if (!h || !fh) return KSFD_EINVAL;
     hipSetDevice(h->device);
     HIPCHK(h, hipMemcpyAsync(h->flat, fh, sizeof(double) * (size_t)h->G.nloc, hipMemcpyHostToDevice, h->st));
-    h->coef_fresh = false;
+    state_changed(h);
     Scope sc(h, KC_MISC, 24.0 * (double)h->G.nloc);
     hipLaunchKernelGGL(k_mul_rho, dim3(h->nblk_vec), dim3(KSFD_BLOCK), 0, h->st, h->kv, h->u, (const double *)h->flat, 1.0);
     HIPCHK(h, hipGetLastError());
@@ -611,6 +614,7 @@
     double hh = *hstep;
     bool prev_accept = !(opts->reserved & 4);
     bool lam_done = false;
+    bool b0_kept = false;
     int rejects = 0;
     const int max_rej = opts->max_reject < 0 ? 0x7fffffff : opts->max_reject;
     const bool single = (opts->reserved & 2) != 0;
@@ -637,6 +641,12 @@
         if (use_spec) {
             if (!h->Zb && alloc_d(h, &h->Zb, (int64_t)h->restart_alloc * h->vlen)) { rc = KSFD_ENOMEM; goto out; }
             if (!h->spec.means_valid && (rc = spec_means(h))) goto out;
+            static const bool means_trace = getenv("KSFD_STAGE_TRACE") != nullptr;
+            if (means_trace) {
+                fprintf(stderr, "[means] a_rr %a -> %a", h->spec.a_rr, (double)(float)h->spec.a_rr);
+                for (int l = 0; l < h->P.nlig; l++) fprintf(stderr, " a_rU%d %a -> %a", l, h->spec.a_rU[l], (double)(float)h->spec.a_rU[l]);
+                fprintf(stderr, "\n");
+            }
         }
         const bool use_pc = !direct && !use_spec && h->mg_ok && h->use_frozen && (opts->pc_type == 1 || (opts->pc_type == 2 && stiff > mg_from));
         bool use_poly = false;
@@ -681,9 +691,13 @@
                 const int gdot_j0 = std::max(0, i - h->guess_max), gdot_n = (guess_on && i > 0 && h->rhs_dots) ? i - gdot_j0 : 0;
                 const bool rhs_norm = use_spec && fused_ok(h) && (!(guess_on && i > 0) || (gdot_n > 0 && gdot_n <= 2 && strip_waves(h) * (1 + gdot_n) <= part_capacity()));
                 rhs_dots_done = rhs_norm && gdot_n > 0;
-                if ((rc = op_rhs(h, h->u, i, bcur, &cmb, rhs_norm, i > 0 ? h->Y + (int64_t)(i - 1) * vs : nullptr, rhs_dots_done ? gdot_n : 0,
+                if (i == 0) h->b0_hint = bcur;
+                const bool b0_there = i == 0 && h->b0_fresh && h->b0_dst == bcur;
+                if (i > 0 && bcur == h->b0_dst) h->b0_fresh = false;
+                if (b0_there) { if (rhs_norm) bnorm2 = h->b0_norm2; }
+                else if ((rc = op_rhs(h, h->u, i, bcur, &cmb, rhs_norm, i > 0 ? h->Y + (int64_t)(i - 1) * vs : nullptr, rhs_dots_done ? gdot_n : 0,
                                  rhs_dots_done ? h->bstore + (int64_t)gdot_j0 * vs : nullptr))) break;
-                if (rhs_norm) bnorm2 = h->hres[0];
+                if (rhs_norm && !b0_there) bnorm2 = h->hres[0];
                 if (rhs_dots_done) for (int j = 0; j < gdot_n; j++) rhs_dot[j] = h->hres[1 + j];
             } else {
             if (i > 0) {
@@ -696,6 +710,7 @@
                     zin = h->Z;
                 }
             }
+            if (h->bvec == h->b0_dst) h->b0_fresh = false;
             if ((rc = op_rhs(h, zin, i, h->bvec))) break;
             if (i > 0) {
                 const double *xs[5]; double a[5]; int nt = 0;
@@ -833,7 +848,8 @@
                                h->b2t[2] - h->bt[2], h->b2t[3] - h->bt[3], opts->atol, opts->rtol, h->errv, h->part);
         }
         h->have_err = true;
-        h->coef_fresh = false;
+        b0_kept = h->b0_fresh;
+        state_changed(h);
         if ((rc = reduce_rows(h, 1, h->nblk_vec, 0))) goto out;
         {
             double ntot = (double)h->G.F * (double)h->cfg.n[0] * (double)h->cfg.n[1] * (double)h->cfg.n[2];
@@ -841,7 +857,7 @@
         }
         if (!(st.wrms == st.wrms) || isinf(st.wrms)) {
             op_copy(h, h->u, h->usave); hipStreamSynchronize(h->st);
-            h->coef_fresh = h->use_frozen;
+            h->coef_fresh = h->use_frozen; h->b0_fresh = b0_kept;
             rc = fail(h, KSFD_ENAN, "non-finite error norm at t=%g h=%g", *t, hh);
             goto out;
         }
@@ -867,7 +883,7 @@
         rejects++;
         st.rejections = rejects;
         if ((rc = op_copy(h, h->u, h->usave))) goto out;
-        h->coef_fresh = h->use_frozen;
+        h->coef_fresh = h->use_frozen; h->b0_fresh = b0_kept;
         hh = hnext;
         *hstep = hnext;
         if (single) break;
@@ -1033,10 +1049,12 @@
         h->mg_fp32 = !(use_fused & 524288);
         h->rec_mg = (use_fused & 1048576) != 0;
         h->rhs_dots = !(use_fused & 2097152);
+        h->step_head = !(use_fused & 4194304);
         if (h->mg_fuse != !(use_fused & 4096)) { h->mg_fuse = !(use_fused & 4096); h->mg_shift = -1.0; if (h->mg_graph) { hipGraphExecDestroy(h->mg_graph); h->mg_graph = nullptr; } }
     }
     if (yseg > 0) h->yseg = yseg;
     if (yseg_jvp > 0) h->yseg_jvp = yseg_jvp;
+    h->b0_fresh = false;
     return KSFD_OK;
 }
 
diff --git a/ksfd_amd/csrc/mg_host.hip.h b/ksfd_amd/csrc/mg_host.hip.h
--- a/ksfd_amd/csrc/mg_host.hip.h
+++ b/ksfd_amd/csrc/mg_host.hip.h
@@ -457,6 +457,7 @@
 static int mg_precond(ksfd_handle *h, double shift, const double *in, double *out)
 {
     int rc;
+    if ((rc = ensure_coef32(h))) return rc;
     if (!h->mg_coef_valid && (rc = mg_restrict_coefs(h))) return rc;
     if (h->mg_shift != shift && (rc = mg_setup_shift(h, shift))) return rc;
     if (h->mg_use32 && h->mg_fp32 && h->mg[0].f32 && h->mg_nu == 2 && mg_can_fuse(h, h->mg[0])) return mg_vcycle32(h, 0, shift, in, out);
diff --git a/ksfd_amd/csrc/ops.hip.h b/ksfd_amd/csrc/ops.hip.h
--- a/ksfd_amd/csrc/ops.hip.h
+++ b/ksfd_amd/csrc/ops.hip.h
@@ -271,13 +271,39 @@
     return KSFD_OK;
 }
 
+static bool coef32_alloc(ksfd_handle *h)
+{
+    const KGeom &G = h->G;
+    if (!h->poly_fp32 || !fused_ok(h) || h->P.nlig > 4 || G.plane % 2 || G.inner % 2) return false;
+    if (!h->coef32 && hipMalloc((void **)&h->coef32, sizeof(float) * (size_t)(3 + h->P.nlig) * G.plane) != hipSuccess) { (void)hipGetLastError(); h->coef32 = nullptr; h->poly_fp32 = false; }
+    return h->coef32 != nullptr;
+}
+static float *coef32_take(ksfd_handle *h)
+{
+    float *c32 = (h->coef32_want && coef32_alloc(h)) ? h->coef32 : nullptr;
+    h->coef32_fresh = c32 != nullptr;
+    h->coef32_want = false;
+    return c32;
+}
+static int ensure_coef32(ksfd_handle *h)
+{
+    h->coef32_want = true;
+    if (h->coef32_fresh || !coef32_alloc(h)) return KSFD_OK;
+    const long long n = (long long)(3 + h->P.nlig) * h->G.plane;
+    {
+        Scope sc(h, KC_GFIELD, 12.0 * (double)n);
+        hipLaunchKernelGGL(k_coef32, dim3(blocks_for(n / 2)), dim3(KSFD_BLOCK), 0, h->st, n, (const double *)h->coef, h->coef32);
+    }
+    HIPCHK(h, hipGetLastError());
+    h->coef32_fresh = true;
+    return KSFD_OK;
+}
+
 static int op_jcoef(ksfd_handle *h, const double *u, bool want_means = false)
 {
     const KGeom &G = h->G;
     const int nbp = plane_blocks(G);
-    if (!h->coef32 && h->poly_fp32 && fused_ok(h) && h->P.nlig <= 4 && G.plane % 2 == 0 && G.inner % 2 == 0 &&
-        hipMalloc((void **)&h->coef32, sizeof(float) * (size_t)(3 + h->P.nlig) * G.plane) != hipSuccess) { h->coef32 = nullptr; h->poly_fp32 = false; }
-    float *c32 = h->poly_fp32 ? h->coef32 : nullptr;
+    float *c32 = coef32_take(h);
     want_means = want_means && (long long)(1 + h->P.nlig) * nbp <= part_capacity();
     {
     Scope sc(h, KC_GFIELD, (8.0 * (G.F + 3 + h->P.nlig) + (c32 ? 4.0 * (3 + h->P.nlig) : 0.0)) * (double)G.plane);
@@ -303,6 +329,39 @@
     h->coef_fresh = true;
     h->mg_coef_valid = false; h->mg_shift = -1.0;
     h->spec.means_valid = h->spec.ok && (long long)(1 + h->P.nlig) * plane_blocks(h->G) <= part_capacity();
+    return KSFD_OK;
+}
+
+static bool step_head_ok(const ksfd_handle *h)
+{
+    if (!h->step_head || !fused_ok(h) || h->ring || !h->use_frozen || !h->fuse_stage || h->Pst_valid[0]) return false;
+    for (int c = 0; c < h->G.F; c++) if (h->src[0][c]) return false;
+    return (4 + h->P.nlig) * strip_waves(h) <= part_capacity();
+}
+static int op_step_head(ksfd_handle *h, double vmax[3])
+{
+    const KGeom &G = h->G;
+    const int nl = h->P.nlig;
+    const KStrips K = make_strips(h);
+    const long long nwaves = strip_waves(h);
+    double *dst = h->b0_hint ? h->b0_hint : ((h->spec_guess && h->bstore) ? h->bstore : h->bvec);
+    float *c32 = coef32_take(h);
+    h->coef_fresh = h->b0_fresh = false;
+    {
+        Scope sc(h, KC_RHS, (8.0 * (2 * G.F + 3 + nl) + (c32 ? 4.0 * (3 + nl) : 0.0)) * (double)G.nloc, vbytes(h, 2));
+        NL_DISPATCH(nl, if constexpr (NL <= 4) hipLaunchKernelGGL((k_rhs2d_head<NL>), dim3(K.nblocks), dim3(KSFD_BLOCK), 0, h->st, G, h->P, K, (const double *)h->u, dst, h->coef, c32, h->part, nwaves));
+    }
+    HIPCHK(h, hipGetLastError());
+    int rc = reduce_rows(h, 4 + nl, (int)nwaves, 2 + (2 + nl));
+    if (rc) return rc;
+    const double ntot = (double)h->cfg.n[0] * (double)h->cfg.n[1] * (double)h->cfg.n[2];
+    h->spec.a_rr = h->hres[1] / ntot;
+    for (int l = 0; l < nl; l++) h->spec.a_rU[l] = h->hres[2 + l] / ntot;
+    h->spec.means_valid = h->spec.ok;
+    vmax[0] = h->hres[2 + nl]; vmax[1] = h->hres[3 + nl]; vmax[2] = 0.0;
+    h->coef_fresh = true;
+    h->mg_coef_valid = false; h->mg_shift = -1.0;
+    h->b0_dst = dst; h->b0_norm2 = h->hres[0]; h->b0_fresh = true;
     return KSFD_OK;
 }
 
diff --git a/ksfd_amd/csrc/pointwise.hip.h b/ksfd_amd/csrc/pointwise.hip.h
--- a/ksfd_amd/csrc/pointwise.hip.h
+++ b/ksfd_amd/csrc/pointwise.hip.h
@@ -270,20 +270,21 @@
 {
     __shared__ double red[KSFD_BLOCK / KSFD_WAVE];
     const double *row = part + (long long)blockIdx.x * nblk;
-    double s = op ? -1.0e300 : 0.0;
+    const bool mx = op >= 2 ? (int)blockIdx.x >= op - 2 : op != 0;
+    double s = mx ? -1.0e300 : 0.0;
     for (int b0 = threadIdx.x; b0 < nblk; b0 += 8 * blockDim.x) {
         double t[8];
 #pragma unroll
-        for (int q = 0; q < 8; q++) { const int b = b0 + q * blockDim.x; t[q] = b < nblk ? row[b] : (op ? -1.0e300 : 0.0); }
-#pragma unroll
-        for (int q = 0; q < 8; q++) s = op ? fmax(s, t[q]) : s + t[q];
-    }
-    s = op ? ksfd_wave_max(s) : ksfd_wave_sum(s);
+        for (int q = 0; q < 8; q++) { const int b = b0 + q * blockDim.x; t[q] = b < nblk ? row[b] : (mx ? -1.0e300 : 0.0); }
+#pragma unroll
+        for (int q = 0; q < 8; q++) s = mx ? fmax(s, t[q]) : s + t[q];
+    }
+    s = mx ? ksfd_wave_max(s) : ksfd_wave_sum(s);
     if ((threadIdx.x & (KSFD_WAVE - 1)) == 0) red[threadIdx.x / KSFD_WAVE] = s;
     __syncthreads();
     if (threadIdx.x == 0) {
         double t = red[0];
-        for (int q = 1; q < KSFD_BLOCK / KSFD_WAVE; q++) t = op ? fmax(t, red[q]) : t + red[q];
+        for (int q = 1; q < KSFD_BLOCK / KSFD_WAVE; q++) t = mx ? fmax(t, red[q]) : t + red[q];
         out[blockIdx.x] = t;
         if (pub) {
             __hip_atomic_store(pub + blockIdx.x, t, __ATOMIC_RELAXED, __HIP_MEMORY_SCOPE_SYSTEM);
diff --git a/ksfd_amd/csrc/stencil.hip.h b/ksfd_amd/csrc/stencil.hip.h
--- a/ksfd_amd/csrc/stencil.hip.h
+++ b/ksfd_amd/csrc/stencil.hip.h
@@ -619,6 +619,139 @@
 }
 
 template <int NL>
+__global__ void __launch_bounds__(KSFD_BLOCK) k_rhs2d_head(KGeom G, KPhys P, KStrips S, const double *__restrict__ u, double *__restrict__ out,
+                                                           double *__restrict__ C, float *__restrict__ C32, double *__restrict__ part, long long nw)
+{
+    const KWaveJob J = ksfd_wave_job(G, S);
+    if (!J.valid) return;
+    double nacc = 0.0, mxa = 0.0, mya = 0.0, macc[NL + 1];
+#pragma unroll
+    for (int i = 0; i <= NL; i++) macc[i] = 0.0;
+    double rw[5][2], gw[5][2], uw[NL][5][2];
+    double nr[2], nu[NL][2];
+
+    auto load_row = [&](long long r) {
+        const long long o = ksfd_rowoff(G, r) + J.c0;
+        double2 t = ksfd_ld2(u + o);
+        nr[0] = t.x; nr[1] = t.y;
+#pragma unroll
+        for (int l = 0; l < NL; l++) {
+            double2 q = ksfd_ld2(u + (long long)(l + 1) * G.plane + o);
+            nu[l][0] = q.x; nu[l][1] = q.y;
+        }
+    };
+    auto push_row = [&](long long q) {
+#pragma unroll
+        for (int s = 0; s < 4; s++) {
+#pragma unroll
+            for (int e = 0; e < 2; e++) {
+                rw[s][e] = rw[s + 1][e];
+                gw[s][e] = gw[s + 1][e];
+#pragma unroll
+                for (int l = 0; l < NL; l++) uw[l][s][e] = uw[l][s + 1][e];
+            }
+        }
+        double gr[2], GU[2][NL];
+#pragma unroll
+        for (int e = 0; e < 2; e++) {
+            double U[NL];
+            double rho = ksfd_clamp(nr[e], P.rhomin);
+#pragma unroll
+            for (int l = 0; l < NL; l++) { U[l] = ksfd_clamp(nu[l][e], P.Umin); uw[l][4][e] = U[l]; }
+            ksfd_G<NL, true>(P, rho, U, gw[4][e], gr[e], GU[e]);
+            rw[4][e] = rho;
+        }
+        if (q >= J.r0 && q < J.r1 && J.store) {
+            const long long o = (long long)G.ng * G.inner + J.row(q) * G.nx + J.c0;
+            ksfd_st2(C + o, rw[4][0], rw[4][1]);
+            ksfd_st2(C + G.plane + o, gw[4][0], gw[4][1]);
+            ksfd_st2(C + 2 * G.plane + o, gr[0], gr[1]);
+#pragma unroll
+            for (int l = 0; l < NL; l++) ksfd_st2(C + (long long)(3 + l) * G.plane + o, GU[0][l], GU[1][l]);
+            if (C32) {
+                ksfd_st2(C32 + o, rw[4][0], rw[4][1]);
+                ksfd_st2(C32 + G.plane + o, gw[4][0], gw[4][1]);
+                ksfd_st2(C32 + 2 * G.plane + o, gr[0], gr[1]);
+#pragma unroll
+                for (int l = 0; l < NL; l++) ksfd_st2(C32 + (long long)(3 + l) * G.plane + o, GU[0][l], GU[1][l]);
+            }
+#pragma unroll
+            for (int e = 0; e < 2; e++) {
+                macc[0] += rw[4][e] * gr[e];
+#pragma unroll
+                for (int l = 0; l < NL; l++) macc[l + 1] += rw[4][e] * GU[e][l];
+            }
+        }
+    };
+
+    for (int q = -2; q <= 1; q++) { load_row(J.row(J.r0 + q)); push_row(J.r0 + q); }
+    load_row(J.row(J.r0 + 2));
+    for (long long r = J.r0; r < J.r1; r++) {
+        push_row(r + 2);
+        if (r + 1 < J.r1) load_row(J.row(r + 3));
+        const KX xr = ksfd_xnb(rw[2][0], rw[2][1]);
+        const KX xg = ksfd_xnb(gw[2][0], gw[2][1]);
+        double d1rx[2], d1gx[2], d2gx[2], d1gy0[2];
+        ksfd_dx(rw[2][0], rw[2][1], xr, d1rx[0], d1rx[1]);
+        ksfd_dx(gw[2][0], gw[2][1], xg, d1gx[0], d1gx[1]);
+        ksfd_dxx(gw[2][0], gw[2][1], xg, d2gx[0], d2gx[1]);
+        double res[NL + 1][2];
+#pragma unroll
+        for (int e = 0; e < 2; e++) {
+            d1gy0[e] = KSFD_D1(gw[0][e], gw[1][e], gw[3][e], gw[4][e]);
+            const double d1ry = KSFD_D1(rw[0][e], rw[1][e], rw[3][e], rw[4][e]) * P.inv_h[1];
+            const double d1gy = d1gy0[e] * P.inv_h[1];
+            const double d2gy = KSFD_D2(gw[0][e], gw[1][e], gw[2][e], gw[3][e], gw[4][e]) * P.inv_h2[1];
+            res[0][e] = (d1rx[e] * P.inv_h[0]) * (d1gx[e] * P.inv_h[0]) + d1ry * d1gy +
+                        rw[2][e] * (d2gx[e] * P.inv_h2[0] + d2gy);
+        }
+#pragma unroll
+        for (int l = 0; l < NL; l++) {
+            const KX xu = ksfd_xnb(uw[l][2][0], uw[l][2][1]);
+            double d2ux[2];
+            ksfd_dxx(uw[l][2][0], uw[l][2][1], xu, d2ux[0], d2ux[1]);
+#pragma unroll
+            for (int e = 0; e < 2; e++) {
+                const double d2uy = KSFD_D2(uw[l][0][e], uw[l][1][e], uw[l][2][e], uw[l][3][e], uw[l][4][e]) * P.inv_h2[1];
+                res[l + 1][e] = -P.lig_gamma[l] * uw[l][2][e] + P.lig_s[l] * rw[2][e] +
+                                P.lig_D[l] * (d2ux[e] * P.inv_h2[0] + d2uy);
+            }
+        }
+        if (J.store) {
+            const long long o = (long long)G.ng * G.inner + J.row(r) * G.nx + J.c0;
+#pragma unroll
+            for (int c = 0; c <= NL; c++) {
+                const double a = res[c][0], b = res[c][1];
+                ksfd_st2(out + (long long)c * G.plane + o, a, b);
+                nacc += a * a + b * b;
+            }
+            mxa = fmax(mxa, fmax(fabs(d1gx[0]), fabs(d1gx[1])));
+            mya = fmax(mya, fmax(fabs(d1gy0[0]), fabs(d1gy0[1])));
+        }
+    }
+    const bool lead = (threadIdx.x & (KSFD_WAVE - 1)) == 0;
+    nacc = ksfd_wave_sum(nacc);
+    if (lead) part[J.wid] = nacc;
+#pragma unroll
+    for (int i = 0; i <= NL; i++) {
+        const double t = ksfd_wave_sum(macc[i]);
+        if (lead) part[(long long)(1 + i) * nw + J.wid] = t;
+    }
+    mxa = ksfd_wave_max(mxa * P.inv_h[0]);
+    mya = ksfd_wave_max(mya * P.inv_h[1]);
+    if (lead) { part[(long long)(2 + NL) * nw + J.wid] = mxa; part[(long long)(3 + NL) * nw + J.wid] = mya; }
+}
+
+__global__ void __launch_bounds__(KSFD_BLOCK) k_coef32(long long n, const double *__restrict__ C, float *__restrict__ C32)
+{
+    const long long stride = (long long)gridDim.x * blockDim.x * 2;
+    for (long long e = ((long long)blockIdx.x * blockDim.x + threadIdx.x) * 2; e < n; e += stride) {
+        const double2 t = ksfd_ld2(C + e);
+        ksfd_st2(C32 + e, t.x, t.y);
+    }
+}
+
+template <int NL>
 __global__ void __launch_bounds__(KSFD_BLOCK) k_jvp2d_fused(KGeom G, KPhys P, KStrips S, const double *__restrict__ u,
                                                             const double *__restrict__ v, int mode, double shift,
                                                             double *__restrict__ out)
```
